# Quantus-Network/qp-zk-circuits

Measured on AMD Instinct MI355X. Metric: Wormhole proofs/sec, higher is better.
Workload: dtype u64

## Files before the change

### include/qpgpu.h

```cpp
#ifndef QPGPU_H
#define QPGPU_H
#include <stddef.h>
#include <stdint.h>

#ifdef __cplusplus
extern "C" {
#endif

typedef struct qpgpu_ctx qpgpu_ctx;
typedef struct qpgpu_circuit qpgpu_circuit;

enum {
    QPGPU_OK = 0,
    QPGPU_EINVAL = -1,
    QPGPU_EDEVICE = -2,
    QPGPU_ENOMEM = -3,
    QPGPU_EUNSAT = -4,
    QPGPU_EBUFSIZE = -5
};

int qpgpu_ctx_create(int device, qpgpu_ctx **out);
void qpgpu_ctx_destroy(qpgpu_ctx *ctx);
const char *qpgpu_last_error(const qpgpu_ctx *ctx);
int qpgpu_ctx_set_stream(qpgpu_ctx *ctx, void *hip_stream);
int qpgpu_sync(qpgpu_ctx *ctx);
const char *qpgpu_version(void);
int qpgpu_ctx_pci_bus_id(const qpgpu_ctx *ctx, char *out, size_t out_len);
int qpgpu_crash_trace_armed(void);

int qpgpu_profile_enable(qpgpu_ctx *ctx, int on);
int qpgpu_profile_read(qpgpu_ctx *ctx, const char *kernel, double *total_ms, uint64_t *launches);

int qpgpu_malloc(qpgpu_ctx *ctx, size_t bytes, void **dptr);
int qpgpu_free(qpgpu_ctx *ctx, void *dptr);
int qpgpu_free_scrubbed(qpgpu_ctx *ctx, void *dptr, size_t bytes);
int qpgpu_memcpy_h2d(qpgpu_ctx *ctx, void *dst_dev, const void *src_host, size_t bytes);
int qpgpu_memcpy_d2h(qpgpu_ctx *ctx, void *dst_host, const void *src_dev, size_t bytes);
int qpgpu_memcpy_d2d(qpgpu_ctx *ctx, void *dst_dev, const void *src_dev, size_t bytes);

typedef struct { uint64_t word; uint32_t region; uint32_t pinned; uint64_t offset_words; uint64_t alloc_bytes; } qpgpu_residue_hit;
#define QPGPU_RESIDUE_MAX_NEEDLES 16
int qpgpu_ctx_residue_scan(qpgpu_ctx *ctx, const uint64_t *needles, size_t n_needles, uint64_t region_mask,
                           uint64_t *hits, qpgpu_residue_hit *first_hits, size_t cap, uint64_t *bytes_scanned);
const char *qpgpu_residue_region_name(uint32_t region);
int qpgpu_ctx_residue_audit_begin(qpgpu_ctx *ctx, const uint64_t *needles, size_t n_needles);
int qpgpu_ctx_residue_audit_end(qpgpu_ctx *ctx, uint64_t *hits, qpgpu_residue_hit *first_hits, size_t cap, uint64_t *buffers_released);

#define QPGPU_HASH_POSEIDON 0
#define QPGPU_HASH_POSEIDON2 1
#define QPGPU_POSEIDON2_PARAM_WORDS 146
int qpgpu_ctx_set_hasher(qpgpu_ctx *ctx, int kind, const uint64_t *params, size_t n_words);
int qpgpu_ctx_get_hasher(const qpgpu_ctx *ctx);
int qpgpu_set_hasher(int kind, const uint64_t *params, size_t n_words);
int qpgpu_get_hasher(void);

enum {
    QPGPU_NTT_FORWARD = 0,
    QPGPU_NTT_INVERSE = 1,
    QPGPU_NTT_OUT_BITREV = 2
};
int qpgpu_ntt_batch(qpgpu_ctx *ctx, uint64_t *data, unsigned log_n, size_t batch, int flags,
                    uint64_t coset_shift);
int qpgpu_ntt_batch_dev(qpgpu_ctx *ctx, const uint64_t *d_in, uint64_t *d_out, unsigned log_n,
                        size_t batch, int flags, uint64_t coset_shift);
int qpgpu_lde_batch_dev(qpgpu_ctx *ctx, const uint64_t *d_coeffs, uint64_t *d_out, unsigned log_n,
                        unsigned rate_bits, size_t batch, int flags, uint64_t coset_shift);

int qpgpu_poseidon_permute_dev(qpgpu_ctx *ctx, uint64_t *d_states, size_t n);
int qpgpu_poseidon2_hash_pad10_dev(qpgpu_ctx *ctx, const uint64_t *params, size_t n_words, const uint64_t *d_in, size_t len,
                                   size_t count, uint64_t *d_out);
size_t qpgpu_merkle_digest_count(unsigned log_leaves, unsigned cap_height);
int qpgpu_merkle_build_dev(qpgpu_ctx *ctx, const uint64_t *d_cols, uint64_t col_stride, uint32_t n_cols,
                           unsigned log_leaves, unsigned cap_height, uint64_t *d_digests, uint64_t *h_cap_out);
int qpgpu_merkle_build_rows_dev(qpgpu_ctx *ctx, const uint64_t *d_rows, uint32_t width, unsigned log_leaves,
                                unsigned cap_height, uint64_t *d_digests, uint64_t *h_cap_out);

int qpgpu_circuit_load(qpgpu_ctx *ctx, const uint64_t *pack_words, size_t n_words, qpgpu_circuit **out);
int qpgpu_circuit_load_batch(qpgpu_ctx *ctx, const uint64_t *pack_words, size_t n_words, unsigned max_batch, qpgpu_circuit **out);
unsigned qpgpu_circuit_max_batch(const qpgpu_circuit *c);
size_t qpgpu_circuit_num_public_inputs(const qpgpu_circuit *c);
void qpgpu_circuit_free(qpgpu_circuit *c);
int qpgpu_circuit_scrub(qpgpu_circuit *c);
int qpgpu_circuit_constants_sigmas_cap(const qpgpu_circuit *c, uint64_t *out, size_t out_words);
int qpgpu_circuit_set_blinding_seed(qpgpu_circuit *c, uint64_t seed);
int qpgpu_circuit_set_witness_check(qpgpu_circuit *c, int on);
int qpgpu_circuit_set_quotient_fused(qpgpu_circuit *c, int on);
int qpgpu_circuit_quotient_info(const qpgpu_circuit *c, int *fused_enabled, int *fused_selected);
int qpgpu_circuit_quotient_pair_info(const qpgpu_circuit *c, int *enabled, int *selected);
size_t qpgpu_proof_size(const qpgpu_circuit *c);
int qpgpu_prove(qpgpu_circuit *c, const uint64_t *wires, const uint64_t *public_inputs, uint8_t *out, size_t out_cap, size_t *out_len);
int qpgpu_prove_dev(qpgpu_circuit *c, const uint64_t *d_wires, const uint64_t *public_inputs, uint8_t *out, size_t out_cap, size_t *out_len);
int qpgpu_prove_batch_dev(qpgpu_circuit *c, const uint64_t *const *d_wires, uint32_t batch, const uint64_t *const *public_inputs,
                          uint8_t *const *outs, size_t out_cap, size_t *out_lens);

int qpgpu_witness_info(qpgpu_circuit *c, uint64_t *num_generators, uint64_t *num_levels, uint64_t *num_free_cells);
int qpgpu_witness_free_mask(qpgpu_circuit *c, uint8_t *mask, size_t mask_len);
int qpgpu_generate_witness_dev(qpgpu_circuit *c, uint64_t *d_wires, const uint64_t *public_inputs);
int qpgpu_generate_witness(qpgpu_circuit *c, uint64_t *wires, const uint64_t *public_inputs);
int qpgpu_circuit_gate_rows(const qpgpu_circuit *c, unsigned gate_type, uint32_t *rows_out, size_t cap, size_t *count);
int qpgpu_generate_witness_batch_dev(qpgpu_circuit *c, uint64_t *d_wires, uint32_t batch, const uint64_t *public_inputs);
int qpgpu_generate_witness_partial_dev(qpgpu_circuit *c, const uint64_t *cells, const uint64_t *values, size_t count,
                                       const uint64_t *public_inputs, uint64_t *d_wires);
int qpgpu_generate_witness_partial_batch_dev(qpgpu_circuit *c, const uint64_t *cells, size_t count, const uint64_t *values,
                                             const uint64_t *public_inputs, uint32_t batch, uint64_t *d_wires, int *status);
int qpgpu_witness_partial_prepare(qpgpu_circuit *c, const uint64_t *cells, size_t count, uint32_t max_batch);
int qpgpu_generate_witness_partial_batch_blinded_dev(qpgpu_circuit *c, const uint64_t *cells, size_t count, size_t n_blinding, const uint64_t *values,
                                                     const uint8_t *seeds, const uint64_t *public_inputs, uint32_t batch, uint64_t *d_wires, int *status);
int qpgpu_witness_public_inputs_dev(qpgpu_circuit *c, const uint64_t *d_wires, uint32_t batch, uint64_t *public_inputs_out);

typedef struct qpgpu_oracle qpgpu_oracle;
#define QPGPU_ORACLE_VALUES 0u
#define QPGPU_ORACLE_COEFFS 1u
#define QPGPU_ORACLE_BLINDING 2u
#define QPGPU_ORACLE_DEVICE_INPUT 4u
int qpgpu_oracle_commit(qpgpu_ctx *ctx, const uint64_t *polys, uint32_t num_polys, unsigned degree_bits, unsigned rate_bits,
                        unsigned cap_height, unsigned flags, uint64_t blinding_seed, uint32_t blinding_stream, qpgpu_oracle **out);
void qpgpu_oracle_free(qpgpu_oracle *o);
int qpgpu_oracle_cap(const qpgpu_oracle *o, uint64_t *out, size_t out_words);
int qpgpu_oracle_eval(qpgpu_oracle *o, const uint64_t point[2], uint32_t first, uint32_t count, uint64_t *out);
#define QPGPU_ORACLE_READ_COEFFS 0u
#define QPGPU_ORACLE_READ_LDE 1u
int qpgpu_oracle_read(qpgpu_oracle *o, unsigned what, uint32_t first, uint32_t count, uint64_t *out);
int qpgpu_oracle_device_ptrs(const qpgpu_oracle *o, const uint64_t **d_coeffs, const uint64_t **d_lde, const uint64_t **d_digests);
int qpgpu_oracle_open(qpgpu_oracle *o, const uint64_t *indices, size_t n, uint64_t *rows_out, uint64_t *paths_out);
size_t qpgpu_oracle_leaf_width(const qpgpu_oracle *o);

int qpgpu_oracle_commit_sharded(qpgpu_ctx *const *ctxs, uint32_t n_ctx, const uint64_t *polys, uint32_t num_polys,
                                unsigned degree_bits, unsigned rate_bits, unsigned cap_height, unsigned flags,
                                uint64_t blinding_seed, uint32_t blinding_stream, qpgpu_oracle **out);
uint32_t qpgpu_oracle_shards(const qpgpu_oracle *o);
int qpgpu_oracle_shard_range(const qpgpu_oracle *o, uint32_t shard, uint64_t *first_leaf, uint64_t *num_leaves);
int qpgpu_oracle_shard_device_ptrs(const qpgpu_oracle *o, uint32_t shard, const uint64_t **d_lde, const uint64_t **d_digests);

int qpgpu_oracle_commit_batch(qpgpu_ctx *ctx, const uint64_t *const *polys, uint32_t batch, uint32_t num_polys, unsigned degree_bits,
                              unsigned rate_bits, unsigned cap_height, unsigned flags, uint64_t blinding_seed, uint32_t blinding_stream,
                              qpgpu_oracle **out);
uint32_t qpgpu_oracle_batch(const qpgpu_oracle *o);
int qpgpu_oracle_strides(const qpgpu_oracle *o, uint64_t *coeffs, uint64_t *lde, uint64_t *digests);
int qpgpu_oracle_eval_batch(qpgpu_oracle *o, const uint64_t *points, uint32_t first, uint32_t count, uint64_t *out);
int qpgpu_oracle_open_batch(qpgpu_oracle *o, const uint64_t *indices, size_t n, uint64_t *rows_out, uint64_t *paths_out);

typedef struct {
    uint64_t sponge_state[12];
    uint64_t input_buffer[8];
    uint64_t output_buffer[8];
    uint32_t input_len, output_len;
} qpgpu_challenger;
void qpgpu_challenger_init(qpgpu_challenger *c);
int qpgpu_ctx_challenger_observe(const qpgpu_ctx *ctx, qpgpu_challenger *c, const uint64_t *elements, size_t n);
int qpgpu_ctx_challenger_get(const qpgpu_ctx *ctx, qpgpu_challenger *c, uint64_t *out);
void qpgpu_challenger_observe(qpgpu_challenger *c, const uint64_t *elements, size_t n);
uint64_t qpgpu_challenger_get(qpgpu_challenger *c);

typedef struct { uint32_t oracle, first, count; } qpgpu_fri_range;
typedef struct { uint64_t point[2]; uint32_t num_ranges; qpgpu_fri_range ranges[8]; } qpgpu_fri_batch;
typedef struct {
    uint32_t rate_bits, cap_height, proof_of_work_bits, num_query_rounds;
    uint32_t num_reduction_rounds; uint32_t reduction_arity_bits[16];
} qpgpu_fri_params;
size_t qpgpu_fri_proof_size(qpgpu_oracle *const *oracles, uint32_t num_oracles, const qpgpu_fri_params *params);
int qpgpu_fri_prove(qpgpu_ctx *ctx, qpgpu_oracle *const *oracles, uint32_t num_oracles, const qpgpu_fri_batch *batches,
                    uint32_t num_batches, const qpgpu_fri_params *params, qpgpu_challenger *challenger,
                    uint8_t *out, size_t out_cap, size_t *out_len);

typedef struct qpgpu_fri_session qpgpu_fri_session;
int qpgpu_fri_begin(qpgpu_ctx *ctx, qpgpu_oracle *const *oracles, uint32_t num_oracles, const qpgpu_fri_batch *batches,
                    uint32_t num_batches, const qpgpu_fri_params *params, const uint64_t alpha[2], qpgpu_fri_session **out);
int qpgpu_fri_round_commit(qpgpu_fri_session *s, uint64_t *cap_out, size_t cap_words);
int qpgpu_fri_round_fold(qpgpu_fri_session *s, const uint64_t beta[2]);
int qpgpu_fri_final_poly(qpgpu_fri_session *s, uint64_t *out, size_t out_words, size_t *num_coeffs);
size_t qpgpu_fri_query_size(const qpgpu_fri_session *s);
int qpgpu_fri_open(qpgpu_fri_session *s, const uint64_t *indices, size_t n, uint8_t *out, size_t out_cap, size_t *out_len);
void qpgpu_fri_session_free(qpgpu_fri_session *s);
int qpgpu_fri_grind(qpgpu_ctx *ctx, const qpgpu_challenger *c, unsigned proof_of_work_bits, uint64_t *nonce_out);

int qpgpu_fri_prove_batch(qpgpu_ctx *ctx, qpgpu_oracle *const *oracles, uint32_t num_oracles, const qpgpu_fri_batch *batches,
                          uint32_t num_batches, const uint64_t *points, uint32_t batch, const qpgpu_fri_params *params,
                          qpgpu_challenger *challengers, uint8_t *const *outs, size_t out_cap, size_t *out_lens);
int qpgpu_fri_begin_batch(qpgpu_ctx *ctx, qpgpu_oracle *const *oracles, uint32_t num_oracles, const qpgpu_fri_batch *batches,
                          uint32_t num_batches, const uint64_t *points, uint32_t batch, const qpgpu_fri_params *params,
                          const uint64_t *alphas, qpgpu_fri_session **out);
uint32_t qpgpu_fri_session_batch(const qpgpu_fri_session *s);
int qpgpu_fri_grind_batch(qpgpu_ctx *ctx, const qpgpu_challenger *cs, uint32_t batch, unsigned proof_of_work_bits, uint64_t *nonces_out);

typedef struct qpgpu_stage_plan qpgpu_stage_plan;
#define QPGPU_STAGE_ERR_CAP 256
int qpgpu_stage_plan_create(qpgpu_ctx *ctx, const uint64_t *words, size_t n_words, const qpgpu_oracle *cs_oracle,
                            qpgpu_stage_plan **out, char *err);
void qpgpu_stage_plan_free(qpgpu_stage_plan *plan);
int qpgpu_stage_plan_info(const qpgpu_stage_plan *plan, unsigned *degree_bits, unsigned *num_challenges,
                          unsigned *num_partial_products, unsigned *quotient_degree_factor, int *fused_selected);
int qpgpu_stage_partial_products(qpgpu_stage_plan *plan, const uint64_t *wires, int wires_on_device, const uint64_t *betas,
                                 const uint64_t *gammas, uint64_t *d_out);
int qpgpu_stage_quotient(qpgpu_stage_plan *plan, const qpgpu_oracle *wires_oracle, const qpgpu_oracle *zs_pp_oracle,
                         const uint64_t *betas, const uint64_t *gammas, const uint64_t *alphas, const uint64_t *public_inputs_hash,
                         uint64_t *d_out);

int qpgpu_stage_plan_create_sharded(qpgpu_ctx *ctx, const uint64_t *words, size_t n_words, const qpgpu_oracle *cs_oracle,
                                    qpgpu_stage_plan **out, char *err);
uint32_t qpgpu_stage_plan_shards(const qpgpu_stage_plan *plan);

int qpgpu_stage_plan_create_batch(qpgpu_ctx *ctx, const uint64_t *words, size_t n_words, const qpgpu_oracle *cs_oracle,
                                  uint32_t max_batch, qpgpu_stage_plan **out, char *err);
uint32_t qpgpu_stage_plan_max_batch(const qpgpu_stage_plan *plan);
int qpgpu_stage_partial_products_batch(qpgpu_stage_plan *plan, const uint64_t *const *wires, uint32_t batch, int wires_on_device,
                                       const uint64_t *betas, const uint64_t *gammas, uint64_t *d_out);
int qpgpu_stage_quotient_batch(qpgpu_stage_plan *plan, const qpgpu_oracle *wires_oracle, const qpgpu_oracle *zs_pp_oracle, uint32_t batch,
                               const uint64_t *betas, const uint64_t *gammas, const uint64_t *alphas,
                               const uint64_t *public_inputs_hashes, uint64_t *d_out);

typedef struct qpgpu_pool qpgpu_pool;
int qpgpu_pool_create(int device, const uint64_t *pack_words, size_t n_words, unsigned workers, qpgpu_pool **out);
int qpgpu_pool_create_batched(int device, const uint64_t *pack_words, size_t n_words, unsigned workers, unsigned max_batch, qpgpu_pool **out);
#define QPGPU_POOL_HOST_WITNESS 1u
int qpgpu_pool_create_multi(const int *devices, unsigned n_devices, const uint64_t *pack_words, size_t n_words, unsigned workers_per_device,
                            unsigned max_batch, unsigned flags, qpgpu_pool **out);
void qpgpu_pool_destroy(qpgpu_pool *p);
int qpgpu_pool_scrub(qpgpu_pool *p);
int qpgpu_pool_residue_scan(qpgpu_pool *p, const uint64_t *needles, size_t n_needles, uint64_t region_mask,
                            uint64_t *hits, qpgpu_residue_hit *first_hits, size_t cap, uint64_t *bytes_scanned);
int qpgpu_pool_set_witness_check(qpgpu_pool *p, int on);
size_t qpgpu_pool_proof_size(const qpgpu_pool *p);
unsigned qpgpu_pool_workers(const qpgpu_pool *p);
unsigned qpgpu_pool_devices(const qpgpu_pool *p);
int qpgpu_pool_serialized(const qpgpu_pool *p);
const char *qpgpu_pool_last_error(const qpgpu_pool *p);
int qpgpu_pool_submit(qpgpu_pool *p, const uint64_t *d_wires, const uint64_t *public_inputs, uint8_t *out, size_t out_cap, uint64_t *ticket);
int qpgpu_pool_submit_on(qpgpu_pool *p, unsigned device_index, const uint64_t *d_wires, const uint64_t *public_inputs, uint8_t *out, size_t out_cap, uint64_t *ticket);
int qpgpu_pool_submit_host(qpgpu_pool *p, const uint64_t *wires, const uint64_t *public_inputs, uint8_t *out, size_t out_cap, uint64_t *ticket);
int qpgpu_pool_set_partial_cells(qpgpu_pool *p, const uint64_t *cells, size_t count);
int qpgpu_pool_set_partial_cells_blinded(qpgpu_pool *p, const uint64_t *cells, size_t count, size_t n_blinding);
int qpgpu_pool_submit_partial(qpgpu_pool *p, const uint64_t *values, const uint64_t *public_inputs, uint8_t *out, size_t out_cap, uint64_t *ticket);
int qpgpu_pool_wait(qpgpu_pool *p, uint64_t ticket, size_t *out_len);

size_t qpgpu_poseidon_constants(uint64_t *round_constants_360, uint64_t *fast_partial, size_t fast_partial_cap);

size_t qpgpu_synth_pack_words(unsigned degree_bits, unsigned num_wires, unsigned num_routed);
size_t qpgpu_synth_p2_sites(unsigned degree_bits, unsigned num_public_inputs, unsigned flags, uint64_t *out, size_t cap_words);
size_t qpgpu_synth_pack_words_ex(unsigned degree_bits, unsigned num_wires, unsigned num_routed, unsigned flags);
int qpgpu_synth_circuit_ex(unsigned degree_bits, unsigned num_wires, unsigned num_routed, unsigned num_public_inputs,
                           uint64_t seed, unsigned flags, uint64_t *pack_out, size_t pack_cap_words, size_t *pack_words,
                           uint64_t *wires_out, uint64_t *pis_out);
int qpgpu_synth_circuit(unsigned degree_bits, unsigned num_wires, unsigned num_routed, unsigned num_public_inputs,
                        uint64_t seed, uint64_t *pack_out, size_t pack_cap_words, size_t *pack_words,
                        uint64_t *wires_out, uint64_t *pis_out);

enum {
    QPGPU_FP_CANON = 0, QPGPU_FP_ADD, QPGPU_FP_SUB, QPGPU_FP_NEG, QPGPU_FP_MUL, QPGPU_FP_SQR, QPGPU_FP_REDUCE128, QPGPU_FP_REDUCE96,
    QPGPU_FP_MUL_EPS, QPGPU_FP_ADD_CANONICAL, QPGPU_FP_MUL7, QPGPU_FP_INV, QPGPU_FP_POW, QPGPU_FP_MUL_POW2, QPGPU_FP_MUL_POW2_DYN,
    QPGPU_FP_MUL_GROUP, QPGPU_FP_ACC, QPGPU_FP_E2_ADD, QPGPU_FP_E2_SUB, QPGPU_FP_E2_MUL, QPGPU_FP_E2_SCALE, QPGPU_FP_E2_INV,
    QPGPU_FP_E2_POW, QPGPU_FP_DIF_REGS, QPGPU_FP_DIF_SPARSE, QPGPU_FP_OP_COUNT
};
int qpgpu_field_probe(qpgpu_ctx *ctx, unsigned op, unsigned param, const uint64_t *a, const uint64_t *b, size_t n,
                      uint64_t *out, size_t out_words, int on_device);

#ifdef __cplusplus
}
#endif
#endif
```

### qp-zk-circuits_amd/__init__.py

```python
from .binding import poseidon_constants, synth_circuit, Circuit, QpGpu, QpGpuError, lib_path, load_library, P, MULT_GEN
from .binding import StagePlan, stage_header_words
from .binding import FriSession, fri_grind
from .binding import FriVerifier
from .binding import fri_prove_batch, fri_grind_batch
from .binding import PolyOracle, Challenger, fri_prove, set_hasher_poseidon, set_hasher_poseidon2, ProvingPool
from .binding import pack_header, pack_public_input_cells, Verifier, poseidon2_qp_params, synth_p2_sites
from .binding import pack_p2_layout, pack_trailers, p2_site_cells, P2_NO_SWAP
from .binding import CircuitConfig, circuit_config, validate_circuit_config
from .binding import FP, FP_OPS, field_probe_host, field_probe_shape
from . import sharding
from . import aggregation
from . import leaf
from . import recursion
```

### qp-zk-circuits_amd/binding.py

```python
import ctypes
import os

import numpy as np

P = 0xFFFFFFFF00000001
MULT_GEN = 14293326489335486720

NTT_FORWARD = 0
NTT_INVERSE = 1
NTT_OUT_BITREV = 2

_HERE = os.path.dirname(os.path.abspath(__file__))


def lib_path():
    return os.path.join(_HERE, "libqpgpu.so")


class QpGpuError(RuntimeError):
    def __init__(self, code, msg):
        super().__init__(f"qpgpu error {code}: {msg}")
        self.code = code


_lib = None


def load_library():
    global _lib
    if _lib is not None:
        return _lib
    path = lib_path()
    if not os.path.exists(path):
        raise FileNotFoundError(f"{path} missing: run `python -c 'import __graft_entry__ as g; g.build()'`")
    lib = ctypes.CDLL(path)
    c = ctypes
    vp, u64p = c.c_void_p, c.c_void_p
    sigs = {
        "qpgpu_version": (c.c_char_p, []),
        "qpgpu_ctx_pci_bus_id": (c.c_int, [c.c_void_p, c.c_char_p, c.c_size_t]),
        "qpgpu_verifier_create": (c.c_int, [vp, c.c_size_t, vp, c.c_size_t, c.c_int, vp, c.c_size_t, c.POINTER(vp), c.c_char_p]),
        "qpgpu_verifier_free": (None, [vp]),
        "qpgpu_verifier_proof_size": (c.c_size_t, [vp]),
        "qpgpu_verifier_constants_sigmas_cap": (c.c_int, [vp, vp, c.c_size_t]),
        "qpgpu_verifier_verify": (c.c_int, [vp, c.c_char_p, c.c_size_t, c.c_char_p]),
        "qpgpu_verifier_verify_many": (c.c_int, [vp, vp, vp, c.c_size_t, c.c_uint, vp, c.c_char_p]),
        "qpgpu_verifier_verify_many_device": (c.c_int, [vp, vp, vp, vp, c.c_size_t, c.c_uint, vp, vp, c.c_char_p]),
        "qpgpu_verifier_verify_many_device_ex": (c.c_int, [vp, vp, vp, vp, c.c_size_t, c.c_uint, c.c_uint, vp, vp, c.c_char_p]),
        "qpgpu_fri_verifier_create": (c.c_int, [vp, c.c_int, vp, c.c_size_t, c.POINTER(vp), c.c_char_p]),
        "qpgpu_fri_verifier_free": (None, [vp]),
        "qpgpu_fri_verifier_proof_size": (c.c_size_t, [vp]),
        "qpgpu_fri_verifier_num_openings": (c.c_size_t, [vp]),
        "qpgpu_fri_verifier_challenges": (c.c_int, [vp, vp, c.c_char_p, c.c_size_t, u64p, u64p, c.POINTER(c.c_uint64), u64p, c.c_char_p]),
        "qpgpu_fri_verify": (c.c_int, [vp, vp, u64p, u64p, u64p, u64p, c.c_uint64, u64p, c.c_char_p, c.c_size_t, c.c_char_p]),
        "qpgpu_fri_verify_many_device": (c.c_int, [vp, vp, c.c_size_t, vp, vp, u64p, u64p, u64p, u64p, u64p, u64p, vp, vp, vp, vp, c.c_char_p]),
        "qpgpu_ctx_create": (c.c_int, [c.c_int, c.POINTER(vp)]),
        "qpgpu_ctx_destroy": (None, [vp]),
        "qpgpu_last_error": (c.c_char_p, [vp]),
        "qpgpu_ctx_set_stream": (c.c_int, [vp, vp]),
        "qpgpu_sync": (c.c_int, [vp]),
        "qpgpu_profile_enable": (c.c_int, [vp, c.c_int]),
        "qpgpu_profile_read": (c.c_int, [vp, c.c_char_p, c.POINTER(c.c_double), c.POINTER(c.c_uint64)]),
        "qpgpu_malloc": (c.c_int, [vp, c.c_size_t, c.POINTER(vp)]),
        "qpgpu_free": (c.c_int, [vp, vp]),
        "qpgpu_free_scrubbed": (c.c_int, [vp, vp, c.c_size_t]),
        "qpgpu_memcpy_h2d": (c.c_int, [vp, vp, vp, c.c_size_t]),
        "qpgpu_memcpy_d2h": (c.c_int, [vp, vp, vp, c.c_size_t]),
        "qpgpu_memcpy_d2d": (c.c_int, [vp, vp, vp, c.c_size_t]),
        "qpgpu_ntt_batch": (c.c_int, [vp, u64p, c.c_uint, c.c_size_t, c.c_int, c.c_uint64]),
        "qpgpu_ntt_batch_dev": (c.c_int, [vp, u64p, u64p, c.c_uint, c.c_size_t, c.c_int, c.c_uint64]),
        "qpgpu_lde_batch_dev": (c.c_int, [vp, u64p, u64p, c.c_uint, c.c_uint, c.c_size_t, c.c_int, c.c_uint64]),
        "qpgpu_poseidon_permute_dev": (c.c_int, [vp, u64p, c.c_size_t]),
        "qpgpu_poseidon2_hash_pad10_dev": (c.c_int, [vp, u64p, c.c_size_t, u64p, c.c_size_t, c.c_size_t, u64p]),
        "qpgpu_poseidon2_qp_params": (c.c_size_t, [u64p, c.c_size_t]),
        "qpgpu_zk_leaf_hash_batch": (c.c_int, [vp, vp, c.c_size_t, vp]),
        "qpgpu_zk_tree_build": (c.c_int, [vp, vp, c.c_size_t, c.c_uint, c.c_uint, c.POINTER(vp), c.c_char_p]),
        "qpgpu_zk_tree_free": (None, [vp]),
        "qpgpu_zk_tree_depth": (c.c_uint, [vp]),
        "qpgpu_zk_tree_leaf_count": (c.c_size_t, [vp]),
        "qpgpu_zk_tree_root": (c.c_int, [vp, vp]),
        "qpgpu_zk_tree_read_level": (c.c_int, [vp, c.c_uint, c.c_size_t, c.c_size_t, vp]),
        "qpgpu_zk_tree_open": (c.c_int, [vp, vp, c.c_size_t, vp, vp]),
        "qpgpu_zk_tree_build_reserved": (c.c_int, [vp, vp, c.c_size_t, c.c_size_t, c.c_uint, c.c_uint, c.POINTER(vp), c.c_char_p]),
        "qpgpu_zk_tree_capacity": (c.c_size_t, [vp]),
        "qpgpu_zk_tree_append": (c.c_int, [vp, vp, c.c_size_t, c.c_uint, vp, c.c_char_p]),
        "qpgpu_zk_tree_snapshot": (c.c_int, [vp, vp]),
        "qpgpu_zk_tree_open_at": (c.c_int, [vp, vp, vp, c.c_size_t, vp, vp]),
        "qpgpu_zk_tree_snapshots_at": (c.c_int, [vp, vp, c.c_size_t, vp]),
        "qpgpu_zk_tree_snapshot_check": (c.c_int, [vp, vp]),
        "qpgpu_zk_tree_open_at_counts": (c.c_int, [vp, vp, vp, c.c_size_t, vp, vp, vp]),
        "qpgpu_zk_tree_truncate": (c.c_int, [vp, c.c_size_t, vp, c.c_char_p]),
        "qpgpu_poseidon2_hash_pad10": (c.c_int, [u64p, c.c_size_t, u64p, c.c_size_t, u64p]),
        "qpgpu_crash_trace_armed": (c.c_int, []),
        "qpgpu_circuit_num_public_inputs": (c.c_size_t, [vp]),
        "qpgpu_merkle_digest_count": (c.c_size_t, [c.c_uint, c.c_uint]),
        "qpgpu_merkle_build_dev": (c.c_int, [vp, u64p, c.c_uint64, c.c_uint32, c.c_uint, c.c_uint, u64p, u64p]),
        "qpgpu_merkle_build_rows_dev": (c.c_int, [vp, u64p, c.c_uint32, c.c_uint, c.c_uint, u64p, u64p]),
        "qpgpu_circuit_load": (c.c_int, [vp, u64p, c.c_size_t, c.POINTER(vp)]),
        "qpgpu_circuit_load_batch": (c.c_int, [vp, u64p, c.c_size_t, c.c_uint, c.POINTER(vp)]),
        "qpgpu_circuit_max_batch": (c.c_uint, [vp]),
        "qpgpu_circuit_scrub": (c.c_int, [vp]),
        "qpgpu_prove_batch_dev": (c.c_int, [vp, vp, c.c_uint32, vp, vp, c.c_size_t, vp]),
        "qpgpu_ctx_set_hasher": (c.c_int, [vp, c.c_int, u64p, c.c_size_t]),
        "qpgpu_ctx_get_hasher": (c.c_int, [vp]),
        "qpgpu_ctx_challenger_observe": (c.c_int, [vp, vp, u64p, c.c_size_t]),
        "qpgpu_ctx_challenger_get": (c.c_int, [vp, vp, c.POINTER(c.c_uint64)]),
        "qpgpu_pool_create_batched": (c.c_int, [c.c_int, u64p, c.c_size_t, c.c_uint, c.c_uint, c.POINTER(vp)]),
        "qpgpu_circuit_free": (None, [vp]),
        "qpgpu_circuit_constants_sigmas_cap": (c.c_int, [vp, u64p, c.c_size_t]),
        "qpgpu_proof_size": (c.c_size_t, [vp]),
        "qpgpu_circuit_set_blinding_seed": (c.c_int, [vp, c.c_uint64]),
        "qpgpu_circuit_set_witness_check": (c.c_int, [vp, c.c_int]),
        "qpgpu_circuit_set_quotient_fused": (c.c_int, [vp, c.c_int]),
        "qpgpu_circuit_quotient_info": (c.c_int, [vp, c.POINTER(c.c_int), c.POINTER(c.c_int)]),
        "qpgpu_circuit_quotient_pair_info": (c.c_int, [vp, c.POINTER(c.c_int), c.POINTER(c.c_int)]),
        "qpgpu_circuit_gate_rows": (c.c_int, [vp, c.c_uint, vp, c.c_size_t, c.POINTER(c.c_size_t)]),
        "qpgpu_prove": (c.c_int, [vp, u64p, u64p, vp, c.c_size_t, c.POINTER(c.c_size_t)]),
        "qpgpu_prove_dev": (c.c_int, [vp, u64p, u64p, vp, c.c_size_t, c.POINTER(c.c_size_t)]),
        "qpgpu_poseidon_constants": (c.c_size_t, [u64p, u64p, c.c_size_t]),
        "qpgpu_pool_create": (c.c_int, [c.c_int, u64p, c.c_size_t, c.c_uint, c.POINTER(vp)]),
        "qpgpu_pool_destroy": (None, [vp]),
        "qpgpu_pool_proof_size": (c.c_size_t, [vp]),
        "qpgpu_pool_workers": (c.c_uint, [vp]),
        "qpgpu_pool_last_error": (c.c_char_p, [vp]),
        "qpgpu_pool_submit": (c.c_int, [vp, u64p, u64p, vp, c.c_size_t, c.POINTER(c.c_uint64)]),
        "qpgpu_pool_wait": (c.c_int, [vp, c.c_uint64, c.POINTER(c.c_size_t)]),
        "qpgpu_pool_set_witness_check": (c.c_int, [vp, c.c_int]),
        "qpgpu_pool_create_multi": (c.c_int, [vp, c.c_uint, u64p, c.c_size_t, c.c_uint, c.c_uint, c.c_uint, c.POINTER(vp)]),
        "qpgpu_pool_devices": (c.c_uint, [vp]),
        "qpgpu_pool_serialized": (c.c_int, [vp]),
        "qpgpu_pool_set_partial_cells": (c.c_int, [vp, u64p, c.c_size_t]),
        "qpgpu_pool_set_partial_cells_blinded": (c.c_int, [vp, u64p, c.c_size_t, c.c_size_t]),
        "qpgpu_pool_submit_on": (c.c_int, [vp, c.c_uint, u64p, u64p, vp, c.c_size_t, c.POINTER(c.c_uint64)]),
        "qpgpu_pool_submit_host": (c.c_int, [vp, u64p, u64p, vp, c.c_size_t, c.POINTER(c.c_uint64)]),
        "qpgpu_pool_submit_partial": (c.c_int, [vp, u64p, u64p, vp, c.c_size_t, c.POINTER(c.c_uint64)]),
        "qpgpu_set_hasher": (c.c_int, [c.c_int, u64p, c.c_size_t]),
        "qpgpu_get_hasher": (c.c_int, []),
        "qpgpu_witness_info": (c.c_int, [vp, c.POINTER(c.c_uint64), c.POINTER(c.c_uint64), c.POINTER(c.c_uint64)]),
        "qpgpu_witness_free_mask": (c.c_int, [vp, vp, c.c_size_t]),
        "qpgpu_generate_witness_dev": (c.c_int, [vp, u64p, u64p]),
        "qpgpu_generate_witness": (c.c_int, [vp, u64p, u64p]),
        "qpgpu_generate_witness_batch_dev": (c.c_int, [vp, u64p, c.c_uint32, u64p]),
        "qpgpu_generate_witness_partial_dev": (c.c_int, [vp, u64p, u64p, c.c_size_t, u64p, u64p]),
        "qpgpu_generate_witness_partial_batch_dev": (c.c_int, [vp, u64p, c.c_size_t, u64p, u64p, c.c_uint32, u64p, vp]),
        "qpgpu_generate_witness_partial_batch_blinded_dev": (c.c_int, [vp, u64p, c.c_size_t, c.c_size_t, u64p, c.c_char_p, u64p, c.c_uint32, u64p, vp]),
        "qpgpu_witness_public_inputs_dev": (c.c_int, [vp, u64p, c.c_uint32, u64p]),
        "qpgpu_witness_partial_prepare": (c.c_int, [vp, u64p, c.c_size_t, c.c_uint32]),
        "qpgpu_oracle_commit": (c.c_int, [vp, u64p, c.c_uint32, c.c_uint, c.c_uint, c.c_uint, c.c_uint, c.c_uint64, c.c_uint32,
                                          c.POINTER(vp)]),
        "qpgpu_oracle_free": (None, [vp]),
        "qpgpu_oracle_cap": (c.c_int, [vp, u64p, c.c_size_t]),
        "qpgpu_oracle_eval": (c.c_int, [vp, u64p, c.c_uint32, c.c_uint32, u64p]),
        "qpgpu_oracle_read": (c.c_int, [vp, c.c_uint, c.c_uint32, c.c_uint32, u64p]),
        "qpgpu_oracle_device_ptrs": (c.c_int, [vp, c.POINTER(vp), c.POINTER(vp), c.POINTER(vp)]),
        "qpgpu_oracle_open": (c.c_int, [vp, u64p, c.c_size_t, u64p, u64p]),
        "qpgpu_oracle_leaf_width": (c.c_size_t, [vp]),
        "qpgpu_oracle_commit_sharded": (c.c_int, [c.POINTER(vp), c.c_uint32, u64p, c.c_uint32, c.c_uint, c.c_uint, c.c_uint, c.c_uint,
                                                  c.c_uint64, c.c_uint32, c.POINTER(vp)]),
        "qpgpu_oracle_shards": (c.c_uint32, [vp]),
        "qpgpu_oracle_shard_range": (c.c_int, [vp, c.c_uint32, c.POINTER(c.c_uint64), c.POINTER(c.c_uint64)]),
        "qpgpu_oracle_shard_device_ptrs": (c.c_int, [vp, c.c_uint32, c.POINTER(vp), c.POINTER(vp)]),
        "qpgpu_stage_plan_create": (c.c_int, [vp, u64p, c.c_size_t, vp, c.POINTER(vp), c.c_char_p]),
        "qpgpu_stage_plan_create_sharded": (c.c_int, [vp, u64p, c.c_size_t, vp, c.POINTER(vp), c.c_char_p]),
        "qpgpu_stage_plan_shards": (c.c_uint32, [vp]),
        "qpgpu_stage_plan_free": (None, [vp]),
        "qpgpu_stage_plan_info": (c.c_int, [vp, c.POINTER(c.c_uint), c.POINTER(c.c_uint), c.POINTER(c.c_uint), c.POINTER(c.c_uint),
                                            c.POINTER(c.c_int)]),
        "qpgpu_stage_partial_products": (c.c_int, [vp, u64p, c.c_int, u64p, u64p, u64p]),
        "qpgpu_stage_quotient": (c.c_int, [vp, vp, vp, u64p, u64p, u64p, u64p, u64p]),
        "qpgpu_challenger_init": (None, [vp]),
        "qpgpu_challenger_observe": (None, [vp, u64p, c.c_size_t]),
        "qpgpu_challenger_get": (c.c_uint64, [vp]),
        "qpgpu_fri_proof_size": (c.c_size_t, [c.POINTER(vp), c.c_uint32, vp]),
        "qpgpu_fri_prove": (c.c_int, [vp, c.POINTER(vp), c.c_uint32, vp, c.c_uint32, vp, vp, vp, c.c_size_t,
                                      c.POINTER(c.c_size_t)]),
        "qpgpu_fri_begin": (c.c_int, [vp, c.POINTER(vp), c.c_uint32, vp, c.c_uint32, vp, u64p, c.POINTER(vp)]),
        "qpgpu_fri_round_commit": (c.c_int, [vp, u64p, c.c_size_t]),
        "qpgpu_fri_round_fold": (c.c_int, [vp, u64p]),
        "qpgpu_fri_final_poly": (c.c_int, [vp, u64p, c.c_size_t, c.POINTER(c.c_size_t)]),
        "qpgpu_fri_query_size": (c.c_size_t, [vp]),
        "qpgpu_fri_open": (c.c_int, [vp, u64p, c.c_size_t, vp, c.c_size_t, c.POINTER(c.c_size_t)]),
        "qpgpu_fri_session_free": (None, [vp]),
        "qpgpu_fri_grind": (c.c_int, [vp, vp, c.c_uint, c.POINTER(c.c_uint64)]),
        "qpgpu_oracle_commit_batch": (c.c_int, [vp, c.POINTER(vp), c.c_uint32, c.c_uint32, c.c_uint, c.c_uint, c.c_uint, c.c_uint,
                                                c.c_uint64, c.c_uint32, c.POINTER(vp)]),
        "qpgpu_oracle_batch": (c.c_uint32, [vp]),
        "qpgpu_oracle_strides": (c.c_int, [vp, c.POINTER(c.c_uint64), c.POINTER(c.c_uint64), c.POINTER(c.c_uint64)]),
        "qpgpu_oracle_eval_batch": (c.c_int, [vp, u64p, c.c_uint32, c.c_uint32, u64p]),
        "qpgpu_oracle_open_batch": (c.c_int, [vp, u64p, c.c_size_t, u64p, u64p]),
        "qpgpu_stage_plan_create_batch": (c.c_int, [vp, u64p, c.c_size_t, vp, c.c_uint32, c.POINTER(vp), c.c_char_p]),
        "qpgpu_stage_plan_max_batch": (c.c_uint32, [vp]),
        "qpgpu_stage_partial_products_batch": (c.c_int, [vp, c.POINTER(vp), c.c_uint32, c.c_int, u64p, u64p, u64p]),
        "qpgpu_stage_quotient_batch": (c.c_int, [vp, vp, vp, c.c_uint32, u64p, u64p, u64p, u64p, u64p]),
        "qpgpu_fri_prove_batch": (c.c_int, [vp, c.POINTER(vp), c.c_uint32, vp, c.c_uint32, u64p, c.c_uint32, vp, vp, c.POINTER(vp),
                                            c.c_size_t, c.POINTER(c.c_size_t)]),
        "qpgpu_fri_begin_batch": (c.c_int, [vp, c.POINTER(vp), c.c_uint32, vp, c.c_uint32, u64p, c.c_uint32, vp, u64p, c.POINTER(vp)]),
        "qpgpu_fri_session_batch": (c.c_uint32, [vp]),
        "qpgpu_fri_grind_batch": (c.c_int, [vp, vp, c.c_uint32, c.c_uint, c.POINTER(c.c_uint64)]),
        "qpgpu_field_probe": (c.c_int, [vp, c.c_uint, c.c_uint, u64p, u64p, c.c_size_t, u64p, c.c_size_t, c.c_int]),
        "qpgpu_synth_pack_words": (c.c_size_t, [c.c_uint, c.c_uint, c.c_uint]),
        "qpgpu_synth_pack_words_ex": (c.c_size_t, [c.c_uint, c.c_uint, c.c_uint, c.c_uint]),
        "qpgpu_synth_p2_sites": (c.c_size_t, [c.c_uint, c.c_uint, c.c_uint, u64p, c.c_size_t]),
        "qpgpu_synth_circuit_ex": (c.c_int, [c.c_uint, c.c_uint, c.c_uint, c.c_uint, c.c_uint64, c.c_uint, u64p, c.c_size_t,
                                             c.POINTER(c.c_size_t), u64p, u64p]),
        "qpgpu_synth_circuit": (c.c_int, [c.c_uint, c.c_uint, c.c_uint, c.c_uint, c.c_uint64, u64p, c.c_size_t,
                                          c.POINTER(c.c_size_t), u64p, u64p]),
        "qpgpu_ctx_residue_scan": (c.c_int, [vp, u64p, c.c_size_t, c.c_uint64, c.POINTER(c.c_uint64), vp, c.c_size_t, c.POINTER(c.c_uint64)]),
        "qpgpu_residue_region_name": (c.c_char_p, [c.c_uint32]),
        "qpgpu_ctx_residue_audit_begin": (c.c_int, [vp, u64p, c.c_size_t]),
        "qpgpu_ctx_residue_audit_end": (c.c_int, [vp, c.POINTER(c.c_uint64), vp, c.c_size_t, c.POINTER(c.c_uint64)]),
        "qpgpu_pool_scrub": (c.c_int, [vp]),
        "qpgpu_pool_residue_scan": (c.c_int, [vp, u64p, c.c_size_t, c.c_uint64, c.POINTER(c.c_uint64), vp, c.c_size_t, c.POINTER(c.c_uint64)]),
    }
    for name, (res, args) in sigs.items():
        fn = getattr(lib, name)
        fn.restype = res
        fn.argtypes = args
    _lib = lib
    return lib


def exported_symbols():
    import glob
    import re
    names = set()
    for hdr in glob.glob(os.path.join(os.path.dirname(_HERE), "include", "*.h")):
        names |= set(re.findall(r"\b(qpgpu_[a-z0-9_]+)\s*\(", open(hdr).read()))
    return sorted(names)


def set_hasher_poseidon():
    load_library().qpgpu_set_hasher(0, None, 0)


def _p2_block(rc_ext, rc_int, diag_m1, m4):
    return np.concatenate([np.asarray(rc_ext, dtype=np.uint64).ravel(), np.asarray(rc_int, dtype=np.uint64).ravel(),
                           np.asarray(diag_m1, dtype=np.uint64).ravel(), np.asarray(m4, dtype=np.uint64).ravel()])


def set_hasher_poseidon2(rc_ext, rc_int, diag_m1, m4):
    flat = _p2_block(rc_ext, rc_int, diag_m1, m4)
    rc = load_library().qpgpu_set_hasher(1, flat.ctypes.data, flat.size)
    if rc != 0:
        raise QpGpuError(rc, "qpgpu_set_hasher: bad Poseidon2 parameter block")


def poseidon2_qp_params():
    flat = np.empty(146, dtype=np.uint64)
    n = load_library().qpgpu_poseidon2_qp_params(flat.ctypes.data, flat.size)
    assert n == 146
    return flat[:96].reshape(8, 12).copy(), flat[96:118].copy(), flat[118:130].copy(), flat[130:146].reshape(4, 4).copy()


def poseidon_constants():
    lib = load_library()
    n = lib.qpgpu_poseidon_constants(None, None, 0)
    rc = np.empty(360, dtype=np.uint64); fp = np.empty(n, dtype=np.uint64)
    lib.qpgpu_poseidon_constants(rc.ctypes.data, fp.ctypes.data, n)
    return rc, fp


FP_OPS = ("canon", "add", "sub", "neg", "mul", "sqr", "reduce128", "reduce96", "mul_eps", "add_canonical", "mul7", "inv", "pow",
          "mul_pow2", "mul_pow2_dyn", "mul_group", "acc", "e2_add", "e2_sub", "e2_mul", "e2_scale", "e2_inv", "e2_pow", "dif_regs",
          "dif_sparse")
FP = {name: i for i, name in enumerate(FP_OPS)}


def field_probe_shape(op, param=0):
    name = FP_OPS[op]
    if name in ("mul_group", "acc"):
        return (param, param, param if name == "mul_group" else 1)
    if name in ("e2_add", "e2_sub", "e2_mul"):
        return (2, 2, 2)
    if name in ("e2_scale", "e2_pow"):
        return (2, 1, 2)
    if name == "e2_inv":
        return (2, 0, 2)
    if name in ("dif_regs", "dif_sparse"):
        return (1 << (param & 0xFF), 0, 1 << (param & 0xFF))
    return (1, 1 if name in ("add", "sub", "mul", "reduce128", "reduce96", "add_canonical", "pow") else 0, 1)

# ... 681 lines not shown
        b, g = self._challenges_batch(betas, batch), self._challenges_batch(gammas, batch)
        if isinstance(wires[0], np.ndarray):
            keep = [np.ascontiguousarray(w, dtype=np.uint64) for w in wires]
            ptrs, on_dev = [w.ctypes.data for w in keep], 0
        else:
            ptrs, on_dev = [_ptr(w) for w in wires], 1
        arr = (ctypes.c_void_p * batch)(*ptrs)
        out = self.gpu.alloc(batch * self.num_zs_pp * self.n * 8)
        rc = self.gpu.lib.qpgpu_stage_partial_products_batch(self.h, arr, batch, on_dev, b.ctypes.data, g.ctypes.data, out.ptr)
        if rc != 0:
            out.free(scrub=True)
            self.gpu._check(rc)
        return out

    def quotient_batch(self, wires_oracle, zs_pp_oracle, batch, betas, gammas, alphas, public_inputs_hashes):
        b, g, a = (self._challenges_batch(x, batch) for x in (betas, gammas, alphas))
        pih = self._challenges_batch(public_inputs_hashes, batch, 4)
        out = self.gpu.alloc(batch * self.num_quotient * self.n * 8)
        rc = self.gpu.lib.qpgpu_stage_quotient_batch(self.h, wires_oracle.h, zs_pp_oracle.h, batch, b.ctypes.data, g.ctypes.data,
                                                     a.ctypes.data, pih.ctypes.data, out.ptr)
        if rc != 0:
            out.free(scrub=True)
            self.gpu._check(rc)
        return out


def _fri_args(oracles, batches, reduction_arity_bits, rate_bits, cap_height, proof_of_work_bits, num_query_rounds):
    hs = (ctypes.c_void_p * len(oracles))(*[o.h for o in oracles])
    bs = (_FriBatch * len(batches))()
    for b, (point, ranges) in zip(bs, batches):
        if np.ndim(point) == 1:
            b.point[0], b.point[1] = int(point[0]), int(point[1])
        b.num_ranges = len(ranges)
        for r, (o, f, cnt) in zip(b.ranges, ranges):
            r.oracle, r.first, r.count = o, f, cnt
    prm = _FriParams(rate_bits, cap_height, proof_of_work_bits, num_query_rounds, len(reduction_arity_bits))
    for i, a in enumerate(reduction_arity_bits):
        prm.reduction_arity_bits[i] = a
    return hs, bs, prm


def fri_prove(gpu, oracles, batches, challenger, reduction_arity_bits, rate_bits=3, cap_height=4, proof_of_work_bits=16,
              num_query_rounds=28):
    hs, bs, prm = _fri_args(oracles, batches, reduction_arity_bits, rate_bits, cap_height, proof_of_work_bits, num_query_rounds)
    size = gpu.lib.qpgpu_fri_proof_size(hs, len(oracles), ctypes.byref(prm))
    if size == 0:
        raise QpGpuError(-1, "fri_prove: bad oracles or FRI parameters")
    out = np.empty(size, dtype=np.uint8)
    ln = ctypes.c_size_t()
    gpu._check(gpu.lib.qpgpu_fri_prove(gpu.ctx, hs, len(oracles), ctypes.byref(bs), len(batches), ctypes.byref(prm),
                                       ctypes.byref(challenger.state), out.ctypes.data, out.size, ctypes.byref(ln)))
    return out[:ln.value].tobytes()


def fri_prove_batch(gpu, oracles, batches, challengers, reduction_arity_bits, rate_bits=3, cap_height=4, proof_of_work_bits=16,
                    num_query_rounds=28):
    nb = len(challengers)
    hs, bs, prm = _fri_args(oracles, batches, reduction_arity_bits, rate_bits, cap_height, proof_of_work_bits, num_query_rounds)
    pts = np.ascontiguousarray(np.array([np.array(pt, dtype=np.uint64).reshape(nb, 2) for pt, _ in batches], dtype=np.uint64))
    size = gpu.lib.qpgpu_fri_proof_size(hs, len(oracles), ctypes.byref(prm))
    if size == 0:
        raise QpGpuError(-1, "fri_prove: bad oracles or FRI parameters")
    states = (ChallengerState * nb)()
    for i, ch in enumerate(challengers):
        ctypes.memmove(ctypes.byref(states[i]), ctypes.byref(ch.state), ctypes.sizeof(ChallengerState))
    outs = [np.empty(size, dtype=np.uint8) for _ in range(nb)]
    optr = (ctypes.c_void_p * nb)(*[o.ctypes.data for o in outs])
    lens = (ctypes.c_size_t * nb)()
    gpu._check(gpu.lib.qpgpu_fri_prove_batch(gpu.ctx, hs, len(oracles), ctypes.byref(bs), len(batches), pts.ctypes.data, nb,
                                             ctypes.byref(prm), ctypes.byref(states), optr, size, lens))
    for i, ch in enumerate(challengers):
        ctypes.memmove(ctypes.byref(ch.state), ctypes.byref(states[i]), ctypes.sizeof(ChallengerState))
    return [outs[i][:lens[i]].tobytes() for i in range(nb)]


def fri_grind_batch(gpu, challengers, proof_of_work_bits):
    nb = len(challengers)
    states = (ChallengerState * nb)()
    for i, ch in enumerate(challengers):
        ctypes.memmove(ctypes.byref(states[i]), ctypes.byref(ch.state), ctypes.sizeof(ChallengerState))
    nonces = (ctypes.c_uint64 * nb)()
    gpu._check(gpu.lib.qpgpu_fri_grind_batch(gpu.ctx, ctypes.byref(states), nb, proof_of_work_bits, nonces))
    return [int(x) for x in nonces]


def fri_grind(gpu, challenger, proof_of_work_bits):
    nonce = ctypes.c_uint64()
    gpu._check(gpu.lib.qpgpu_fri_grind(gpu.ctx, ctypes.byref(challenger.state), proof_of_work_bits, ctypes.byref(nonce)))
    return int(nonce.value)


class FriSession:

    def __init__(self, gpu, oracles, batches, alpha, reduction_arity_bits, rate_bits=3, cap_height=4, batch=None):
        self.gpu, self.oracles, self.batch = gpu, list(oracles), batch
        hs, bs, prm = _fri_args(oracles, batches, reduction_arity_bits, rate_bits, cap_height, 0, 0)
        h = ctypes.c_void_p()
        if batch is None:
            a = np.array([int(alpha[0]), int(alpha[1])], dtype=np.uint64)
            gpu._check(gpu.lib.qpgpu_fri_begin(gpu.ctx, hs, len(oracles), ctypes.byref(bs), len(batches), ctypes.byref(prm), a.ctypes.data,
                                               ctypes.byref(h)))
        else:
            a = np.ascontiguousarray(np.array(alpha, dtype=np.uint64).reshape(batch, 2))
            pts = np.ascontiguousarray(np.array([np.array(pt, dtype=np.uint64).reshape(batch, 2) for pt, _ in batches], dtype=np.uint64))
            gpu._check(gpu.lib.qpgpu_fri_begin_batch(gpu.ctx, hs, len(oracles), ctypes.byref(bs), len(batches), pts.ctypes.data, batch,
                                                     ctypes.byref(prm), a.ctypes.data, ctypes.byref(h)))
            assert int(gpu.lib.qpgpu_fri_session_batch(h)) == batch
        self.h = h
        self.cap_height, self.arity_bits = cap_height, list(reduction_arity_bits)
        self.lde_size = 1 << (oracles[0].degree_bits + rate_bits)
        self.final_len = 1 << (oracles[0].degree_bits - sum(self.arity_bits))
        self.query_size = int(gpu.lib.qpgpu_fri_query_size(h))

    def close(self):
        if self.h:
            self.gpu.lib.qpgpu_fri_session_free(self.h)
            self.h = None

    def __enter__(self):
        return self

    def __exit__(self, *a):
        self.close()

    def round_commit(self):
        shape = (1 << self.cap_height, 4) if self.batch is None else (self.batch, 4 << self.cap_height)
        cap = np.empty(shape, dtype=np.uint64)
        self.gpu._check(self.gpu.lib.qpgpu_fri_round_commit(self.h, cap.ctypes.data, cap.size))
        return cap

    def round_fold(self, beta):
        b = np.ascontiguousarray(np.array(beta, dtype=np.uint64).reshape(self.batch or 1, 2))
        self.gpu._check(self.gpu.lib.qpgpu_fri_round_fold(self.h, b.ctypes.data))

    def final_poly(self):
        out = np.empty((self.final_len, 2) if self.batch is None else (self.batch, self.final_len, 2), dtype=np.uint64)
        n = ctypes.c_size_t()
        self.gpu._check(self.gpu.lib.qpgpu_fri_final_poly(self.h, out.ctypes.data, out.size, ctypes.byref(n)))
        assert n.value == self.final_len
        return out

    def open(self, indices):
        if self.batch is not None:
            idx = np.ascontiguousarray(np.array(indices, dtype=np.uint64).reshape(self.batch, -1))
            n, per = idx.shape[1], idx.shape[1] * self.query_size
            out = np.empty(max(1, self.batch * per), dtype=np.uint8)
            ln = ctypes.c_size_t()
            self.gpu._check(self.gpu.lib.qpgpu_fri_open(self.h, idx.ctypes.data if n else None, n, out.ctypes.data, self.batch * per,
                                                        ctypes.byref(ln)))
            assert ln.value == self.batch * per
            return [out[b * per:(b + 1) * per].tobytes() for b in range(self.batch)]
        idx = np.ascontiguousarray(indices, dtype=np.uint64).ravel()
        out = np.empty(max(1, idx.size * self.query_size), dtype=np.uint8)
        ln = ctypes.c_size_t()
        self.gpu._check(self.gpu.lib.qpgpu_fri_open(self.h, idx.ctypes.data if idx.size else None, idx.size, out.ctypes.data,
                                                    idx.size * self.query_size, ctypes.byref(ln)))
        return out[:ln.value].tobytes()


class _FriOracleShape(ctypes.Structure):
    _fields_ = [("num_polys", ctypes.c_uint32), ("blinded", ctypes.c_uint32)]


class _FriInstance(ctypes.Structure):
    _fields_ = [("degree_bits", ctypes.c_uint32), ("num_oracles", ctypes.c_uint32), ("oracles", ctypes.POINTER(_FriOracleShape)),
                ("num_batches", ctypes.c_uint32), ("batches", ctypes.POINTER(_FriBatch)), ("params", _FriParams)]
# ... 241 lines not shown
        return self._submitted(rc, t, (p, out, None))

    def scrub(self):
        rc = self.lib.qpgpu_pool_scrub(self.h)
        if rc != 0:
            raise QpGpuError(rc, self.lib.qpgpu_pool_last_error(self.h).decode())

    def residue_scan(self, needles, regions=None, cap=16):
        rc, hits, first, nbytes = _residue_call(self.lib.qpgpu_pool_residue_scan, self.h, needles, regions, cap)
        if rc != 0:
            raise QpGpuError(rc, self.lib.qpgpu_pool_last_error(self.h).decode())
        return hits, first, nbytes

    def wait(self, ticket, copy=True):
        ln = ctypes.c_size_t()
        rc = self.lib.qpgpu_pool_wait(self.h, ticket, ctypes.byref(ln))
        p, out, _ = self._keep.pop(ticket, (None, None, None))
        if rc != 0:
            raise QpGpuError(rc, self.lib.qpgpu_pool_last_error(self.h).decode())
        return out[:ln.value].tobytes() if copy else ln.value


class _ResidueAudit:
    def __init__(self, gpu, needles, cap):
        self.gpu, self.cap = gpu, cap
        self.needles = np.ascontiguousarray(needles, dtype=np.uint64)
        self.hits = self.buffers_released = None
        self.first_hits = []

    def __enter__(self):
        self.gpu._check(self.gpu.lib.qpgpu_ctx_residue_audit_begin(self.gpu.ctx, self.needles.ctypes.data, self.needles.size))
        return self

    def __exit__(self, *a):
        hits, released = ctypes.c_uint64(), ctypes.c_uint64()
        first = _blank_hits(self.cap)
        self.gpu._check(self.gpu.lib.qpgpu_ctx_residue_audit_end(self.gpu.ctx, ctypes.byref(hits), first, self.cap, ctypes.byref(released)))
        self.hits, self.buffers_released = hits.value, released.value
        self.first_hits = _written_hits(first, self.cap)


class _Stage3:

    def poseidon_permute(self, states):
        st = np.ascontiguousarray(states, dtype=np.uint64).reshape(-1, 12)
        d = self.to_device(st)
        self._check(self.lib.qpgpu_poseidon_permute_dev(self.ctx, d.ptr, st.shape[0]))
        out = d.download().reshape(-1, 12)
        d.free()
        return out

    def poseidon2_hash_pad10(self, preimages, params=None):
        pre = np.ascontiguousarray(preimages, dtype=np.uint64)
        pre = pre.reshape(1, -1) if pre.ndim == 1 else pre
        count, ln = pre.shape
        d_in = self.to_device(pre) if pre.size else self.alloc(8)
        d_out = self.alloc(max(count, 1) * 32)
        try:
            if params is None:
                self._check(self.lib.qpgpu_poseidon2_hash_pad10_dev(self.ctx, None, 0, d_in.ptr, ln, count, d_out.ptr))
            else:
                blk = np.ascontiguousarray(params, dtype=np.uint64)
                self._check(self.lib.qpgpu_poseidon2_hash_pad10_dev(self.ctx, blk.ctypes.data, blk.size, d_in.ptr, ln, count, d_out.ptr))
            self.sync()
            return d_out.download()[:count * 4].reshape(count, 4).copy()
        finally:
            d_in.free(); d_out.free()

    def merkle_digest_count(self, log_leaves, cap_height):
        return self.lib.qpgpu_merkle_digest_count(log_leaves, cap_height)

    def merkle_build_dev(self, d_cols, col_stride, n_cols, log_leaves, cap_height, d_digests):
        cap = np.empty((1 << cap_height, 4), dtype=np.uint64)
        self._check(self.lib.qpgpu_merkle_build_dev(self.ctx, _ptr(d_cols), col_stride, n_cols, log_leaves,
                                                    cap_height, _ptr(d_digests), cap.ctypes.data))
        return cap

    def merkle_build_rows_dev(self, d_rows, width, log_leaves, cap_height, d_digests):
        cap = np.empty((1 << cap_height, 4), dtype=np.uint64)
        self._check(self.lib.qpgpu_merkle_build_rows_dev(self.ctx, _ptr(d_rows), width, log_leaves, cap_height,
                                                         _ptr(d_digests), cap.ctypes.data))
        return cap


class QpGpu(_Stage3):

    def __init__(self, device=0, stream=None, hasher=None):
        self.lib = load_library()
        ctx = ctypes.c_void_p()
        rc = self.lib.qpgpu_ctx_create(device, ctypes.byref(ctx))
        if rc != 0:
            raise QpGpuError(rc, "qpgpu_ctx_create failed (no gfx950 device visible?)")
        self.ctx = ctx
        if hasher is not None:
            if isinstance(hasher, str):
                self._check(self.lib.qpgpu_ctx_set_hasher(self.ctx, 0, None, 0))
            else:
                flat = _p2_block(*hasher)
                self._check(self.lib.qpgpu_ctx_set_hasher(self.ctx, 1, flat.ctypes.data, flat.size))
        if stream is not None:
            self._check(self.lib.qpgpu_ctx_set_stream(self.ctx, ctypes.c_void_p(stream)))

    def close(self):
        if self.ctx:
            self.lib.qpgpu_ctx_destroy(self.ctx)
            self.ctx = None

    def __enter__(self):
        return self

    def __exit__(self, *a):
        self.close()

    def _check(self, rc):
        if rc != 0:
            raise QpGpuError(rc, self.lib.qpgpu_last_error(self.ctx).decode())

    def last_error(self):
        return self.lib.qpgpu_last_error(self.ctx).decode()

    def sync(self):
        self._check(self.lib.qpgpu_sync(self.ctx))

    def commit_sharded(self, ctxs, polys, **kw):
        assert ctxs and ctxs[0] is self, "the home context comes first"
        return PolyOracle.commit_sharded(ctxs, polys, **kw)

    def pci_bus_id(self):
        buf = ctypes.create_string_buffer(16)
        self._check(self.lib.qpgpu_ctx_pci_bus_id(self.ctx, buf, 16))
        return buf.value.decode()

    def profile(self, on=True):
        self._check(self.lib.qpgpu_profile_enable(self.ctx, 1 if on else 0))

    def profile_read(self, kernel):
        ms, n = ctypes.c_double(), ctypes.c_uint64()
        self._check(self.lib.qpgpu_profile_read(self.ctx, kernel.encode(), ctypes.byref(ms), ctypes.byref(n)))
        return ms.value, n.value

    def residue_scan(self, needles, regions=None, cap=16):
        rc, hits, first, nbytes = _residue_call(self.lib.qpgpu_ctx_residue_scan, self.ctx, needles, regions, cap)
        self._check(rc)
        return hits, first, nbytes

    def residue_audit(self, needles, cap=16):
        return _ResidueAudit(self, needles, cap)

    def alloc(self, nbytes):
        return DeviceBuffer(self, nbytes)

    def to_device(self, arr):
        arr = np.ascontiguousarray(arr)
        return DeviceBuffer(self, arr.nbytes).upload(arr)

    def field_probe(self, op, a, b=None, param=0):
        rc, out = _field_probe(self.ctx, op, a, b, param, True)
        self._check(rc)
        return out

    def ntt_host(self, data, log_n, inverse=False, coset_shift=0, bitrev=False):
        a = np.array(data, dtype=np.uint64, copy=True).reshape(-1, 1 << log_n)
        flags = (NTT_INVERSE if inverse else 0) | (NTT_OUT_BITREV if bitrev else 0)
        self._check(self.lib.qpgpu_ntt_batch(self.ctx, a.ctypes.data, log_n, a.shape[0], flags, coset_shift))
        return a

# ... 16 lines not shown
```

### qp-zk-circuits_amd/csrc/fri_api.cpp

```cpp
#include <hip/hip_runtime.h>
#include <algorithm>
#include <cstring>
#include <string>
#include "fri_prover.hpp"
#include "oracle_handle.hpp"

using gl::e2;
using gl::u64;

namespace {
struct FriCall {
    FriParams fp;
    std::vector<size_t> widths;
    std::vector<FriBatch> bs;
    std::vector<const PolyOracle *> os;
    size_t max_count = 0;
    uint32_t nb = 1;
};

int fri_setup(qpgpu_oracle *const *oracles, uint32_t n, const qpgpu_fri_params *params, FriParams &fp, std::vector<size_t> &widths) {
    if (!oracles || n == 0 || !params || params->num_reduction_rounds > 16) return QPGPU_EINVAL;
    for (uint32_t i = 0; i < n; i++) if (!oracles[i] || oracles[i]->ctx != oracles[0]->ctx) return QPGPU_EINVAL;
    fp.degree_bits = oracles[0]->o.log_n; fp.rate_bits = params->rate_bits; fp.cap_h = params->cap_height;
    fp.pow_bits = params->proof_of_work_bits; fp.num_queries = params->num_query_rounds;
// ... 198 lines not shown
        return ctx->fail(QPGPU_EINVAL, "fri_round_commit: cap_words is " + std::to_string(cap_words) + ", the cap has " + std::to_string(want) + " words" +
                                           (s->st.nb > 1 ? " for the session's " + std::to_string(s->st.nb) + " proofs" : ""));
    QP_FRI_ORDER(s, FriSteps::COMMIT);
    QP_TRY(fri_round_commit(s->st));
    std::memcpy(cap_out, s->st.caps.back().data(), cap_words * 8);
    return QPGPU_OK;
}

int qpgpu_fri_round_fold(qpgpu_fri_session *s, const uint64_t *beta) {
    if (!s) return QPGPU_EINVAL;
    qpgpu_ctx *ctx = s->ctx;
    QP_DEV(ctx);
    if (!beta) return ctx->fail(QPGPU_EINVAL, "fri_round_fold: beta is NULL");
    QP_FRI_ORDER(s, FriSteps::FOLD);
    std::vector<e2> b(s->st.nb);
    for (uint32_t i = 0; i < s->st.nb; i++) b[i] = gl::e2_make(gl::canon(beta[2 * i]), gl::canon(beta[2 * i + 1]));
    return fri_round_fold(s->st, b.data());
}

int qpgpu_fri_final_poly(qpgpu_fri_session *s, uint64_t *out, size_t out_words, size_t *num_coeffs) {
    if (!s) return QPGPU_EINVAL;
    qpgpu_ctx *ctx = s->ctx;
    QP_DEV(ctx);
    if (!out) return ctx->fail(QPGPU_EINVAL, "fri_final_poly: out is NULL");
    const size_t len = s->st.w->proof.final_len, nb = s->st.nb;
    if (out_words != nb * 2 * len)
        return ctx->fail(QPGPU_EINVAL, "fri_final_poly: out_words is " + std::to_string(out_words) + ", the final polynomial has " + std::to_string(nb * 2 * len) + " words" +
                                           (nb > 1 ? " for the session's " + std::to_string(nb) + " proofs" : ""));
    QP_FRI_ORDER(s, FriSteps::FINAL_POLY);
    std::vector<u64> fc;
    QP_TRY(fri_final_poly(s->st, fc));
    for (size_t b = 0; b < nb; b++)
        for (size_t i = 0; i < len; i++) { out[2 * (b * len + i)] = fc[2 * b * len + i]; out[2 * (b * len + i) + 1] = fc[2 * b * len + len + i]; }
    if (num_coeffs) *num_coeffs = len;
    return QPGPU_OK;
}

size_t qpgpu_fri_query_size(const qpgpu_fri_session *s) { return s ? s->st.w->proof.round_bytes : 0; }

int qpgpu_fri_open(qpgpu_fri_session *s, const uint64_t *indices, size_t n, uint8_t *out, size_t out_cap, size_t *out_len) {
    if (!s) return QPGPU_EINVAL;
    qpgpu_ctx *ctx = s->ctx;
    QP_DEV(ctx);
    QP_FRI_ORDER(s, FriSteps::OPEN);
    if (n == 0) { if (out_len) *out_len = 0; return QPGPU_OK; }
    if (!indices) return ctx->fail(QPGPU_EINVAL, "fri_open: indices is NULL");
    if (!out) return ctx->fail(QPGPU_EINVAL, "fri_open: out is NULL");
    const size_t qs = qpgpu_fri_query_size(s), nb = s->st.nb;
    if (out_cap / qs / nb < n)
        return ctx->fail(QPGPU_EINVAL, "fri_open: out_cap is " + std::to_string(out_cap) + ", " + std::to_string(n) + " query rounds take " +
                                           (nb > 1 ? std::to_string(nb) + " x " : "") + std::to_string(n) + " x " + std::to_string(qs) + " bytes");
    const unsigned L = s->st.p.degree_bits + s->st.p.rate_bits;
    for (size_t b = 0; b < nb; b++)
        for (size_t i = 0; i < n; i++)
            if (indices[b * n + i] >> L)
                return ctx->fail(QPGPU_EINVAL, "fri_open: indices[" + (nb > 1 ? std::to_string(b) + "][" : "") + std::to_string(i) + "] = " + std::to_string(indices[b * n + i]) +
                                                   " is not below 2^" + std::to_string(L));
    Stager &stage = s->space.stage;
    if (!s->opened) { s->opened = true; s->open_pos = stage.pos; }
    std::vector<ByteWriter> ws;
    for (size_t b = 0; b < nb; b++) ws.push_back(ByteWriter{out + b * n * qs, n * qs});
    std::vector<u64> idx;
    for (size_t at = 0; at < n; at += kOpenChunk) {
        stage.pos = s->open_pos;
        const uint32_t m = (uint32_t)std::min<size_t>(kOpenChunk, n - at);
        idx.resize(nb * m);
        for (size_t b = 0; b < nb; b++) std::memcpy(idx.data() + b * m, indices + b * n + at, (size_t)m * 8);
        QP_TRY(fri_gather(s->st, idx.data(), m, ws.data()));
    }
    if (out_len) *out_len = nb * n * qs;
    return QPGPU_OK;
}

static int grind_impl(qpgpu_ctx *ctx, const qpgpu_challenger *cs, uint32_t nb, unsigned proof_of_work_bits, uint64_t *nonces_out) {
    if (proof_of_work_bits > 40) return ctx->fail(QPGPU_EINVAL, "fri_grind: proof_of_work_bits above 40");
    std::vector<Challenger> chs(nb, Challenger(ctx->hasher));
    for (uint32_t b = 0; b < nb; b++) {
        if (!challenger_to_host(&cs[b], chs[b])) return ctx->fail(QPGPU_EINVAL, "fri_grind: invalid challenger state (input_len must be < 8, output_len <= 8)");
        if (chs[b].n_in != chs[0].n_in) return ctx->fail(QPGPU_EINVAL, "fri_grind: challengers[" + std::to_string(b) + "] holds another number of pending inputs than challengers[0]: the transcripts of a batch advance together");
    }
    if (proof_of_work_bits == 0) { for (uint32_t b = 0; b < nb; b++) nonces_out[b] = 0; return QPGPU_OK; }
    ctx->hasher_in_use = true;
    QP_TRY(merkle_ensure_constants(ctx));
    QP_TRY(ctx->ensure_scratch((size_t)nb * 16 * 8));
    Stager bounce;
    std::vector<u64> nonces(nb, 0);
    u64 *t = ctx->scratch;
    QP_TRY(fri_grind(ctx, chs.data(), nb, proof_of_work_bits, PowTables{t, t + 12 * (size_t)nb, t + 13 * (size_t)nb}, bounce, nonces.data()));
    for (uint32_t b = 0; b < nb; b++) nonces_out[b] = nonces[b];
    return QPGPU_OK;
}

int qpgpu_fri_grind(qpgpu_ctx *ctx, const qpgpu_challenger *c, unsigned proof_of_work_bits, uint64_t *nonce_out) {
    if (!ctx || !c || !nonce_out) return QPGPU_EINVAL;
    QP_DEV(ctx);
    return grind_impl(ctx, c, 1, proof_of_work_bits, nonce_out);
}

int qpgpu_fri_grind_batch(qpgpu_ctx *ctx, const qpgpu_challenger *cs, uint32_t batch, unsigned proof_of_work_bits, uint64_t *nonces_out) {
    if (!ctx || !cs || !nonces_out) return QPGPU_EINVAL;
    QP_DEV(ctx);
    if (batch == 0 || batch > 1024) return ctx->fail(QPGPU_EINVAL, "fri_grind_batch: batch must be 1..1024");
    return grind_impl(ctx, cs, batch, proof_of_work_bits, nonces_out);
}

}
```

### qp-zk-circuits_amd/csrc/fri_prover.cpp

```cpp
#include <hip/hip_runtime.h>
#include <sys/random.h>
#include <algorithm>
#include <string>
#include "fri_prover.hpp"
#include "merkle.hpp"
#include "prover_kernels.hpp"

using gl::e2;
using gl::u64;

int Stager::put(qpgpu_ctx *ctx, void *dst, const void *src, size_t bytes) {
    const size_t w = (bytes + 7) / 8;
    if (!h || pos + w > words) {
        QP_TRY(ctx->reserve_read_back(bytes));
        QP_HIP(ctx, hipStreamSynchronize(ctx->stream));
        std::memcpy(ctx->h_pin, src, bytes);
        QP_HIP(ctx, pk_copy(dst, ctx->h_pin, bytes, ctx->stream));
        QP_HIP(ctx, hipStreamSynchronize(ctx->stream));
        return QPGPU_OK;
    }
    u64 *slot = h + pos;
    pos += w;
    std::memcpy(slot, src, bytes);
    QP_HIP(ctx, pk_copy(dst, slot, bytes, ctx->stream));
// ... 6 lines not shown
        for (size_t r = 0; r < rows; r++) QP_TRY(put(ctx, dst + r * dst_pitch, src + r * src_pitch, row_words * 8));
        return QPGPU_OK;
    }
    u64 *slot = h + pos;
    pos += w;
    for (size_t r = 0; r < rows; r++) std::memcpy(slot + r * row_words, src + r * src_pitch, row_words * 8);
    QP_HIP(ctx, pk_unpack_rows(slot, dst_pitch, row_words, rows, dst, ctx->stream));
    return QPGPU_OK;
}

int salt_key_random(uint32_t key[8]) {
    size_t got = 0;
    while (got < 32) {
        const ssize_t r = getrandom((uint8_t *)key + got, 32 - got, 0);
        if (r <= 0) return QPGPU_EDEVICE;
        got += (size_t)r;
    }
    return QPGPU_OK;
}
void salt_key_from_seed(uint64_t seed, uint32_t key[8]) {
    key[0] = (uint32_t)seed; key[1] = (uint32_t)(seed >> 32);
    key[2] = 0x51504750u; key[3] = 0x53414c54u;
    key[4] = key[5] = key[6] = key[7] = 0;
}

int oracle_commit_coeffs(qpgpu_ctx *ctx, PolyOracle &o, const uint32_t *d_keys) {
    const unsigned L = o.log_lde();
    const uint32_t nb = o.nb;
    if (nb > 1 && (o.ps_coeffs != ((u64)o.ncols << o.log_n) || o.ps_lde != ((u64)o.ncols << L)))
        return ctx->fail(QPGPU_EINVAL, "oracle_commit: batched oracles are dense arrays");
    QP_TRY(ntt_run(ctx, o.coeffs, o.lde, o.log_n, L, (size_t)nb * o.ncols, false, true, gl::MULT_GEN));
    MerkleLeafArgs a{};
    a.src0 = o.lde; a.stride0 = 1ull << L; a.ncols0 = o.ncols; a.n_leaves = 1ull << L; a.digests = o.digests;
    a.batch = nb; a.ps_src0 = o.ps_lde; a.ps_digests = o.ps_digests;
    if (o.salt) {
        if (!d_keys) return ctx->fail(QPGPU_EINVAL, "oracle_commit: a blinded oracle needs salt keys");
        QP_HIP(ctx, pk_salt(d_keys, o.oracle_index, 1ull << L, o.salt, nb, ctx->stream));
        a.src1 = o.salt; a.stride1 = 1ull << L; a.ncols1 = 4; a.ps_src1 = o.ps_salt;
    }
    QP_TRY(merkle_build(ctx, a, L, o.cap_h, o.digests));
    const size_t total = digest_words(L, o.cap_h), cw = o.cap_words();
    o.cap.resize(cw * nb);
    QP_TRY(ctx->read_back_2d(o.cap.data(), o.digests + total - cw, o.ps_digests * 8, cw * 8, nb));
    return QPGPU_OK;
}

int oracle_commit_values(qpgpu_ctx *ctx, const u64 *d_values, PolyOracle &o, const uint32_t *d_keys) {
    QP_TRY(ntt_run(ctx, d_values, o.coeffs, o.log_n, o.log_n, (size_t)o.nb * o.ncols, true, false, 0));
    return oracle_commit_coeffs(ctx, o, d_keys);
}

namespace {
proof_layout::Fri proof_part(const FriParams &p, const std::vector<size_t> &leaf_widths) {
    return proof_layout::fri_part(p.degree_bits, p.rate_bits, p.cap_h, std::vector<uint64_t>(p.arity_bits.begin(), p.arity_bits.end()), p.num_queries, leaf_widths);
}
struct Layout {
    size_t comp, fin, vals, coeffs0, coeffs1, gather, alpha, ws;
    std::vector<size_t> digests, leafrows;
    proof_layout::Fri proof;
    size_t gather_words;
    size_t t_points, t_shifts, t_betas, pow_states, pow_bases, pow_results, qidx, total;
};
Layout layout(const FriParams &p, const std::vector<size_t> &leaf_widths, size_t max_batch_polys, uint32_t nb) {
    Layout l;
    const size_t n = 1ull << p.degree_bits, lde_n = n << p.rate_bits;
    const unsigned L = p.degree_bits + p.rate_bits;
    size_t off = 0;
    auto take = [&](size_t words) { size_t o = off; off += (words + 1) & ~(size_t)1; return o; };
    l.comp = take(2 * n); l.fin = take(2 * n); l.vals = take(2 * lde_n); l.coeffs0 = take(2 * n); l.coeffs1 = take(2 * n);
    unsigned lvl = L;
    for (unsigned a : p.arity_bits) {
        lvl -= a;
        l.digests.push_back(take(digest_words(lvl, p.cap_h)));
        l.leafrows.push_back(take((size_t)2 << (lvl + a)));
    }
    l.proof = proof_part(p, leaf_widths);
    size_t gw = 0;
    for (const proof_layout::Opening &o : l.proof.op) gw += o.row_words + o.path_len * 4;
    l.gather_words = gw * p.num_queries;
    l.gather = take(l.gather_words); l.alpha = take(2 * max_batch_polys);
    l.ws = off;
    off = l.ws * nb;
    l.t_points = take(2 * (size_t)nb); l.t_shifts = take(2 * (size_t)nb); l.t_betas = take(2 * (size_t)nb);
    l.pow_states = take(12 * (size_t)nb); l.pow_bases = take(nb); l.pow_results = take(nb); l.qidx = take((size_t)nb * p.num_queries);
    l.total = off;
    return l;
}
}

size_t FriWork::words(const FriParams &p, const std::vector<size_t> &leaf_widths, size_t max_batch_polys, uint32_t nb) {
    return layout(p, leaf_widths, max_batch_polys, nb).total;
}
void FriWork::bind(u64 *base, const FriParams &p, const std::vector<size_t> &leaf_widths, size_t mbp, uint32_t nb) {
    const Layout l = layout(p, leaf_widths, mbp, nb);
    ws = l.ws; nb_cap = nb;
    comp = base + l.comp; fin = base + l.fin; vals = base + l.vals; coeffs[0] = base + l.coeffs0; coeffs[1] = base + l.coeffs1;
    digests.clear(); leafrows.clear();
    for (size_t o : l.digests) digests.push_back(base + o);
    for (size_t o : l.leafrows) leafrows.push_back(base + o);
    gather = base + l.gather; alpha_ext = (e2 *)(base + l.alpha);
    gather_words = l.gather_words; max_batch_polys = mbp; proof = l.proof;
    t_points = (e2 *)(base + l.t_points); t_shifts = (e2 *)(base + l.t_shifts); t_betas = (e2 *)(base + l.t_betas);
    pow_states = base + l.pow_states; pow_bases = base + l.pow_bases; pow_results = base + l.pow_results; qidx = base + l.qidx;
}

size_t fri_proof_bytes(const FriParams &p, const std::vector<size_t> &leaf_widths) { return proof_part(p, leaf_widths).total; }

int fri_begin(qpgpu_ctx *ctx, const FriParams &p, const PolyOracle *const *oracles, size_t n_oracles, const std::vector<FriBatch> &batches,
              uint32_t nb, const e2 *alphas, FriWork &w, Stager &stage, bool one_call, FriState &s) {
    hipStream_t st = ctx->stream;
    const unsigned d = p.degree_bits, L = d + p.rate_bits, cap_h = p.cap_h;
    const u64 n = 1ull << d;
    if (nb == 0 || nb > w.nb_cap) return ctx->fail(QPGPU_EINVAL, "fri_prove: batch larger than the workspace");
    if (w.proof.op.size() != n_oracles + p.arity_bits.size()) return ctx->fail(QPGPU_EINVAL, "fri_prove: workspace bound for other oracles or FRI rounds");
    for (size_t i = 0; i < n_oracles; i++) {
        if (oracles[i]->log_n != d || oracles[i]->rate_bits != p.rate_bits || oracles[i]->cap_h != cap_h)
            return ctx->fail(QPGPU_EINVAL, "fri_prove: oracle " + std::to_string(i) + " does not match the FRI parameters");
        if (oracles[i]->nb != 1 && oracles[i]->nb < nb) return ctx->fail(QPGPU_EINVAL, "fri_prove: oracle committed for fewer proofs than the batch");
    }
    { unsigned tot = 0; for (unsigned a : p.arity_bits) { tot += a; if (a == 0 || a > 8) return ctx->fail(QPGPU_EINVAL, "fri_prove: bad reduction arity"); }
      if (tot > d || L - tot < cap_h) return ctx->fail(QPGPU_EINVAL, "fri_prove: reduction schedule does not fit the degree / cap height"); }

    size_t max_count = 0;
    for (const FriBatch &fb : batches) {
        if (fb.ranges.empty() || fb.ranges.size() > 8) return ctx->fail(QPGPU_EINVAL, "fri_prove: a batch needs 1..8 polynomial ranges");
        if (fb.points.size() != nb) return ctx->fail(QPGPU_EINVAL, "fri_prove: one opening point per proof expected");
        size_t cnt = 0;
        for (const FriRange &rg : fb.ranges) {
            if (rg.oracle >= n_oracles || (size_t)rg.first + rg.count > oracles[rg.oracle]->ncols || rg.count == 0)
                return ctx->fail(QPGPU_EINVAL, "fri_prove: polynomial range outside its oracle");
            cnt += rg.count;
        }
        max_count = std::max(max_count, cnt);
    }
    if (max_count == 0 || max_count > w.max_batch_polys) return ctx->fail(QPGPU_EINVAL, "fri_prove: empty batch or workspace too small");
    ctx->prof_begin("prove_fri_batch");
    {
        std::vector<e2> apw((size_t)nb * max_count);
        for (uint32_t b = 0; b < nb; b++) {
            e2 a = gl::e2_from(1);
            for (size_t i = 0; i < max_count; i++) { apw[(size_t)b * max_count + i] = gl::e2_canon(a); a = gl::e2_mul(a, alphas[b]); }
        }
        QP_TRY(stage.put_rows(ctx, (u64 *)w.alpha_ext, w.ws, (const u64 *)apw.data(), 2 * max_count, 2 * max_count, nb));
    }
    for (size_t bi = 0; bi < batches.size(); bi++) {
        const FriBatch &fb = batches[bi];
        ReduceArgs ra{};
        size_t count = 0;
        for (size_t r = 0; r < fb.ranges.size(); r++) {
            const FriRange &rg = fb.ranges[r];
            const PolyOracle *o = oracles[rg.oracle];
            ra.src[r] = o->coeffs + (size_t)rg.first * n; ra.ps_src[r] = o->ps_coeffs; ra.ncols[r] = rg.count;
            count += rg.count;
        }
        ra.nsrc = (uint32_t)fb.ranges.size();
        ra.alpha_pows = w.alpha_ext; ra.comp_a = w.comp; ra.comp_b = w.comp + n; ra.n = n;
        ra.batch = nb; ra.ps_alpha = w.ws / 2; ra.ps_comp = w.ws;
        QP_HIP(ctx, pk_reduce_polys(ra, st));
        std::vector<e2> pts(nb), shifts(nb);
        for (uint32_t b = 0; b < nb; b++) {
            pts[b] = gl::e2_canon(fb.points[b]);
            shifts[b] = bi == 0 ? gl::e2_from(1) : gl::e2_canon(gl::e2_pow(alphas[b], count));
        }
        QP_TRY(stage.put(ctx, w.t_points, pts.data(), nb * sizeof(e2)));
        QP_TRY(stage.put(ctx, w.t_shifts, shifts.data(), nb * sizeof(e2)));
        QP_HIP(ctx, pk_divide_linear(w.comp, w.comp + n, n, w.t_points, w.t_shifts, bi == 0 ? 0 : 1, w.fin, w.fin + n, nb, w.ws, w.ws, st));
    }
    ctx->prof_end();

    s = FriState();
    s.ctx = ctx; s.p = p; s.oracles.assign(oracles, oracles + n_oracles); s.nb = nb; s.w = &w; s.stage = &stage; s.one_call = one_call;
    s.steps = FriSteps((unsigned)p.arity_bits.size());
    s.shift = gl::MULT_GEN;
    s.coef = w.fin; s.valid = n; s.log_len = L; s.slot = 0;
    ctx->prof_begin("prove_fri_commit");
    NttProofs np; np.nproofs = nb; np.in_ps = w.ws; np.out_ps = w.ws;
    QP_TRY(ntt_run(ctx, s.coef, w.vals, d, L, 2, false, true, s.shift, np));
    if (!one_call) ctx->prof_end();
    return QPGPU_OK;
}

int fri_round_commit(FriState &s) {
    qpgpu_ctx *ctx = s.ctx; hipStream_t st = ctx->stream; FriWork &w = *s.w;
    const HasherDev hd = ctx->hasher_dev();
    const size_t r = s.steps.round;
    const uint32_t nb = s.nb;
    const unsigned ab = s.p.arity_bits[r], cap_h = s.p.cap_h;
    const u64 len = 1ull << s.log_len, arity = 1ull << ab;
    const unsigned log_leaves = s.log_len - ab;
    const size_t cap_words = s.cap_words();
    if (!s.one_call) ctx->prof_begin("prove_fri_commit");
    u64 *rows = w.leafrows[r];
    QP_HIP(ctx, pk_interleave_ext(w.vals, w.vals + len, len, rows, nb, w.ws, w.ws, st));
    QP_HIP(ctx, merkle_leaf_hash_rows(rows, 1ull << log_leaves, (uint32_t)(2 * arity), w.digests[r], nb, w.ws, w.ws, hd, st));
    {
        u64 cnt = 1ull << log_leaves; u64 *lvl = w.digests[r];
        QP_HIP(ctx, merkle_reduce_to_cap(lvl, cnt, 1ull << cap_h, nb, w.ws, hd, st));
        while (cnt > (1ull << cap_h)) { lvl += cnt * 4; cnt >>= 1; }
        std::vector<u64> capv(cap_words * nb);
        QP_TRY(ctx->read_back_2d(capv.data(), lvl, w.ws * 8, cap_words * 8, nb));
        s.caps.push_back(capv);
    }
    if (!s.one_call) ctx->prof_end();
    s.tree_log_leaves.push_back(log_leaves);
    s.steps.done(FriSteps::COMMIT);
    return QPGPU_OK;
}

int fri_round_fold(FriState &s, const e2 *betas) {
    qpgpu_ctx *ctx = s.ctx; hipStream_t st = ctx->stream; FriWork &w = *s.w;
    const size_t r = s.steps.round;
    const uint32_t nb = s.nb;
    const unsigned ab = s.p.arity_bits[r];
    const u64 arity = 1ull << ab;
    if (!s.one_call) ctx->prof_begin("prove_fri_commit");
    QP_TRY(s.stage->put(ctx, w.t_betas, betas, nb * sizeof(e2)));
    const u64 new_valid = s.valid >> ab;
    u64 *ncoef = w.coeffs[s.slot]; s.slot ^= 1;
    QP_HIP(ctx, pk_fri_fold(s.coef, s.coef + s.valid, new_valid, (uint32_t)arity, w.t_betas, ncoef, ncoef + new_valid, nb, w.ws, w.ws, st));
    s.coef = ncoef; s.valid = new_valid; s.log_len -= ab;
    s.shift = gl::pow(s.shift, arity);
    s.steps.done(FriSteps::FOLD);
    if (r + 1 < s.p.arity_bits.size()) {
        unsigned lv = 0; while ((1ull << lv) < s.valid) lv++;
        NttProofs np; np.nproofs = nb; np.in_ps = w.ws; np.out_ps = w.ws;
        QP_TRY(ntt_run(ctx, s.coef, w.vals, lv, s.log_len, 2, false, true, s.shift, np));
    }
    if (!s.one_call) ctx->prof_end();
    return QPGPU_OK;
}

int fri_final_poly(FriState &s, std::vector<u64> &out) {
    qpgpu_ctx *ctx = s.ctx;
    if (!s.one_call) ctx->prof_begin("prove_fri_commit");
    out.resize(2 * s.valid * s.nb);
    QP_TRY(ctx->read_back_2d(out.data(), s.coef, s.w->ws * 8, 2 * s.valid * 8, s.nb));
    ctx->prof_end();
    return QPGPU_OK;
}

int fri_grind(qpgpu_ctx *ctx, const Challenger *chs, uint32_t nb, unsigned pow_bits, const PowTables &t, Stager &stage, u64 *witness) {
    hipStream_t st = ctx->stream;
    ctx->prof_begin("prove_pow");
    for (uint32_t b = 0; b < nb; b++) witness[b] = 0;
    if (pow_bits > 0) {
        const HasherDev hd = ctx->hasher_dev();
        std::vector<u64> states(12 * (size_t)nb);
        for (uint32_t b = 0; b < nb; b++) {
            std::memcpy(states.data() + 12 * (size_t)b, chs[b].state, 12 * 8);
            for (int i = 0; i < chs[b].n_in; i++) states[12 * (size_t)b + i] = chs[b].in[i];
            if (chs[b].n_in != chs[0].n_in) return ctx->fail(QPGPU_EDEVICE, "prove: transcripts of a batch diverged in length");
        }
        QP_TRY(stage.put(ctx, t.states, states.data(), states.size() * 8));
        PowArgs pw{};
        pw.states = t.states; pw.bases = t.bases; pw.results = t.results;
        pw.pos = (uint32_t)chs[0].n_in; pw.pow_bits = pow_bits; pw.batch = nb;
        const u64 span = std::max<u64>(1ull << 16, 4ull << pw.pow_bits);
        pw.count = span;
        std::vector<u64> bases(nb, 0), res(nb);
        std::vector<char> found(nb, 0);
        uint32_t n_found = 0;
        QP_HIP(ctx, hipMemsetAsync(t.results, 0xFF, 8 * (size_t)nb, st));
        const size_t stage_pos = stage.pos;
        for (u64 round = 0; n_found < nb; round++) {
            stage.pos = stage_pos;
            for (uint32_t b = 0; b < nb; b++) bases[b] = found[b] ? ~0ull : round * span;
            QP_TRY(stage.put(ctx, t.bases, bases.data(), 8 * (size_t)nb));
            QP_HIP(ctx, pk_pow(pw, hd, st));
            QP_TRY(ctx->read_back(res.data(), t.results, 8 * (size_t)nb));
            for (uint32_t b = 0; b < nb; b++)
                if (!found[b] && res[b] != ~0ull) { witness[b] = res[b]; found[b] = 1; n_found++; }
            if (round * span > (1ull << 41)) return ctx->fail(QPGPU_EDEVICE, "prove: proof of work not found");
        }
    }
    ctx->prof_end();
    return QPGPU_OK;
}

int fri_gather(FriState &s, const u64 *qidx, uint32_t nq, ByteWriter *outs) {
    qpgpu_ctx *ctx = s.ctx; hipStream_t st = ctx->stream; FriWork &w = *s.w;
    const uint32_t nb = s.nb;
    const size_t n_oracles = s.oracles.size();
    const u64 lde_n = s.lde_n();
    if (nq > s.p.num_queries) return ctx->fail(QPGPU_EINVAL, "fri_gather: more query indices than the workspace holds");
    ctx->prof_begin("prove_queries");
    QP_TRY(s.stage->put(ctx, w.qidx, qidx, (size_t)nq * nb * 8));
    struct Sec { size_t off, words; bool is_path; };
    std::vector<Sec> secs;
    struct Routed { size_t oracle, off; };
    std::vector<Routed> sharded;
    size_t goff = 0;
    for (size_t i = 0; i < n_oracles; i++) {
        const PolyOracle *o = s.oracles[i];
        const uint32_t plen0 = (uint32_t)w.proof.op[i].path_len;
        if (o->sh) {
            if (nb != 1) return ctx->fail(QPGPU_EINVAL, "fri_gather: sharded oracles are not taken in a lockstep batch yet");
            sharded.push_back({i, goff});
            secs.push_back({goff, o->ncols, false}); goff += (size_t)o->ncols * nq;
            if (o->blinded) { secs.push_back({goff, 4, false}); goff += (size_t)4 * nq; }
            secs.push_back({goff, (size_t)plen0 * 4, true}); goff += (size_t)plen0 * 4 * nq;
            continue;
        }
        QP_HIP(ctx, pk_gather_rows(o->lde, lde_n, o->ncols, w.qidx, nq, w.gather + goff, nb, o->ps_lde, w.ws, st));
        secs.push_back({goff, o->ncols, false}); goff += (size_t)o->ncols * nq;
        if (o->salt) {
            QP_HIP(ctx, pk_gather_rows(o->salt, lde_n, 4, w.qidx, nq, w.gather + goff, nb, o->ps_salt, w.ws, st));
            secs.push_back({goff, 4, false}); goff += (size_t)4 * nq;
        }
        QP_HIP(ctx, pk_gather_paths(o->digests, lde_n, plen0, w.qidx, 0, nq, w.gather + goff, nb, o->ps_digests, w.ws, st));
        secs.push_back({goff, (size_t)plen0 * 4, true}); goff += (size_t)plen0 * 4 * nq;
    }
    for (size_t r = 0; r < s.p.arity_bits.size(); r++) {
        const proof_layout::Opening &op = w.proof.op[n_oracles + r];
        const uint32_t width = (uint32_t)op.row_words, pl = (uint32_t)op.path_len, sh = (uint32_t)op.shift;
        QP_HIP(ctx, pk_gather_leaf_rows(w.leafrows[r], width, w.qidx, sh, nq, w.gather + goff, nb, w.ws, w.ws, st));
        secs.push_back({goff, width, false}); goff += (size_t)width * nq;
        QP_HIP(ctx, pk_gather_paths(w.digests[r], 1ull << s.tree_log_leaves[r], pl, w.qidx, sh, nq, w.gather + goff, nb, w.ws, w.ws, st));
        secs.push_back({goff, (size_t)pl * 4, true}); goff += (size_t)pl * 4 * nq;
    }
    if (goff * s.p.num_queries != w.gather_words * nq) return ctx->fail(QPGPU_EDEVICE, "prove: internal gather size mismatch");
    std::vector<u64> gathered(goff * nb);
    QP_TRY(ctx->read_back_2d(gathered.data(), w.gather, w.ws * 8, goff * 8, nb));
    for (const Routed &rt : sharded) {
        const PolyOracle *o = s.oracles[rt.oracle];
        const size_t width = (size_t)o->ncols + (o->blinded ? 4 : 0), plen0 = w.proof.op[rt.oracle].path_len;
        std::vector<u64> rows(width * nq), paths(plen0 * 4 * nq);
        QP_TRY(oracle_sharded_open(*o, qidx, nq, rows.data(), plen0 ? paths.data() : nullptr));
        u64 *g_rows = gathered.data() + rt.off, *g_salt = g_rows + (size_t)o->ncols * nq, *g_paths = g_rows + width * nq;
        for (uint32_t q = 0; q < nq; q++) {
            std::memcpy(g_rows + (size_t)q * o->ncols, rows.data() + q * width, (size_t)o->ncols * 8);
            if (o->blinded) std::memcpy(g_salt + (size_t)q * 4, rows.data() + q * width + o->ncols, 32);
        }
        if (plen0) std::memcpy(g_paths, paths.data(), paths.size() * 8);
    }
    ctx->prof_end();
    for (uint32_t b = 0; b < nb; b++) {
        const u64 *g = gathered.data() + (size_t)b * goff;
        for (uint32_t q = 0; q < nq; q++) {
            for (const Sec &sc : secs) {
                if (sc.is_path) outs[b].u8((uint8_t)(sc.words / 4));
                outs[b].vec(g + sc.off + (size_t)q * sc.words, sc.words);
            }
        }
    }
    return QPGPU_OK;
}

int fri_prove(qpgpu_ctx *ctx, const FriParams &p, const PolyOracle *const *oracles, size_t n_oracles,
              const std::vector<FriBatch> &batches, uint32_t nb, Challenger *chs, FriWork &w, Stager &stage, ByteWriter *outs) {
    if (p.pow_bits > 40) return ctx->fail(QPGPU_EINVAL, "fri_prove: proof_of_work_bits above 40");
    if (nb == 0 || nb > w.nb_cap) return ctx->fail(QPGPU_EINVAL, "fri_prove: batch larger than the workspace");
    const u64 lde_n = 1ull << (p.degree_bits + p.rate_bits);
// ... 46 lines not shown
```

### qp-zk-circuits_amd/csrc/fri_prover.hpp

```cpp
#pragma once
#include "fri_steps.hpp"
#include "prover_host.hpp"

struct FriState {
    qpgpu_ctx *ctx = nullptr;
    FriParams p;
    std::vector<const PolyOracle *> oracles;
    uint32_t nb = 0;
    FriWork *w = nullptr;
    Stager *stage = nullptr;
    bool one_call = false;
    FriSteps steps;
    gl::u64 *coef = nullptr;
    gl::u64 valid = 0, shift = 0;
    unsigned log_len = 0;
    size_t slot = 0;
    std::vector<unsigned> tree_log_leaves;
    std::vector<std::vector<gl::u64>> caps;
    size_t cap_words() const { return (size_t)4 << p.cap_h; }
    gl::u64 lde_n() const { return 1ull << (p.degree_bits + p.rate_bits); }
};

int fri_begin(qpgpu_ctx *ctx, const FriParams &p, const PolyOracle *const *oracles, size_t n_oracles, const std::vector<FriBatch> &batches,
              uint32_t nb, const gl::e2 *alphas, FriWork &w, Stager &stage, bool one_call, FriState &s);
int fri_round_commit(FriState &s);
int fri_round_fold(FriState &s, const gl::e2 *betas);
int fri_final_poly(FriState &s, std::vector<gl::u64> &out);
struct PowTables { gl::u64 *states, *bases, *results; };
int fri_grind(qpgpu_ctx *ctx, const Challenger *chs, uint32_t nb, unsigned pow_bits, const PowTables &t, Stager &stage, gl::u64 *witness);
int fri_gather(FriState &s, const gl::u64 *qidx, uint32_t nq, ByteWriter *outs);
```

### qp-zk-circuits_amd/csrc/merkle_api.cpp

```cpp
#include <hip/hip_runtime.h>
#include <cstring>
#include <mutex>
#include "ctx.hpp"
#include "merkle.hpp"
#include "poseidon.hpp"

bool qpgpu_ctx::hasher_is_qp() const {
    const poseidon2::Params &q = poseidon2::qp_params();
    return memcmp(hasher.p2.rc_ext, q.rc_ext, sizeof q.rc_ext) == 0 && memcmp(hasher.p2.rc_int, q.rc_int, sizeof q.rc_int) == 0 &&
           memcmp(hasher.p2.diag_m1, q.diag_m1, sizeof q.diag_m1) == 0 && memcmp(hasher.p2.m4, q.m4, sizeof q.m4) == 0;
}

int merkle_ensure_constants(qpgpu_ctx *ctx) {
    static std::mutex mu;
    static bool uploaded[64] = {false}, uploaded_p2[64] = {false};
    {
        std::lock_guard<std::mutex> lk(mu);
        const int dev = ctx->device;
        if (dev < 0 || dev >= 64) return ctx->fail(QPGPU_EINVAL, "device index out of range");
        if (!uploaded[dev]) {
            QP_HIP(ctx, merkle_upload_constants(poseidon::host_hash_round_constants()));
            uploaded[dev] = true;
        }
        if (ctx->hasher.kind == hasher::POSEIDON2 && ctx->hasher_is_qp() && !uploaded_p2[dev] && merkle_mx_in_use()) {
// ... 46 lines not shown
    if (!ctx) return QPGPU_EINVAL;
    QP_DEV(ctx);
    if (ctx->hasher_in_use) return ctx->fail(QPGPU_EINVAL, "ctx_set_hasher: circuits or oracles already exist on this context; choose the hasher first");
    if (kind == hasher::POSEIDON) { ctx->hasher.kind = hasher::POSEIDON; return QPGPU_OK; }
    if (kind != hasher::POSEIDON2) return ctx->fail(QPGPU_EINVAL, "ctx_set_hasher: unknown hasher kind");
    poseidon2::Params p;
    if (parse_p2(params, n_words, p) != QPGPU_OK) return ctx->fail(QPGPU_EINVAL, "ctx_set_hasher: bad Poseidon2 parameter block");
    ctx->hasher.kind = hasher::POSEIDON2; ctx->hasher.p2 = p;
    if (ctx->d_p2) {
        QP_HIP(ctx, hipMemcpyAsync(ctx->d_p2, &ctx->hasher.p2, sizeof(poseidon2::Params), hipMemcpyHostToDevice, ctx->stream));
        QP_HIP(ctx, hipStreamSynchronize(ctx->stream));
    }
    return QPGPU_OK;
}
extern "C" int qpgpu_ctx_get_hasher(const qpgpu_ctx *ctx) { return ctx ? ctx->hasher.kind : QPGPU_EINVAL; }

int merkle_build(qpgpu_ctx *ctx, const MerkleLeafArgs &leaf, unsigned log_leaves, unsigned cap_height, uint64_t *d_digests) {
    int rc = merkle_ensure_constants(ctx);
    if (rc) return rc;
    if (cap_height > log_leaves) return ctx->fail(QPGPU_EINVAL, "merkle: cap_height exceeds tree height");
    const HasherDev hd = ctx->hasher_dev();
    const uint32_t nb = leaf.batch ? leaf.batch : 1;
    ctx->prof_begin("merkle_leaf_hash");
    hipError_t e = merkle_leaf_hash(leaf, hd, ctx->stream);
    ctx->prof_end();
    QP_HIP(ctx, e);
    ctx->prof_begin("merkle_nodes");
    e = merkle_reduce_to_cap(d_digests, 1ull << log_leaves, 1ull << cap_height, nb, leaf.ps_digests, hd, ctx->stream);
    ctx->prof_end();
    QP_HIP(ctx, e);
    return QPGPU_OK;
}

extern "C" {

size_t qpgpu_merkle_digest_count(unsigned log_leaves, unsigned cap_height) {
    if (cap_height > log_leaves) return 0;
    return (size_t)((2ull << log_leaves) - (1ull << cap_height));
}

int qpgpu_merkle_build_dev(qpgpu_ctx *ctx, const uint64_t *d_cols, uint64_t col_stride, uint32_t n_cols,
                           unsigned log_leaves, unsigned cap_height, uint64_t *d_digests, uint64_t *h_cap_out) {
    if (!ctx) return QPGPU_EINVAL;
    QP_DEV(ctx);
    if (!d_cols || !d_digests || n_cols == 0) return ctx->fail(QPGPU_EINVAL, "merkle: null buffer or no columns");
    if (log_leaves > 40) return ctx->fail(QPGPU_EINVAL, "merkle: log_leaves out of range");
    MerkleLeafArgs a{};
    a.src0 = d_cols; a.stride0 = col_stride; a.ncols0 = n_cols; a.src1 = nullptr; a.ncols1 = 0; a.stride1 = 0;
    a.n_leaves = 1ull << log_leaves; a.digests = d_digests; a.batch = 1;
    ctx->hasher_in_use = true;
    int rc = merkle_build(ctx, a, log_leaves, cap_height, d_digests);
    if (rc) return rc;
    if (h_cap_out) {
        size_t total = qpgpu_merkle_digest_count(log_leaves, cap_height), cap_n = (size_t)1 << cap_height;
        QP_HIP(ctx, hipMemcpyAsync(h_cap_out, d_digests + (total - cap_n) * 4, cap_n * 4 * sizeof(uint64_t), hipMemcpyDeviceToHost, ctx->stream));
        QP_HIP(ctx, hipStreamSynchronize(ctx->stream));
    }
    return QPGPU_OK;
}

int qpgpu_merkle_build_rows_dev(qpgpu_ctx *ctx, const uint64_t *d_rows, uint32_t width, unsigned log_leaves,
                                unsigned cap_height, uint64_t *d_digests, uint64_t *h_cap_out) {
    if (!ctx) return QPGPU_EINVAL;
    QP_DEV(ctx);
    if (!d_rows || !d_digests || width == 0) return ctx->fail(QPGPU_EINVAL, "merkle: null buffer or zero width");
    if (cap_height > log_leaves) return ctx->fail(QPGPU_EINVAL, "merkle: cap_height exceeds tree height");
    int rc = merkle_ensure_constants(ctx);
    if (rc) return rc;
    uint64_t cnt = 1ull << log_leaves;
    ctx->hasher_in_use = true;
    const HasherDev hd = ctx->hasher_dev();
    QP_HIP(ctx, merkle_leaf_hash_rows(d_rows, cnt, width, d_digests, 1, 0, 0, hd, ctx->stream));
    QP_HIP(ctx, merkle_reduce_to_cap(d_digests, cnt, 1ull << cap_height, 1, 0, hd, ctx->stream));
    uint64_t *lvl = d_digests;
    while (cnt > (1ull << cap_height)) { lvl += cnt * 4; cnt >>= 1; }
    if (h_cap_out) {
        size_t cap_n = (size_t)1 << cap_height;
        QP_HIP(ctx, hipMemcpyAsync(h_cap_out, lvl, cap_n * 4 * sizeof(uint64_t), hipMemcpyDeviceToHost, ctx->stream));
        QP_HIP(ctx, hipStreamSynchronize(ctx->stream));
    }
    return QPGPU_OK;
}

int qpgpu_poseidon2_hash_pad10_dev(qpgpu_ctx *ctx, const uint64_t *params, size_t n_words, const uint64_t *d_in, size_t len, size_t count, uint64_t *d_out) {
    if (!ctx) return QPGPU_EINVAL;
    QP_DEV(ctx);
    if ((!d_in && len && count) || (!d_out && count)) return ctx->fail(QPGPU_EINVAL, "poseidon2_hash_pad10: null buffer");
    if (len > (1u << 20)) return ctx->fail(QPGPU_EINVAL, "poseidon2_hash_pad10: preimage longer than 2^20 elements");
    if (!params && n_words == 0) {
        int rc = ctx->ensure_p2_app();
        if (rc) return rc;
        QP_HIP(ctx, poseidon2_hash_pad10_batch(d_in, len, count, d_out, ctx->d_p2_app, true, ctx->stream));
        return QPGPU_OK;
    }
    poseidon2::Params p;
    if (parse_p2(params, n_words, p) != QPGPU_OK) return ctx->fail(QPGPU_EINVAL, "poseidon2_hash_pad10: bad Poseidon2 parameter block");
    void *v = nullptr;
    QP_HIP(ctx, hipMalloc(&v, sizeof p));
    hipError_t e = hipMemcpyAsync(v, &p, sizeof p, hipMemcpyHostToDevice, ctx->stream);
    if (e == hipSuccess) e = poseidon2_hash_pad10_batch(d_in, len, count, d_out, (const poseidon2::Params *)v, false, ctx->stream);
    const hipError_t e2 = hipStreamSynchronize(ctx->stream);
    (void)hipFree(v);
    if (e != hipSuccess) return ctx->hip_fail(e, "poseidon2_hash_pad10");
    if (e2 != hipSuccess) return ctx->hip_fail(e2, "poseidon2_hash_pad10");
    return QPGPU_OK;
}

int qpgpu_poseidon_permute_dev(qpgpu_ctx *ctx, uint64_t *d_states, size_t n) {
    if (!ctx) return QPGPU_EINVAL;
    QP_DEV(ctx);
    if (!d_states && n) return ctx->fail(QPGPU_EINVAL, "poseidon: null buffer");
    int rc = merkle_ensure_constants(ctx);
    if (rc) return rc;
    ctx->hasher_in_use = true;
    QP_HIP(ctx, poseidon_permute_batch(d_states, n, ctx->hasher_dev(), ctx->stream));
    return QPGPU_OK;
}

}
```

### qp-zk-circuits_amd/csrc/merkle_kernels.hip

```cpp
#include <hip/hip_runtime.h>
#include <cstdlib>
#include "merkle.hpp"
#include "poseidon.hpp"
#include "prover_kernels.hpp"

using gl::u32;
using gl::u64;

__constant__ u64 c_poseidon_rc[poseidon::ROUNDS * poseidon::WIDTH];

hipError_t merkle_tp_upload_constants(const u64 *rc360);
hipError_t merkle_tp_leaves(const MerkleLeafArgs &a, u64 total, const HasherDev &h, hipStream_t st);
hipError_t merkle_tp_rows(const u64 *rows, u64 n_leaves, u32 width, u64 *digests, u32 batch, u64 ps_rows, u64 ps_digests, const HasherDev &h, hipStream_t st);
hipError_t merkle_tp_nodes(const u64 *in, u64 *out, u64 n_out, u32 batch, u64 ps, const HasherDev &h, hipStream_t st);
hipError_t merkle_tp_pow(const PowArgs &a, dim3 g, const HasherDev &h, hipStream_t st);
hipError_t verify_upload_constants(const u64 *rc360);
hipError_t verify_head_upload_constants(const u64 *rc360);
hipError_t fri_verify_upload_constants(const u64 *rc360);
hipError_t merkle_mx_upload_constants(const u64 *rc360);
hipError_t merkle_mx_leaves(const MerkleLeafArgs &a, u64 total, const HasherDev &h, hipStream_t st);
hipError_t merkle_mx_nodes(const u64 *in, u64 *out, u64 n_out, u32 batch, u64 ps, const HasherDev &h, hipStream_t st);
hipError_t merkle_mx_pow(const PowArgs &a, const HasherDev &h, hipStream_t st);
static bool mx_serves(const HasherDev &h) { return h.kind != hasher::POSEIDON2 || h.qp; }

uint64_t qpgpu_tp_min_threads() {
    static const uint64_t v = [] { const char *e = getenv("QPGPU_TP_MIN_THREADS"); return e && *e ? strtoull(e, nullptr, 10) : (uint64_t)1 << 18; }();
    return v;
}

static bool mx_enabled() {
    static const bool v = [] { const char *e = getenv("QPGPU_MX"); return !(e && *e == '0'); }();
    return v;
}
static u64 coop_max_init() {
    const char *e = getenv("QPGPU_COOP_MAX");
    if (e && *e) { const long long v = atoll(e); if (v >= 0) return (u64)v; }
    return 16384;
}
static const u64 COOP_MAX = coop_max_init();
static u32 tput_batch() {
    static const u32 v = [] { const char *e = getenv("QPGPU_TPUT_BATCH"); return e && *e ? (u32)strtoul(e, nullptr, 10) : 8u; }();
    return v;
}
static inline bool tput(u32 batch) { return batch >= tput_batch(); }
static inline u64 coop_max_for(u32 batch) { return tput(batch) ? 0 : COOP_MAX; }
static inline u64 tp_min_for(u32 batch) { return tput(batch) ? 0 : qpgpu_tp_min_threads(); }

bool merkle_mx_in_use() { return mx_enabled(); }
hipError_t merkle_upload_constants(const u64 *rc360) {
    hipError_t e = hipMemcpyToSymbol(HIP_SYMBOL(c_poseidon_rc), rc360, sizeof(u64) * poseidon::ROUNDS * poseidon::WIDTH);
    if (e == hipSuccess) e = merkle_tp_upload_constants(rc360);
    if (e == hipSuccess) e = verify_upload_constants(rc360);
    if (e == hipSuccess) e = verify_head_upload_constants(rc360);
    if (e == hipSuccess) e = fri_verify_upload_constants(rc360);
    if (e != hipSuccess || !mx_enabled()) return e;
    return merkle_mx_upload_constants(rc360);
}

#include "merkle_hash_impl.hpp"

namespace {

__device__ __forceinline__ u64 coop_permute(u64 s, const int g, const int lane_base) {
    constexpr u32 C[12] = {17, 15, 41, 16, 2, 28, 13, 13, 39, 18, 34, 20};
    int src[12];
#pragma unroll
    for (int i = 0; i < 12; i++) { int e = g + i; e -= e >= 12 ? 12 : 0; src[i] = lane_base + (g < 12 ? e : i); }
#pragma unroll 1
    for (int r = 0; r < poseidon::ROUNDS; r++) {
        const u64 rc = g < 12 ? c_poseidon_rc[r * 12 + g] : 0;
        s = gl::add(s, rc);
        const bool full = r < poseidon::HALF_FULL || r >= poseidon::HALF_FULL + poseidon::PARTIAL;
        const u64 sb = poseidon::sbox7(s);
        s = (full || g == 0) ? sb : s;
        const u32 lo = (u32)s, hi = (u32)(s >> 32);
        u64 al = 0, ah = 0;
#pragma unroll
        for (int i = 0; i < 12; i++) {
            const u32 l = (u32)__shfl((int)lo, src[i], 64), h = (u32)__shfl((int)hi, src[i], 64);
            al += (u64)l * C[i];
            ah += (u64)h * C[i];
        }
        if (g == 0) { al += (u64)lo * 8u; ah += (u64)hi * 8u; }
        const u64 low = al + (ah << 32);
        const u32 top = (u32)(ah >> 32) + (low < al ? 1u : 0u);
        s = gl::reduce96(low, top);
    }
    return gl::canon(s);
}

__global__ void __launch_bounds__(256) node_coop_kernel(const u64 *in, u64 *out, u64 n_out, u32 batch, u64 ps) {
    const u64 ggrp = (blockIdx.x * (u64)blockDim.x + threadIdx.x) >> 4;
    const int lane = threadIdx.x & 63, g = lane & 15, base = lane & 48;
    const bool live = ggrp < n_out * batch;
    const u64 pr = live ? ggrp >> ilog2_64(n_out) : 0, grp = ggrp & (n_out - 1);
    in += pr * ps; out += pr * ps;
    u64 s = (live && g < 8) ? in[grp * 8 + g] : 0;
    s = coop_permute(s, g, base);
    if (live && g < 4) out[grp * 4 + g] = s;
}

template <int MAXM>
__global__ void __launch_bounds__(MAXM >= 512 ? 512 : 256) tree_top_kernel(u64 *levels, u64 cnt, u32 m, u64 ps) {
// ... 60 lines not shown
        return c < a.ncols0 ? a.src0[(u64)c * a.stride0 + j] : a.src1[(u64)(c - a.ncols0) * a.stride1 + j];
    };
    if (W <= 4) {
        if (live && g < 4) a.digests[j * 4 + g] = g < (int)W ? gl::canon(elem(g)) : 0;
        return;
    }
    u64 s = 0;
    for (u32 c = 0; c < W; c += 8) {
        if (g < 8 && c + g < W) s = elem(c + g);
        s = coop_permute(s, g, base);
    }
    if (live && g < 4) a.digests[j * 4 + g] = s;
}

template <bool QP>
__global__ void __launch_bounds__(256) p2_pad10_sponge_kernel(const u64 *in, u64 len, u64 count, u64 *out, const poseidon2::Params *p2) {
    const u64 i = blockIdx.x * (u64)blockDim.x + threadIdx.x;
    if (i >= count) return;
    const u64 *src = in + i * len;
    u64 s[12];
#pragma unroll
    for (int k = 0; k < 12; k++) s[k] = 0;
    for (u64 c = 0; c <= len; c += 8) {
#pragma unroll
        for (int k = 0; k < 8; k++) {
            const u64 idx = c + k;
            const u64 v = idx < len ? gl::canon(src[idx]) : (idx == len ? 1 : 0);
            s[k] = gl::add_canonical(s[k], v);
        }
        if constexpr (QP) poseidon2::permute_qp(s, *p2); else poseidon2::permute(s, *p2);
    }
#pragma unroll
    for (int k = 0; k < 4; k++) out[i * 4 + k] = s[k];
}

template <class Perm>
__global__ void permute_kernel(u64 *states, u64 n, const poseidon2::Params *p2) {
    const u64 i = blockIdx.x * (u64)blockDim.x + threadIdx.x;
    if (i >= n) return;
    u64 s[12];
#pragma unroll
    for (int k = 0; k < 12; k++) s[k] = gl::canon(states[i * 12 + k]);
    Perm::permute(s, p2);
#pragma unroll
    for (int k = 0; k < 12; k++) states[i * 12 + k] = s[k];
}

}

hipError_t pk_pow(const PowArgs &a, const HasherDev &h, hipStream_t st) {
    if (a.count == 0 || a.batch == 0) return hipSuccess;
    const u64 chunks = (a.count + 255) / 256;
    if (chunks * a.batch > 0x7FFFFFFFull) return hipErrorInvalidValue;
    dim3 g((unsigned)(chunks * a.batch));
    if (chunks * a.batch * 256 < tp_min_for(a.batch)) return hash_launch_pow(a, g, h, st);
    return (mx_serves(h) && mx_enabled()) ? merkle_mx_pow(a, h, st) : merkle_tp_pow(a, g, h, st);
}

hipError_t merkle_leaf_hash(const MerkleLeafArgs &a0, const HasherDev &h, hipStream_t st) {
    MerkleLeafArgs a = a0;
    if (a.batch == 0) a.batch = 1;
    if (a.n_leaves == 0) return hipSuccess;
    if (a.n_leaves & (a.n_leaves - 1)) return hipErrorInvalidValue;
    const u64 total = a.n_leaves * a.batch;
    const bool p2 = h.kind == hasher::POSEIDON2;
    if (!p2 && total <= coop_max_for(a.batch) / 2) {
        dim3 block(256), grid((unsigned)((total * 16 + 255) / 256));
        hipLaunchKernelGGL(leaf_cols_coop_kernel, grid, block, 0, st, a);
        return hipGetLastError();
    }
    if (total < tp_min_for(a.batch)) return hash_launch_leaves(a, total, h, st);
    return (mx_serves(h) && a.ncols0 + a.ncols1 > 4 && mx_enabled()) ? merkle_mx_leaves(a, total, h, st) : merkle_tp_leaves(a, total, h, st);
}
hipError_t merkle_leaf_hash_rows(const u64 *rows, u64 n_leaves, u32 width, u64 *digests, u32 batch, u64 ps_rows, u64 ps_digests, const HasherDev &h, hipStream_t st) {
    if (n_leaves == 0 || batch == 0) return hipSuccess;
    if (n_leaves & (n_leaves - 1)) return hipErrorInvalidValue;
    const u64 total = n_leaves * batch;
    const bool p2 = h.kind == hasher::POSEIDON2;
    if (!p2 && total <= coop_max_for(batch)) {
        dim3 block(256), grid((unsigned)((total * 16 + 255) / 256));
        hipLaunchKernelGGL(leaf_rows_coop_kernel, grid, block, 0, st, rows, n_leaves, width, digests, batch, ps_rows, ps_digests);
        return hipGetLastError();
    }
    return total >= tp_min_for(batch) ? merkle_tp_rows(rows, n_leaves, width, digests, batch, ps_rows, ps_digests, h, st)
                                           : hash_launch_rows(rows, n_leaves, width, digests, batch, ps_rows, ps_digests, h, st);
}
static hipError_t merkle_reduce_level(const u64 *in, u64 *out, u64 n_out, u32 batch, u64 ps, const HasherDev &h, hipStream_t st) {
    if (n_out == 0) return hipSuccess;
    const u64 total = n_out * batch;
    const bool p2 = h.kind == hasher::POSEIDON2;
    if (!p2 && total <= coop_max_for(batch)) {
        dim3 block(256), grid((unsigned)((total * 16 + 255) / 256));
        hipLaunchKernelGGL(node_coop_kernel, grid, block, 0, st, in, out, n_out, batch, ps);
        return hipGetLastError();
    }
    if (total < tp_min_for(batch)) return hash_launch_nodes(in, out, n_out, batch, ps, h, st);
    return (mx_serves(h) && mx_enabled()) ? merkle_mx_nodes(in, out, n_out, batch, ps, h, st) : merkle_tp_nodes(in, out, n_out, batch, ps, h, st);
}
hipError_t merkle_reduce_to_cap(u64 *levels, u64 cnt, u64 cap_n, u32 batch, u64 ps, const HasherDev &h, hipStream_t st) {
    if (batch == 0) return hipSuccess;
    if ((cnt & (cnt - 1)) || (cap_n & (cap_n - 1))) return hipErrorInvalidValue;
    u64 *lvl = levels;
    while (cnt > cap_n) {
        const u64 m = cnt / cap_n;
        static const u32 top_m = [] { const char *e = getenv("QPGPU_TREE_TOP"); const int v = e ? atoi(e) : 32; return (u32)(v < 0 ? 0 : v > 512 ? 512 : v); }();
        if (top_m >= 2 && !tput(batch) && h.kind != hasher::POSEIDON2 && m <= top_m && cap_n <= 65535 && batch <= 65535) {
            if (m <= 32) hipLaunchKernelGGL((tree_top_kernel<32>), dim3((unsigned)cap_n, batch), dim3(256), 0, st, lvl, cnt, (u32)m, ps);
            else if (m <= 256) hipLaunchKernelGGL((tree_top_kernel<256>), dim3((unsigned)cap_n, batch), dim3(256), 0, st, lvl, cnt, (u32)m, ps);
            else hipLaunchKernelGGL((tree_top_kernel<512>), dim3((unsigned)cap_n, batch), dim3(512), 0, st, lvl, cnt, (u32)m, ps);
            return hipGetLastError();
        }
        hipError_t e = merkle_reduce_level(lvl, lvl + cnt * 4, cnt / 2, batch, ps, h, st);
        if (e != hipSuccess) return e;
        lvl += cnt * 4; cnt >>= 1;
    }
    return hipSuccess;
}
hipError_t poseidon2_hash_pad10_batch(const u64 *in, u64 len, u64 count, u64 *out, const poseidon2::Params *p2, bool qp_set, hipStream_t st) {
    if (count == 0) return hipSuccess;
    const dim3 grid((unsigned)((count + 255) / 256)), block(256);
    if (qp_set) hipLaunchKernelGGL((p2_pad10_sponge_kernel<true>), grid, block, 0, st, in, len, count, out, p2);
    else hipLaunchKernelGGL((p2_pad10_sponge_kernel<false>), grid, block, 0, st, in, len, count, out, p2);
    return hipGetLastError();
}
hipError_t poseidon_permute_batch(u64 *states, u64 n, const HasherDev &h, hipStream_t st) {
    if (n == 0) return hipSuccess;
    dim3 block(256), grid((unsigned)((n + 255) / 256));
    if (h.kind == hasher::POSEIDON2) hipLaunchKernelGGL((permute_kernel<Poseidon2P>), grid, block, 0, st, states, n, h.p2);
    else hipLaunchKernelGGL((permute_kernel<PoseidonV1>), grid, block, 0, st, states, n, h.p2);
    return hipGetLastError();
}
```

### qp-zk-circuits_amd/csrc/merkle_kernels_mx.hip

```cpp
#define POSEIDON_GROUPED_SBOX 1
#include <hip/hip_runtime.h>
#include <vector>
#include "merkle.hpp"
#include "poseidon_mfma.hpp"
#include "prover_kernels.hpp"

using gl::u32;
using gl::u64;

namespace mx {
constexpr int WG = 512;
__constant__ u64 c_poseidon_rc[poseidon::ROUNDS * poseidon::WIDTH];
__device__ uint4 g_table[pmf::TABLE_BYTES / 16];
__device__ uint4 g_table_p2[pmf::TABLE_BYTES / 16];

#define MX_KERNEL __global__ void __launch_bounds__(WG) __attribute__((amdgpu_waves_per_eu(4, 4)))

struct PoseidonV1 {
    static __device__ __forceinline__ const uint4 *table() { return g_table; }
    static __device__ __forceinline__ void body(u64 (&s)[12], const poseidon2::Params *, const unsigned char *lds) {
        pmf::permute_head(s, c_poseidon_rc, lds);
        pmf::permute_tail_rounds(s, c_poseidon_rc);
    }
    template <int FIRST, int COUNT, bool CANON>
    static __device__ __forceinline__ void last_rows(u64 (&s)[12]) { pmf::last_layer_rows<FIRST, COUNT, CANON>(s); }
    static __device__ __forceinline__ void own_copy(u64 (&s)[12]) {
#pragma unroll
        for (int i = 0; i < 12; i++) asm volatile("" : "+v"(s[i]));
    }
};
struct Poseidon2QP {
    static __device__ __forceinline__ const uint4 *table() { return g_table_p2; }
    static __device__ __forceinline__ void body(u64 (&s)[12], const poseidon2::Params *p2, const unsigned char *lds) { pmf::permute_p2qp(s, *p2, lds); }
    template <int FIRST, int COUNT, bool CANON>
    static __device__ __forceinline__ void last_rows(u64 (&)[12]) {}
    static __device__ __forceinline__ void own_copy(u64 (&)[12]) {}
};
template <class Perm, int FIRST, int COUNT, bool CANON>
__device__ __forceinline__ void permute_rows(u64 (&s)[12], const poseidon2::Params *p2, const unsigned char *lds) {
    Perm::body(s, p2, lds);
    Perm::template last_rows<FIRST, COUNT, CANON>(s);
}
template <class Perm>
__device__ __forceinline__ const unsigned char *table_to_lds() {
    extern __shared__ uint4 mx_lds[];
    const uint4 *t = Perm::table();
    for (int i = threadIdx.x; i < pmf::TABLE_BYTES / 16; i += WG) mx_lds[i] = t[i];
    __syncthreads();
    return (const unsigned char *)mx_lds;
}
__device__ __forceinline__ u32 ilog2_64(u64 x) { return 63u - (u32)__clzll((long long)x); }

template <class Perm>
MX_KERNEL leaf_hash_kernel(MerkleLeafArgs a, const poseidon2::Params *p2) {
    const unsigned char *lds = table_to_lds<Perm>();
    const u64 total = a.n_leaves * a.batch;
    u64 gj = blockIdx.x * (u64)WG + threadIdx.x;
    const bool live = gj < total;
    gj = live ? gj : total - 1;
    const u64 pr = gj >> ilog2_64(a.n_leaves), j = gj & (a.n_leaves - 1);
    a.src0 += pr * a.ps_src0; a.src1 += pr * a.ps_src1; a.digests += pr * a.ps_digests;
    const u32 W = a.ncols0 + a.ncols1;
    auto elem = [&](u32 c) -> u64 {
        return c < a.ncols0 ? a.src0[(u64)c * a.stride0 + j] : a.src1[(u64)(c - a.ncols0) * a.stride1 + j];
    };
    u64 s[12];
#pragma unroll
    for (int i = 0; i < 12; i++) s[i] = 0;
    for (u32 c = 0; c < W; c += 8) {
#pragma unroll
        for (int i = 0; i < 8; i++)
            if (c + i < W) s[i] = elem(c + i);
        Perm::body(s, p2, lds);
        const u32 rest = W - c;
        if (rest <= 8) { Perm::own_copy(s); Perm::template last_rows<0, 4, true>(s); }
        else if (rest >= 16) { Perm::own_copy(s); Perm::template last_rows<8, 4, false>(s); }
        else { Perm::own_copy(s); Perm::template last_rows<0, 12, false>(s); }
    }
    if (live) {
        u64 *out = a.digests + j * 4;
#pragma unroll
        for (int i = 0; i < 4; i++) out[i] = s[i];
    }
}

template <class Perm>
MX_KERNEL node_kernel(const u64 *in, u64 *out, u64 n_out, u32 batch, u64 ps, u32 per_thread, const poseidon2::Params *p2) {
    const unsigned char *lds = table_to_lds<Perm>();
    const u64 total = n_out * batch;
    const u32 sh = ilog2_64(n_out);
    for (u32 k = 0; k < per_thread; k++) {
        u64 gi = ((u64)blockIdx.x * per_thread + k) * WG + threadIdx.x;
        const bool live = gi < total;
        gi = live ? gi : total - 1;
        const u64 pr = gi >> sh, i = gi & (n_out - 1);
        const ulonglong2 *p = reinterpret_cast<const ulonglong2 *>(in + pr * ps + i * 8);
        const ulonglong2 a = p[0], b = p[1], c = p[2], d = p[3];
        u64 s[12];
        s[0] = a.x; s[1] = a.y; s[2] = b.x; s[3] = b.y; s[4] = c.x; s[5] = c.y; s[6] = d.x; s[7] = d.y;
        s[8] = s[9] = s[10] = s[11] = 0;
        permute_rows<Perm, 0, 4, true>(s, p2, lds);
        if (live) {
            ulonglong2 *o = reinterpret_cast<ulonglong2 *>(out + pr * ps + i * 4);
            o[0] = make_ulonglong2(s[0], s[1]);
            o[1] = make_ulonglong2(s[2], s[3]);
        }
    }
}

template <class Perm>
MX_KERNEL pow_kernel(PowArgs a, const poseidon2::Params *p2) {
    const u32 chunk = blockIdx.x / a.batch, pr = (blockIdx.x % a.batch + chunk) % a.batch;
    const u64 first = (u64)chunk * WG;
    if (first >= a.count) return;
    const u64 base = a.bases[pr];
    if (base == ~0ull) return;
    __shared__ u32 s_leave;
    if (threadIdx.x == 0) s_leave = __hip_atomic_load(&a.results[pr], __ATOMIC_RELAXED, __HIP_MEMORY_SCOPE_AGENT) < base + first ? 1u : 0u;
    __syncthreads();
    if (s_leave) return;
    const unsigned char *lds = table_to_lds<Perm>();
    const u64 idx = first + threadIdx.x, nonce = base + idx;
    const u64 *st = a.states + 12 * (u64)pr;
    u64 s[12];
#pragma unroll
    for (int i = 0; i < 12; i++) s[i] = (i == (int)a.pos) ? nonce : st[i];
    permute_rows<Perm, 7, 1, true>(s, p2, lds);
    if (idx < a.count && (s[7] >> (64 - a.pow_bits)) == 0) atomicMin((unsigned long long *)&a.results[pr], (unsigned long long)nonce);
}

template <class Perm>
MX_KERNEL selftest_kernel(u64 *states, const poseidon2::Params *p2) {
    const unsigned char *lds = table_to_lds<Perm>();
    const u64 t = blockIdx.x * (u64)WG + threadIdx.x;
    u64 s[12];
#pragma unroll
    for (int i = 0; i < 12; i++) s[i] = states[t * 12 + i];
    permute_rows<Perm, 0, 12, true>(s, p2, lds);
#pragma unroll
    for (int i = 0; i < 12; i++) states[t * 12 + i] = s[i];
}
}

template <class Perm>
static hipError_t allow_table_in_lds() {
    hipError_t e = hipFuncSetAttribute((const void *)mx::leaf_hash_kernel<Perm>, hipFuncAttributeMaxDynamicSharedMemorySize, pmf::TABLE_BYTES);
    if (e == hipSuccess) e = hipFuncSetAttribute((const void *)mx::node_kernel<Perm>, hipFuncAttributeMaxDynamicSharedMemorySize, pmf::TABLE_BYTES);
    if (e == hipSuccess) e = hipFuncSetAttribute((const void *)mx::pow_kernel<Perm>, hipFuncAttributeMaxDynamicSharedMemorySize, pmf::TABLE_BYTES);
    return e;
}
template <class Perm, class HostPerm>
static hipError_t device_selftest(HostPerm host_perm, const poseidon2::Params *host_p2) {
    constexpr int N = 4 * mx::WG;
    std::vector<u64> in((size_t)N * 12), out((size_t)N * 12);
    u64 seed = 0x9E3779B97F4A7C15ull;
    for (int t = 0; t < N; t++)
        for (int i = 0; i < 12; i++) {
            seed = seed * 6364136223846793005ull + 1442695040888963407ull;
            u64 v = (seed ^ (seed >> 31)) % gl::P;
            if (t % 9 == 0) v = (i & 1) ? gl::P - 1 - (v & 3) : (v & 7);
            in[(size_t)t * 12 + i] = v;
        }
    u64 *d = nullptr; poseidon2::Params *dp = nullptr; hipStream_t st = nullptr;
    hipError_t e = hipMalloc((void **)&d, in.size() * 8);
    if (e == hipSuccess && host_p2) { e = hipMalloc((void **)&dp, sizeof *host_p2); if (e == hipSuccess) e = hipMemcpy(dp, host_p2, sizeof *host_p2, hipMemcpyHostToDevice); }
    if (e == hipSuccess) e = hipMemcpy(d, in.data(), in.size() * 8, hipMemcpyHostToDevice);
    if (e == hipSuccess) e = hipStreamCreateWithFlags(&st, hipStreamNonBlocking);
    if (e == hipSuccess) e = hipFuncSetAttribute((const void *)mx::selftest_kernel<Perm>, hipFuncAttributeMaxDynamicSharedMemorySize, pmf::TABLE_BYTES);
    if (e == hipSuccess) {
        hipLaunchKernelGGL(mx::selftest_kernel<Perm>, dim3(N / mx::WG), dim3(mx::WG), pmf::TABLE_BYTES, st, d, dp);
        e = hipGetLastError();
        if (e == hipSuccess) e = hipStreamSynchronize(st);
    }
    if (e == hipSuccess) e = hipMemcpy(out.data(), d, out.size() * 8, hipMemcpyDeviceToHost);
    if (e == hipSuccess)
        for (int t = 0; t < N && e == hipSuccess; t++) {
            u64 s[12];
            for (int i = 0; i < 12; i++) s[i] = in[(size_t)t * 12 + i];
            host_perm(s);
            for (int i = 0; i < 12; i++) if (s[i] != out[(size_t)t * 12 + i]) e = hipErrorAssert;
        }
    constexpr u64 NL = 1ull << 19, NN = NL / 2, POW_COUNT = 1ull << 18;
    constexpr u32 WCOLS = 17, POW_BITS = 11, POW_BATCH = 2;
    u64 *d_cols = nullptr, *d_dig = nullptr, *d_pow = nullptr;
    std::vector<u64> cols((size_t)WCOLS * NL), dig(4 * (NL + NN)), powbuf(12 * POW_BATCH + 2 * POW_BATCH);
    if (e == hipSuccess) {
        for (size_t i = 0; i < cols.size(); i++) { seed = seed * 6364136223846793005ull + 1442695040888963407ull; cols[i] = (seed ^ (seed >> 29)) % gl::P; }
        for (u32 b = 0; b < POW_BATCH; b++) {
            for (int i = 0; i < 12; i++) { seed = seed * 6364136223846793005ull + 1442695040888963407ull; powbuf[12 * b + i] = (seed ^ (seed >> 29)) % gl::P; }
            powbuf[12 * POW_BATCH + b] = 1000 * (b + 1);
            powbuf[12 * POW_BATCH + POW_BATCH + b] = ~0ull;
        }
        e = hipMalloc((void **)&d_cols, cols.size() * 8);
        if (e == hipSuccess) e = hipMalloc((void **)&d_dig, dig.size() * 8);
        if (e == hipSuccess) e = hipMalloc((void **)&d_pow, powbuf.size() * 8);
        if (e == hipSuccess) e = hipMemcpy(d_cols, cols.data(), cols.size() * 8, hipMemcpyHostToDevice);
        if (e == hipSuccess) e = hipMemcpy(d_pow, powbuf.data(), powbuf.size() * 8, hipMemcpyHostToDevice);
    }
    if (e == hipSuccess) {
        MerkleLeafArgs la{};
        la.src0 = d_cols; la.stride0 = NL; la.ncols0 = WCOLS; la.n_leaves = NL; la.digests = d_dig; la.batch = 1;
        hipLaunchKernelGGL(mx::leaf_hash_kernel<Perm>, dim3((unsigned)(NL / mx::WG)), dim3(mx::WG), pmf::TABLE_BYTES, st, la, dp);
        hipLaunchKernelGGL(mx::node_kernel<Perm>, dim3((unsigned)(NN / mx::WG)), dim3(mx::WG), pmf::TABLE_BYTES, st, d_dig, d_dig + 4 * NL, NN, 1u, (u64)0, 1u, dp);
        PowArgs pa{};
        pa.states = d_pow; pa.bases = d_pow + 12 * POW_BATCH; pa.results = d_pow + 12 * POW_BATCH + POW_BATCH;
        pa.pos = 3; pa.pow_bits = POW_BITS; pa.batch = POW_BATCH; pa.count = POW_COUNT;
        hipLaunchKernelGGL(mx::pow_kernel<Perm>, dim3((unsigned)(POW_COUNT / mx::WG * POW_BATCH)), dim3(mx::WG), pmf::TABLE_BYTES, st, pa, dp);
        e = hipGetLastError();
        if (e == hipSuccess) e = hipStreamSynchronize(st);
        if (e == hipSuccess) e = hipMemcpy(dig.data(), d_dig, dig.size() * 8, hipMemcpyDeviceToHost);
        if (e == hipSuccess) e = hipMemcpy(powbuf.data(), d_pow, powbuf.size() * 8, hipMemcpyDeviceToHost);
    }
    if (e == hipSuccess) {
        for (u64 w = 0; w < NL / 64 && e == hipSuccess; w++) {
            const u64 j = w * 64 + (w * 7) % 64;
            u64 s[12] = {0};
            for (u32 c = 0; c < WCOLS; c += 8) {
                for (u32 i = 0; i < 8 && c + i < WCOLS; i++) s[i] = cols[(size_t)(c + i) * NL + j];
                host_perm(s);
            }
            for (int i = 0; i < 4; i++) if (s[i] != dig[4 * j + i]) e = hipErrorAssert;
        }
        for (u64 w = 0; w < NN / 64 && e == hipSuccess; w++) {
            const u64 i0 = w * 64 + (w * 11) % 64;
            u64 s[12] = {0};
            for (int i = 0; i < 8; i++) s[i] = dig[8 * i0 + i];
            host_perm(s);
            for (int i = 0; i < 4; i++) if (s[i] != dig[4 * NL + 4 * i0 + i]) e = hipErrorAssert;
        }
        for (u32 b = 0; b < POW_BATCH && e == hipSuccess; b++) {
            const u64 base = 1000 * (b + 1), got = powbuf[12 * POW_BATCH + POW_BATCH + b];
            u64 want = ~0ull;
            for (u64 k = 0; k < POW_COUNT && want == ~0ull; k++) {
                u64 s[12];
                for (int i = 0; i < 12; i++) s[i] = i == 3 ? base + k : powbuf[12 * b + i];
                host_perm(s);
                if ((s[7] >> (64 - POW_BITS)) == 0) want = base + k;
            }
            if (got != want) e = hipErrorAssert;
        }
    }
    if (d_cols) (void)hipFree(d_cols);
    if (d_dig) (void)hipFree(d_dig);
    if (d_pow) (void)hipFree(d_pow);
    if (st) (void)hipStreamDestroy(st);
    if (d) (void)hipFree(d);
    if (dp) (void)hipFree(dp);
    return e;
}
hipError_t merkle_mx_upload_constants(const u64 *rc360) {
    std::vector<unsigned char> tab(pmf::TABLE_BYTES);
    if (!pmf::build_tables(rc360, tab.data()) || !pmf::host_selfcheck(rc360, tab.data(), 64)) return hipErrorInvalidValue;
    hipError_t e = hipMemcpyToSymbol(HIP_SYMBOL(mx::c_poseidon_rc), rc360, sizeof(u64) * poseidon::ROUNDS * poseidon::WIDTH);
    if (e != hipSuccess) return e;
    e = hipMemcpyToSymbol(HIP_SYMBOL(mx::g_table), tab.data(), pmf::TABLE_BYTES);
    if (e == hipSuccess) e = allow_table_in_lds<mx::PoseidonV1>();
    return e != hipSuccess ? e : device_selftest<mx::PoseidonV1>([&](u64 (&s)[12]) { poseidon::permute(s, rc360); }, nullptr);
}
hipError_t merkle_upload_p2_tables(const poseidon2::Params &qp) {
    std::vector<unsigned char> tab(pmf::TABLE_BYTES);
    if (!pmf::build_tables_p2(qp, tab.data()) || !pmf::host_selfcheck_p2(qp, tab.data(), 64)) return hipErrorInvalidValue;
    hipError_t e = hipMemcpyToSymbol(HIP_SYMBOL(mx::g_table_p2), tab.data(), pmf::TABLE_BYTES);
    if (e == hipSuccess) e = allow_table_in_lds<mx::Poseidon2QP>();
    return e != hipSuccess ? e : device_selftest<mx::Poseidon2QP>([&](u64 (&s)[12]) { poseidon2::permute(s, qp); }, &qp);
}
hipError_t merkle_mx_leaves(const MerkleLeafArgs &a, u64 total, const HasherDev &h, hipStream_t st) {
    const u64 blocks = (total + mx::WG - 1) / mx::WG;
    if (blocks > 0x7FFFFFFFull) return hipErrorInvalidValue;
    if (h.kind == hasher::POSEIDON2) hipLaunchKernelGGL(mx::leaf_hash_kernel<mx::Poseidon2QP>, dim3((unsigned)blocks), dim3(mx::WG), pmf::TABLE_BYTES, st, a, h.p2);
    else hipLaunchKernelGGL(mx::leaf_hash_kernel<mx::PoseidonV1>, dim3((unsigned)blocks), dim3(mx::WG), pmf::TABLE_BYTES, st, a, h.p2);
    return hipGetLastError();
}
hipError_t merkle_mx_nodes(const u64 *in, u64 *out, u64 n_out, u32 batch, u64 ps, const HasherDev &h, hipStream_t st) {
    const u64 total = n_out * batch;
    u64 per_thread = total >> 18;
    per_thread = per_thread < 1 ? 1 : per_thread > 8 ? 8 : per_thread;
    const u64 blocks = (total + mx::WG * per_thread - 1) / (mx::WG * per_thread);
    if (blocks > 0x7FFFFFFFull) return hipErrorInvalidValue;
    if (h.kind == hasher::POSEIDON2) hipLaunchKernelGGL(mx::node_kernel<mx::Poseidon2QP>, dim3((unsigned)blocks), dim3(mx::WG), pmf::TABLE_BYTES, st, in, out, n_out, batch, ps, (u32)per_thread, h.p2);
    else hipLaunchKernelGGL(mx::node_kernel<mx::PoseidonV1>, dim3((unsigned)blocks), dim3(mx::WG), pmf::TABLE_BYTES, st, in, out, n_out, batch, ps, (u32)per_thread, h.p2);
    return hipGetLastError();
}
hipError_t merkle_mx_pow(const PowArgs &a, const HasherDev &h, hipStream_t st) {
    const u64 chunks = (a.count + mx::WG - 1) / mx::WG;
    if (chunks * a.batch > 0x7FFFFFFFull) return hipErrorInvalidValue;
    if (h.kind == hasher::POSEIDON2) hipLaunchKernelGGL(mx::pow_kernel<mx::Poseidon2QP>, dim3((unsigned)(chunks * a.batch)), dim3(mx::WG), pmf::TABLE_BYTES, st, a, h.p2);
    else hipLaunchKernelGGL(mx::pow_kernel<mx::PoseidonV1>, dim3((unsigned)(chunks * a.batch)), dim3(mx::WG), pmf::TABLE_BYTES, st, a, h.p2);
    return hipGetLastError();
}
```

### qp-zk-circuits_amd/csrc/poseidon.hpp

```cpp
#pragma once
#include <stddef.h>
#include "gl64.hpp"

namespace poseidon {
using gl::u32;
using gl::u64;

constexpr int WIDTH = 12, RATE = 8, HALF_FULL = 4, PARTIAL = 22, ROUNDS = 30;

GL_HD u64 sbox7(u64 x) {
    u64 x2 = gl::sqr(x), x4 = gl::sqr(x2), x3 = gl::mul(x, x2);
    return gl::mul(x3, x4);
}
#if defined(__HIP_DEVICE_COMPILE__) && defined(POSEIDON_GROUPED_SBOX)
template <int N>
__device__ __forceinline__ void sbox7_layer(u64 (&x)[N]) {
    u64 x2[N], x3[N], x4[N];
    gl::mul_group(x2, x, x);
    gl::mul_group(x4, x2, x2);
    gl::mul_group(x3, x, x2);
    gl::mul_group(x, x3, x4);
}
__device__ __forceinline__ u64 sbox7_lane(u64 x) {
    u64 a[1] = {x}, x2[1];
// ... 153 lines not shown
    }
}
GL_HD void spectrum_times_circulant(Spectrum &s) {
    const i64 T = s.U1[0] + s.U1[1] + s.U1[2];
    const i64 A0 = T + s.U1[2], A1 = T + s.U1[0], A2 = T + s.U1[1];
    const i64 B0 = shl(s.Um[2], 3) - s.Um[0] - shl(s.Um[1], 1);
    const i64 B1 = -(shl(s.Um[0], 3) + s.Um[1] + shl(s.Um[2], 1));
    const i64 B2 = shl(s.Um[0], 1) - shl(s.Um[1], 3) - s.Um[2];
    const i64 f0 = s.F[0], f1 = s.F[1], f2 = s.F[2], h0 = s.H[0], h1 = s.H[1], h2 = s.H[2];
    const i64 R0 = shl(f0, 1) - h0 + f1 - shl(h1, 4) + f2 + shl(h2, 2);
    const i64 R1 = -shl(f0, 2) + h0 + shl(f1, 1) - h1 + f2 - shl(h2, 4);
    const i64 R2 = shl(f0, 4) + h0 - shl(f1, 2) + h1 + shl(f2, 1) - h2;
    const i64 I0 = f0 + shl(h0, 1) + shl(f1, 4) + h1 - shl(f2, 2) + h2;
    const i64 I1 = -f0 - shl(h0, 2) + f1 + shl(h1, 1) + shl(f2, 4) + h2;
    const i64 I2 = -f0 + shl(h0, 4) - f1 - shl(h1, 2) + f2 + shl(h2, 1);
    s.U1[0] = shl(A0, 6); s.U1[1] = shl(A1, 6); s.U1[2] = shl(A2, 6);
    s.Um[0] = shl(B0, 2); s.Um[1] = shl(B1, 2); s.Um[2] = shl(B2, 2);
    s.F[0] = shl(R0, 1); s.F[1] = shl(R1, 1); s.F[2] = shl(R2, 1);
    s.H[0] = shl(I0, 1); s.H[1] = shl(I1, 1); s.H[2] = shl(I2, 1);
}
GL_HD i64 spectrum_lane0(const Spectrum &s) { return (s.U1[0] + s.Um[0] + shl(s.F[0], 1)) >> 2; }
GL_HD void vector_of(const Spectrum &s, i64 (&x)[WIDTH]) {
#pragma unroll
    for (int b = 0; b < 3; b++) {
        const i64 p = s.U1[b] + s.Um[b], q = s.U1[b] - s.Um[b], f2 = shl(s.F[b], 1), h2 = shl(s.H[b], 1);
        x[b] = (p + f2) >> 2; x[b + 6] = (p - f2) >> 2; x[b + 3] = (q + h2) >> 2; x[b + 9] = (q - h2) >> 2;
    }
}
GL_HD u64 join_halves(i64 lo, i64 hi) {
    const u64 al = (u64)lo, ah = (u64)hi;
    const u64 low = al + (ah << 32);
    const u32 top = (u32)(ah >> 32) + (low < al ? 1u : 0u);
    return gl::reduce96(low, top);
}
GL_HD void renormalize_pair(i64 &lo, i64 &hi) {
    const i64 k = (lo >> 32) & ~(i64)3;
    lo -= shl(k, 32); hi += k;
    const i64 m = (hi >> 32) & ~(i64)3;
    hi -= shl(m, 32); hi += m; lo -= m;
}
GL_HD void renormalize(Spectrum &sl, Spectrum &sh) {
#pragma unroll
    for (int b = 0; b < 3; b++) {
        renormalize_pair(sl.U1[b], sh.U1[b]); renormalize_pair(sl.Um[b], sh.Um[b]);
        renormalize_pair(sl.F[b], sh.F[b]); renormalize_pair(sl.H[b], sh.H[b]);
    }
}
GL_HD u64 join_signed_halves(i64 lo, i64 hi) { return join_halves(lo + (((i64)1 << 60) + ((i64)1 << 28)), hi + (((i64)1 << 60) - ((i64)1 << 29))); }

GL_HD void partial_rounds_spectral(u64 (&s)[WIDTH], const u64 *rc0) {
    i64 lo[WIDTH], hi[WIDTH];
#pragma unroll
    for (int i = 0; i < WIDTH; i++) { lo[i] = (i64)(u32)s[i]; hi[i] = (i64)(s[i] >> 32); }
    Spectrum sl, sh;
    spectrum_of(lo, sl); spectrum_of(hi, sh);
    i64 x_lo = lo[0], x_hi = hi[0];
    i64 d_lo = 0, d_hi = 0;
    u64 x0 = s[0];
#pragma unroll 1
    for (int k0 = 0; k0 < PARTIAL; k0 += 3) {
#pragma unroll
        for (int kk = 0; kk < 3; kk++) {
            const int k = k0 + kk;
            if (k < PARTIAL) {
                if (k) x0 = join_signed_halves(x_lo + d_lo, x_hi + d_hi);
                const u64 y = sbox7_lane(gl::add_canonical(x0, rc0[k * WIDTH]));
                const i64 y_lo = (i64)(u32)y, y_hi = (i64)(y >> 32);
                const i64 in_lo = y_lo - x_lo, in_hi = y_hi - x_hi;
                sl.U1[0] += in_lo; sl.Um[0] += in_lo; sl.F[0] += in_lo;
                sh.U1[0] += in_hi; sh.Um[0] += in_hi; sh.F[0] += in_hi;
                spectrum_times_circulant(sl); spectrum_times_circulant(sh);
                d_lo = shl(y_lo, 3); d_hi = shl(y_hi, 3);
                if (kk == 2 && k + 1 < PARTIAL) renormalize(sl, sh);
                x_lo = spectrum_lane0(sl); x_hi = spectrum_lane0(sh);
            }
        }
    }
    vector_of(sl, lo); vector_of(sh, hi);
    lo[0] += d_lo; hi[0] += d_hi;
#pragma unroll
    for (int i = 0; i < WIDTH; i++) s[i] = join_signed_halves(lo[i], hi[i]);
}

GL_HD void permute(u64 (&s)[WIDTH], const u64 *rc) {
    int r = 0;
    for (int k = 0; k < HALF_FULL; k++, r++) {
#pragma unroll
        for (int i = 0; i < WIDTH; i++) s[i] = gl::add_canonical(s[i], rc[r * WIDTH + i]);
        sbox7_layer(s);
        mds_layer(s);
    }
#pragma unroll
    for (int i = 1; i < WIDTH; i++) s[i] = gl::add_canonical(s[i], rc[r * WIDTH + i]);
    partial_rounds_spectral(s, rc + r * WIDTH);
    r += PARTIAL;
    for (int k = 0; k < HALF_FULL; k++, r++) {
#pragma unroll
        for (int i = 0; i < WIDTH; i++) s[i] = gl::add_canonical(s[i], rc[r * WIDTH + i]);
        sbox7_layer(s);
        mds_layer(s);
    }
#pragma unroll
    for (int i = 0; i < WIDTH; i++) s[i] = gl::canon(s[i]);
}
GL_HD void permute_layerwise(u64 (&s)[WIDTH], const u64 *rc) {
    int r = 0;
    for (int k = 0; k < HALF_FULL; k++, r++) {
#pragma unroll
        for (int i = 0; i < WIDTH; i++) s[i] = sbox7(gl::add_canonical(s[i], rc[r * WIDTH + i]));
        mds_layer(s);
    }
#pragma unroll
    for (int i = 1; i < WIDTH; i++) s[i] = gl::add_canonical(s[i], rc[r * WIDTH + i]);
    for (int k = 0; k < PARTIAL; k++, r++) {
        s[0] = sbox7(gl::add_canonical(s[0], rc[r * WIDTH]));
        mds_layer(s);
    }
    for (int k = 0; k < HALF_FULL; k++, r++) {
#pragma unroll
        for (int i = 0; i < WIDTH; i++) s[i] = sbox7(gl::add_canonical(s[i], rc[r * WIDTH + i]));
        mds_layer(s);
    }
#pragma unroll
    for (int i = 0; i < WIDTH; i++) s[i] = gl::canon(s[i]);
}
GL_HD void permute_textbook(u64 (&s)[WIDTH], const u64 *rc) {
    int r = 0;
    for (int k = 0; k < ROUNDS; k++, r++) {
        const bool full = k < HALF_FULL || k >= HALF_FULL + PARTIAL;
        for (int i = 0; i < WIDTH; i++) s[i] = gl::add_canonical(s[i], rc[r * WIDTH + i]);
        for (int i = 0; i < (full ? WIDTH : 1); i++) s[i] = sbox7(s[i]);
        mds_layer_naive(s);
    }
    for (int i = 0; i < WIDTH; i++) s[i] = gl::canon(s[i]);
}

constexpr int FP_FIRST = 0, FP_RC = 12, FP_VS = 34, FP_WHATS = FP_VS + 22 * 11, FP_INIT = FP_WHATS + 22 * 11, FP_WORDS = FP_INIT + 121;
constexpr u64 MDS_00 = 25;

GL_HD void fast_partial_enter(u64 (&s)[WIDTH], const u64 *fp) {
#pragma unroll
    for (int i = 0; i < WIDTH; i++) s[i] = gl::add(s[i], fp[FP_FIRST + i]);
    u64 t[11];
    for (int c = 0; c < 11; c++) {
        u64 acc = 0;
        for (int r = 0; r < 11; r++) acc = gl::add(acc, gl::mul(fp[FP_INIT + c * 11 + r], s[1 + r]));
        t[c] = acc;
    }
    for (int c = 0; c < 11; c++) s[1 + c] = t[c];
}
GL_HD void fast_partial_linear(u64 (&s)[WIDTH], const u64 *fp, int r) {
    const u64 s0 = gl::add(s[0], fp[FP_RC + r]);
    u64 d = gl::mul(s0, MDS_00);
    for (int i = 0; i < 11; i++) d = gl::add(d, gl::mul(fp[FP_WHATS + r * 11 + i], s[1 + i]));
    for (int i = 0; i < 11; i++) s[1 + i] = gl::add(s[1 + i], gl::mul(s0, fp[FP_VS + r * 11 + i]));
    s[0] = d;
}
const u64 *host_fast_partial();

void derive_round_constants(u64 *out360);
const u64 *host_round_constants();
const u64 *host_hash_round_constants();

}

namespace poseidon2 {
using gl::u64;
struct Params {
    u64 rc_ext[8 * 12];
    u64 rc_int[22];
    u64 diag_m1[12];
    u64 m4[16];
};
constexpr int PARAM_WORDS = 96 + 22 + 12 + 16;
const Params &qp_params();

GL_HD void ext_layer(u64 (&s)[12], const Params &p) {
    u64 t[12];
#pragma unroll
    for (int b = 0; b < 3; b++)
#pragma unroll
        for (int i = 0; i < 4; i++) {
            u64 acc = 0;
#pragma unroll
            for (int j = 0; j < 4; j++) acc = gl::add(acc, gl::mul(p.m4[4 * i + j], s[4 * b + j]));
            t[4 * b + i] = acc;
// ... 98 lines not shown
```

### qp-zk-circuits_amd/csrc/poseidon_mfma.hpp

```cpp
#pragma once
#include <string.h>
#include <utility>
#include "poseidon.hpp"

namespace pmf {
using gl::u32;
using gl::u64;
#if defined(__HIPCC__)
typedef int v4i __attribute__((ext_vector_type(4)));
typedef int v16i __attribute__((ext_vector_type(16)));
#endif

constexpr int LIMBS = 8, N_GROUP = 6, N_FIN = 3, FIN_STEPS = 9, N_ELEM = 36;
constexpr int group_steps(int g) { return 3 + g; }
constexpr int group_base(int g) { int b = 0; for (int i = 0; i < g; i++) b += group_steps(i); return b; }
constexpr int N_GROUP_TILES = group_base(N_GROUP);
constexpr int N_TILES = N_GROUP_TILES + N_FIN * FIN_STEPS;
constexpr int CINIT_OFF = N_TILES * 1024;
constexpr int G_OFF = CINIT_OFF + (N_GROUP + N_FIN) * 128;
constexpr int TABLE_BYTES = G_OFF + 32;
static_assert(N_GROUP_TILES == 33 && TABLE_BYTES % 16 == 0, "table layout");
constexpr u64 DIGIT_BIAS = 0x8080808080808080ull;

constexpr u64 mds_entry(int r, int j) {
// ... 380 lines not shown
    for (int i = 0; i < 4; i++) {
        const v4i c = cp[i];
        a0[4 * i] = c[0]; a0[4 * i + 1] = c[1]; a0[4 * i + 2] = c[2]; a0[4 * i + 3] = c[3];
    }
    a1 = a0;
    const v4i *ap = (const v4i *)(st.lds + (size_t)tile0 * 1024) + lane;
#pragma unroll
    for (int q = 0; q < STEPS; q++) {
        const v4i a = ap[q * 64];
        a0 = __builtin_amdgcn_mfma_i32_32x32x32_i8(a, st.B0[q], a0, 0, 0, 0);
        a1 = __builtin_amdgcn_mfma_i32_32x32x32_i8(a, st.B1[q], a1, 0, 0, 0);
    }
#ifndef PMF_NO_KEEPALIVE
    asm volatile("" : "+v"(a0), "+v"(a1));
#endif
#pragma unroll
    for (int i = 0; i < 16; i++) {
        u32 x = (u32)a0[i], yv = (u32)a1[i];
        swap32(x, yv);
        Z[i >> 3][i & 7] = x; Z[2 + (i >> 3)][i & 7] = yv;
    }
}
struct SboxOfInput { __device__ __forceinline__ u64 operator()(int, u64 x) const { return poseidon::sbox7_lane(x); } };
template <int G, bool SMALL_G, class F>
__device__ __forceinline__ void group_step(Run &st, F &f) {
    u32 Z[4][LIMBS];
    gemm<group_steps(G)>(st, group_base(G), G, Z);
    constexpr int n = 4 * G + 4 <= 22 ? 4 : 22 - 4 * G;
#pragma unroll
    for (int o = 0; o < n; o++) {
        const int k = 4 * G + o;
        u64 x;
        if constexpr (SMALL_G) {
            constexpr u32 Gc[3] = {G0, G1, G2};
            u64 lo, yy[MAX_GROUP_TERMS] = {};
            u32 top, gg[MAX_GROUP_TERMS] = {};
            recombine_wide(Z[o], lo, top);
#pragma unroll
            for (int i = 0; i < o; i++) { yy[i] = st.y[4 * G + i]; gg[i] = Gc[o - 1 - i]; }
            x = reduce96_terms(lo, top, yy, gg, o);
        } else {
            x = recombine(Z[o]);
#pragma unroll
            for (int j = 4 * G; j < k; j++) x = gl::add(x, gl::mul(st.y[j], st.Gd[k - 1 - j]));
        }
        st.y[k] = f(k, x);
    }
#pragma unroll
    for (int o = 0; o < n; o++) {
        const u64 t = to_digits(st.y[4 * G + o]);
        st.Dlo[12 + 4 * G + o] = (u32)t; st.Dhi[12 + 4 * G + o] = (u32)(t >> 32);
    }
    form_step(st, 3 + G);
}
template <bool SMALL_G, class F, int... G>
__device__ __forceinline__ void all_groups(Run &st, F &f, std::integer_sequence<int, G...>) { (group_step<G, SMALL_G>(st, f), ...); }

template <bool SMALL_G, class F>
__device__ __forceinline__ void partial_rounds(u64 (&s)[12], const unsigned char *lds, F &f) {
    Run st;
    st.lds = lds;
    if (!SMALL_G) {
#pragma unroll
        for (int d = 0; d < 3; d++) {
            const u64 g = *(const u64 *)(lds + G_OFF + 8 * d);
            st.Gd[d] = ((u64)(u32)__builtin_amdgcn_readfirstlane((int)(g >> 32)) << 32) | (u32)__builtin_amdgcn_readfirstlane((int)(u32)g);
        }
    }
#pragma unroll
    for (int e = 0; e < N_ELEM; e++) {
        const u64 t = e < 12 ? to_digits(s[e]) : 0;
        st.Dlo[e] = (u32)t; st.Dhi[e] = (u32)(t >> 32);
    }
    form_step(st, 0); form_step(st, 1); form_step(st, 2);
    all_groups<SMALL_G>(st, f, std::make_integer_sequence<int, N_GROUP>{});
#pragma unroll
    for (int f = 0; f < N_FIN; f++) {
        u32 Z[4][LIMBS];
        gemm<FIN_STEPS>(st, N_GROUP_TILES + f * FIN_STEPS, N_GROUP + f, Z);
#pragma unroll
        for (int o = 0; o < 4; o++) s[4 * f + o] = recombine(Z[o]);
    }
}
__device__ __forceinline__ void permute_head(u64 (&s)[12], const u64 *rc, const unsigned char *lds) {
    using namespace poseidon;
#pragma unroll
    for (int i = 0; i < WIDTH; i++) s[i] = gl::add_canonical(s[i], rc[i]);
    for (int k = 0; k < HALF_FULL; k++) {
        sbox7_layer(s);
        if (k + 1 < HALF_FULL) mds_layer_words_rc(s, rc + (k + 1) * WIDTH);
    }
    SboxOfInput f;
    partial_rounds<true>(s, lds, f);
}
__device__ __forceinline__ void permute_tail_rounds(u64 (&s)[12], const u64 *rc) {
    using namespace poseidon;
    int r = HALF_FULL + 1 + PARTIAL;
    for (int k = 1; k < HALF_FULL; k++, r++) {
        sbox7_layer(s);
        mds_layer_words_rc(s, rc + r * WIDTH);
    }
    sbox7_layer(s);
}
template <int FIRST, int COUNT, bool CANON>
__device__ __forceinline__ void last_layer_rows(u64 (&s)[12]) {
    poseidon::mds_layer_rows_words<FIRST, COUNT>(s);
    if (CANON) {
#pragma unroll
        for (int i = FIRST; i < FIRST + COUNT; i++) s[i] = gl::canon(s[i]);
    }
}
template <int FIRST, int COUNT, bool CANON>
__device__ __forceinline__ void permute_tail_rows(u64 (&s)[12], const u64 *rc) {
    permute_tail_rounds(s, rc);
    last_layer_rows<FIRST, COUNT, CANON>(s);
}
__device__ __forceinline__ void permute_tail(u64 (&s)[12], const u64 *rc) { permute_tail_rows<0, 12, true>(s, rc); }
__device__ __forceinline__ void permute(u64 (&s)[12], const u64 *rc, const unsigned char *lds) {
    permute_head(s, rc, lds);
    permute_tail(s, rc);
}
__device__ __forceinline__ void permute_p2qp(u64 (&s)[12], const poseidon2::Params &p, const unsigned char *lds) {
    poseidon2::ext_layer_qp(s);
    for (int r = 0; r < 4; r++) {
#pragma unroll
        for (int i = 0; i < 12; i++) s[i] = gl::add_canonical(s[i], p.rc_ext[r * 12 + i]);
        poseidon::sbox7_layer(s);
        if (r < 3) poseidon2::ext_layer_qp(s);
    }
    SboxOfInput f;
    partial_rounds<false>(s, lds, f);
    poseidon::sbox7_layer(s);
    poseidon2::ext_layer_qp(s);
    for (int r = 5; r < 8; r++) {
#pragma unroll
        for (int i = 0; i < 12; i++) s[i] = gl::add_canonical(s[i], p.rc_ext[r * 12 + i]);
        poseidon::sbox7_layer(s);
        poseidon2::ext_layer_qp(s);
    }
#pragma unroll
    for (int i = 0; i < 12; i++) s[i] = gl::canon(s[i]);
}
#elif defined(__HIPCC__)
__device__ void permute(u64 (&s)[12], const u64 *rc, const unsigned char *lds);
__device__ void permute_head(u64 (&s)[12], const u64 *rc, const unsigned char *lds);
__device__ void permute_tail(u64 (&s)[12], const u64 *rc);
__device__ void permute_tail_rounds(u64 (&s)[12], const u64 *rc);
template <int FIRST, int COUNT, bool CANON> __device__ void last_layer_rows(u64 (&)[12]) {}
template <int FIRST, int COUNT, bool CANON> __device__ void permute_tail_rows(u64 (&)[12], const u64 *) {}
__device__ void permute_p2qp(u64 (&s)[12], const poseidon2::Params &p, const unsigned char *lds);
template <bool SMALL_G, class F> __device__ void partial_rounds(u64 (&)[12], const unsigned char *, F &) {}
#endif

}
```

### qp-zk-circuits_amd/csrc/prover_host.hpp

```cpp
#pragma once
#include <hip/hip_runtime_api.h>
#include <cstring>
#include <vector>
#include "challenger.hpp"
#include "ctx.hpp"
#include "gl64.hpp"
#include "poseidon.hpp"
#include "proof_layout.hpp"

struct ByteWriter {
    uint8_t *p; size_t cap, len = 0; bool overflow = false;
    void u64le(gl::u64 v) { if (len + 8 > cap) { overflow = true; len += 8; return; } std::memcpy(p + len, &v, 8); len += 8; }
    void u8(uint8_t v) { if (len + 1 > cap) { overflow = true; len += 1; return; } p[len++] = v; }
    void vec(const gl::u64 *v, size_t n) { for (size_t i = 0; i < n; i++) u64le(v[i]); }
    void ext(gl::e2 v) { u64le(v.a); u64le(v.b); }
};

struct OracleShards;
struct PolyOracle {
    uint32_t ncols = 0;
    unsigned log_n = 0, rate_bits = 0, cap_h = 0;
    gl::u64 *coeffs = nullptr, *lde = nullptr, *digests = nullptr;
    gl::u64 *salt = nullptr;
    uint32_t nb = 1;
    gl::u64 ps_coeffs = 0, ps_lde = 0, ps_digests = 0, ps_salt = 0;
    uint32_t oracle_index = 0;
    std::vector<gl::u64> cap;
    const OracleShards *sh = nullptr;
    bool blinded = false;
    bool salted() const { return salt || blinded; }
    gl::u64 lde_n() const { return 1ull << (log_n + rate_bits); }
    unsigned log_lde() const { return log_n + rate_bits; }
    size_t cap_words() const { return (size_t)4 << cap_h; }
    const gl::u64 *cap_of(uint32_t b) const { return cap.data() + (size_t)(nb == 1 ? 0 : b) * cap_words(); }
    void set_batch(uint32_t n_proofs, bool shared = false);
};

inline size_t digest_words(unsigned log_leaves, unsigned cap_h) { return ((2ull << log_leaves) - (1ull << cap_h)) * 4; }

inline void PolyOracle::set_batch(uint32_t n_proofs, bool shared) {
    nb = shared ? 1 : n_proofs;
    if (shared) { ps_coeffs = ps_lde = ps_digests = ps_salt = 0; return; }
    ps_coeffs = (gl::u64)ncols << log_n; ps_lde = (gl::u64)ncols << log_lde();
    ps_digests = digest_words(log_lde(), cap_h); ps_salt = (gl::u64)4 << log_lde();
}

struct Stager {
    gl::u64 *h = nullptr;
    size_t words = 0, pos = 0;
    int put(qpgpu_ctx *ctx, void *dst, const void *src, size_t bytes);
    int put_rows(qpgpu_ctx *ctx, gl::u64 *dst, size_t dst_pitch, const gl::u64 *src, size_t src_pitch, size_t row_words, size_t rows);
};

struct FriParams {
    unsigned degree_bits = 0, rate_bits = 0, cap_h = 0, pow_bits = 0;
    uint32_t num_queries = 0;
    std::vector<unsigned> arity_bits;
};
struct FriRange { uint32_t oracle, first, count; };
struct FriBatch { std::vector<gl::e2> points; std::vector<FriRange> ranges; };

struct FriWork {
    gl::u64 ws = 0;
    uint32_t nb_cap = 0;
    gl::u64 *comp = nullptr, *fin = nullptr, *vals = nullptr, *coeffs[2] = {nullptr, nullptr};
    std::vector<gl::u64 *> digests, leafrows;
    gl::u64 *gather = nullptr;
    gl::e2 *alpha_ext = nullptr;
    size_t gather_words = 0, max_batch_polys = 0;
    proof_layout::Fri proof;
    gl::e2 *t_points = nullptr, *t_shifts = nullptr, *t_betas = nullptr;
    gl::u64 *pow_states = nullptr, *pow_bases = nullptr, *pow_results = nullptr, *qidx = nullptr;
    static size_t words(const FriParams &p, const std::vector<size_t> &leaf_widths, size_t max_batch_polys, uint32_t nb);
    void bind(gl::u64 *base, const FriParams &p, const std::vector<size_t> &leaf_widths, size_t max_batch_polys, uint32_t nb);
    static size_t stage_words(const FriParams &p, size_t max_batch_polys, uint32_t nb) {
        return (size_t)nb * (2 * max_batch_polys + p.num_queries + 2 * 2 * 4 + 2 * (p.arity_bits.size() + 1) + 14 + 8) + 64;
    }
};

int oracle_commit_coeffs(qpgpu_ctx *ctx, PolyOracle &o, const uint32_t *d_keys);
int oracle_commit_values(qpgpu_ctx *ctx, const gl::u64 *d_values, PolyOracle &o, const uint32_t *d_keys);
int oracle_sharded_open(const PolyOracle &o, const gl::u64 *indices, size_t n, gl::u64 *rows_out, gl::u64 *paths_out);

int fri_prove(qpgpu_ctx *ctx, const FriParams &p, const PolyOracle *const *oracles, size_t n_oracles,
              const std::vector<FriBatch> &batches, uint32_t nb, Challenger *chs, FriWork &w, Stager &stage, ByteWriter *outs);
size_t fri_proof_bytes(const FriParams &p, const std::vector<size_t> &leaf_widths);

int salt_key_random(uint32_t key[8]);
void salt_key_from_seed(uint64_t seed, uint32_t key[8]);

#define QP_TRY(expr) do { int _rc = (expr); if (_rc) return _rc; } while (0)
```

### qp-zk-circuits_amd/csrc/prover_kernels.hpp

```cpp
#pragma once
#include <hip/hip_runtime_api.h>
#include <stdint.h>
#include "circuit.hpp"
#include "gl64.hpp"
#include "quotient_kernels.hpp"

struct PpArgs {
    const uint64_t *wires;
    const uint64_t *sigmas;
    const uint64_t *omega_pows;
    const uint64_t *beta_k_is;
    const uint64_t *betas, *gammas;
    uint64_t *qcp;
    uint64_t *rowprod;
    uint64_t n;
    uint32_t num_routed, chunk, nchunks, nch;
    uint32_t batch;
    uint64_t ps_wires, ps_small, ps_qcp, ps_rowprod;
};

struct ReduceArgs {
    const uint64_t *src[8];
    uint64_t ps_src[8];
    uint32_t ncols[8];
    uint32_t nsrc;
    const gl::e2 *alpha_pows;
    uint64_t *comp_a, *comp_b;
    uint64_t n;
    uint32_t batch;
    uint64_t ps_alpha, ps_comp;
};

struct PowArgs {
    const uint64_t *states;
    const uint64_t *bases;
    uint64_t *results;
    uint32_t pos, pow_bits, batch;
    uint64_t count;
};

hipError_t pk_pp_rows(const PpArgs &a, hipStream_t st);
hipError_t pk_pp_scan(const uint64_t *rowprod, uint64_t *z, uint64_t n, uint32_t nch_total, hipStream_t st);
hipError_t pk_pp_finish(const PpArgs &a, const uint64_t *z, uint64_t *zs_pp, uint64_t ps_z, uint64_t ps_zs, hipStream_t st);
hipError_t pk_scale_powers(uint64_t *data, uint64_t n, uint64_t ncols, const uint64_t *pw_lo, const uint64_t *pw_hi, uint32_t lo_bits, hipStream_t st);
hipError_t pk_poly_eval(const uint64_t *coeffs, uint64_t n, uint32_t npolys, const gl::e2 *points, uint32_t npoints, gl::e2 *out,
                        uint32_t batch, uint64_t ps_coeffs, uint64_t ps_points, uint64_t ps_out, hipStream_t st);
hipError_t pk_reduce_polys(const ReduceArgs &a, hipStream_t st);
hipError_t pk_divide_linear(const uint64_t *comp_a, const uint64_t *comp_b, uint64_t n, const gl::e2 *zs, const gl::e2 *shifts, int mode,
                            uint64_t *fin_a, uint64_t *fin_b, uint32_t batch, uint64_t ps_comp, uint64_t ps_fin, hipStream_t st);
hipError_t pk_copy(void *dst, const void *src, size_t bytes, hipStream_t st);
hipError_t pk_unpack_rows(const uint64_t *src, uint64_t pitch_words, uint64_t width_words, uint64_t rows, uint64_t *dst, hipStream_t st);
hipError_t pk_pack_rows(const uint64_t *src, uint64_t pitch_words, uint64_t width_words, uint64_t rows, uint64_t *dst, hipStream_t st);
hipError_t pk_interleave_ext(const uint64_t *va, const uint64_t *vb, uint64_t n, uint64_t *rows, uint32_t batch, uint64_t ps_vals, uint64_t ps_rows, hipStream_t st);
hipError_t pk_fri_fold(const uint64_t *ca, const uint64_t *cb, uint64_t new_n, uint32_t arity, const gl::e2 *betas, uint64_t *oa, uint64_t *ob,
                       uint32_t batch, uint64_t ps_in, uint64_t ps_out, hipStream_t st);
struct HasherDev;
hipError_t pk_pow(const PowArgs &a, const HasherDev &h, hipStream_t st);
hipError_t pk_gather_rows(const uint64_t *cols, uint64_t stride, uint32_t ncols, const uint64_t *idx, uint32_t nq, uint64_t *out,
                          uint32_t batch, uint64_t ps_cols, uint64_t ps_out, hipStream_t st);
hipError_t pk_gather_paths(const uint64_t *digests, uint64_t n_leaves, uint32_t path_len, const uint64_t *idx, uint32_t shift, uint32_t nq, uint64_t *out,
                           uint32_t batch, uint64_t ps_digests, uint64_t ps_out, hipStream_t st);
hipError_t pk_gather_leaf_rows(const uint64_t *rows, uint32_t width, const uint64_t *idx, uint32_t shift, uint32_t nq, uint64_t *out,
                               uint32_t batch, uint64_t ps_rows, uint64_t ps_out, hipStream_t st);
hipError_t pk_salt(const uint32_t *keys, uint32_t oracle_index, uint64_t lde_n, uint64_t *out, uint32_t batch, hipStream_t st);
hipError_t pk_salt_slice(const uint32_t *key, uint32_t oracle_index, uint64_t first_leaf, uint64_t count, uint64_t *out, hipStream_t st);
hipError_t pk_random_felts(const uint32_t *keys, uint64_t count, uint64_t *out, uint64_t pitch, uint32_t batch, hipStream_t st);
hipError_t pk_coset_tables(uint64_t lde_n, uint32_t log_lde, uint64_t shift, const uint64_t *pw_lo, const uint64_t *pw_hi, uint32_t lo_bits, const uint64_t *zh,
                           uint32_t rate, uint64_t n_field, uint64_t *x_coset, uint64_t *l0_coset, hipStream_t st);
```

Measured before the change: 1718.

## Precompute Poseidon PoW first round on host and add MFMA row-leaf hashing

For proof-of-work grinding with Poseidon v1, the first full round's contribution from all fixed state words is precomputed on the host into a head table. The kernel then only applies the sbox to the nonce lane and a linear combination, and starts the permutation from round 1. Separately, wide-row Merkle leaf hashing above the tensor-path threshold now goes through a new MFMA row kernel. New API entry points and self-tests are added. This cuts per-nonce work in grinding and speeds leaf hashing, at the cost of extra scratch space and more code paths.

```diff
diff --git a/include/qpgpu.h b/include/qpgpu.h
--- a/include/qpgpu.h
+++ b/include/qpgpu.h
@@ -74,6 +74,8 @@
                            unsigned log_leaves, unsigned cap_height, uint64_t *d_digests, uint64_t *h_cap_out);
 int qpgpu_merkle_build_rows_dev(qpgpu_ctx *ctx, const uint64_t *d_rows, uint32_t width, unsigned log_leaves,
                                 unsigned cap_height, uint64_t *d_digests, uint64_t *h_cap_out);
+int qpgpu_merkle_leaf_hash_rows_dev(qpgpu_ctx *ctx, const uint64_t *d_rows, uint32_t width, unsigned log_leaves, uint32_t batch,
+                                    uint64_t ps_rows, uint64_t ps_digests, uint64_t *d_digests);
 
 int qpgpu_circuit_load(qpgpu_ctx *ctx, const uint64_t *pack_words, size_t n_words, qpgpu_circuit **out);
 int qpgpu_circuit_load_batch(qpgpu_ctx *ctx, const uint64_t *pack_words, size_t n_words, unsigned max_batch, qpgpu_circuit **out);
@@ -182,6 +184,8 @@
                           const uint64_t *alphas, qpgpu_fri_session **out);
 uint32_t qpgpu_fri_session_batch(const qpgpu_fri_session *s);
 int qpgpu_fri_grind_batch(qpgpu_ctx *ctx, const qpgpu_challenger *cs, uint32_t batch, unsigned proof_of_work_bits, uint64_t *nonces_out);
+int qpgpu_pow_search(qpgpu_ctx *ctx, const uint64_t *states, uint32_t batch, uint32_t pos, unsigned proof_of_work_bits,
+                     const uint64_t *bases, uint64_t count, uint64_t *results_out);
 
 typedef struct qpgpu_stage_plan qpgpu_stage_plan;
 #define QPGPU_STAGE_ERR_CAP 256
diff --git a/qp-zk-circuits_amd/__init__.py b/qp-zk-circuits_amd/__init__.py
--- a/qp-zk-circuits_amd/__init__.py
+++ b/qp-zk-circuits_amd/__init__.py
@@ -2,7 +2,7 @@
 from .binding import StagePlan, stage_header_words
 from .binding import FriSession, fri_grind
 from .binding import FriVerifier
-from .binding import fri_prove_batch, fri_grind_batch
+from .binding import fri_prove_batch, fri_grind_batch, pow_search
 from .binding import PolyOracle, Challenger, fri_prove, set_hasher_poseidon, set_hasher_poseidon2, ProvingPool
 from .binding import pack_header, pack_public_input_cells, Verifier, poseidon2_qp_params, synth_p2_sites
 from .binding import pack_p2_layout, pack_trailers, p2_site_cells, P2_NO_SWAP
diff --git a/qp-zk-circuits_amd/binding.py b/qp-zk-circuits_amd/binding.py
--- a/qp-zk-circuits_amd/binding.py
+++ b/qp-zk-circuits_amd/binding.py
@@ -96,6 +96,7 @@
         "qpgpu_merkle_digest_count": (c.c_size_t, [c.c_uint, c.c_uint]),
         "qpgpu_merkle_build_dev": (c.c_int, [vp, u64p, c.c_uint64, c.c_uint32, c.c_uint, c.c_uint, u64p, u64p]),
         "qpgpu_merkle_build_rows_dev": (c.c_int, [vp, u64p, c.c_uint32, c.c_uint, c.c_uint, u64p, u64p]),
+        "qpgpu_merkle_leaf_hash_rows_dev": (c.c_int, [vp, u64p, c.c_uint32, c.c_uint, c.c_uint32, c.c_uint64, c.c_uint64, u64p]),
         "qpgpu_circuit_load": (c.c_int, [vp, u64p, c.c_size_t, c.POINTER(vp)]),
         "qpgpu_circuit_load_batch": (c.c_int, [vp, u64p, c.c_size_t, c.c_uint, c.POINTER(vp)]),
         "qpgpu_circuit_max_batch": (c.c_uint, [vp]),
@@ -197,6 +198,7 @@
         "qpgpu_fri_begin_batch": (c.c_int, [vp, c.POINTER(vp), c.c_uint32, vp, c.c_uint32, u64p, c.c_uint32, vp, u64p, c.POINTER(vp)]),
         "qpgpu_fri_session_batch": (c.c_uint32, [vp]),
         "qpgpu_fri_grind_batch": (c.c_int, [vp, vp, c.c_uint32, c.c_uint, c.POINTER(c.c_uint64)]),
+        "qpgpu_pow_search": (c.c_int, [vp, u64p, c.c_uint32, c.c_uint32, c.c_uint, u64p, c.c_uint64, u64p]),
         "qpgpu_field_probe": (c.c_int, [vp, c.c_uint, c.c_uint, u64p, u64p, c.c_size_t, u64p, c.c_size_t, c.c_int]),
         "qpgpu_synth_pack_words": (c.c_size_t, [c.c_uint, c.c_uint, c.c_uint]),
         "qpgpu_synth_pack_words_ex": (c.c_size_t, [c.c_uint, c.c_uint, c.c_uint, c.c_uint]),
@@ -1044,6 +1046,15 @@
     nonces = (ctypes.c_uint64 * nb)()
     gpu._check(gpu.lib.qpgpu_fri_grind_batch(gpu.ctx, ctypes.byref(states), nb, proof_of_work_bits, nonces))
     return [int(x) for x in nonces]
+
+
+def pow_search(gpu, states, pos, proof_of_work_bits, bases, count):
+    st = np.ascontiguousarray(states, dtype=np.uint64).reshape(-1, 12)
+    bs = np.ascontiguousarray(bases, dtype=np.uint64)
+    out = np.empty(st.shape[0], dtype=np.uint64)
+    gpu._check(gpu.lib.qpgpu_pow_search(gpu.ctx, st.ctypes.data, st.shape[0], pos, proof_of_work_bits, bs.ctypes.data, count,
+                                        out.ctypes.data))
+    return out
 
 
 def fri_grind(gpu, challenger, proof_of_work_bits):
@@ -1451,6 +1462,10 @@
                                                          _ptr(d_digests), cap.ctypes.data))
         return cap
 
+    def merkle_leaf_hash_rows_dev(self, d_rows, width, log_leaves, batch, ps_rows, ps_digests, d_digests):
+        self._check(self.lib.qpgpu_merkle_leaf_hash_rows_dev(self.ctx, _ptr(d_rows), width, log_leaves, batch, ps_rows, ps_digests,
+                                                             _ptr(d_digests)))
+
 
 class QpGpu(_Stage3):
 
diff --git a/qp-zk-circuits_amd/csrc/fri_api.cpp b/qp-zk-circuits_amd/csrc/fri_api.cpp
--- a/qp-zk-circuits_amd/csrc/fri_api.cpp
+++ b/qp-zk-circuits_amd/csrc/fri_api.cpp
@@ -304,13 +304,31 @@
     if (proof_of_work_bits == 0) { for (uint32_t b = 0; b < nb; b++) nonces_out[b] = 0; return QPGPU_OK; }
     ctx->hasher_in_use = true;
     QP_TRY(merkle_ensure_constants(ctx));
-    QP_TRY(ctx->ensure_scratch((size_t)nb * 16 * 8));
+    QP_TRY(ctx->ensure_scratch((size_t)nb * (16 + poseidon::POW_HEAD_WORDS) * 8));
     Stager bounce;
     std::vector<u64> nonces(nb, 0);
     u64 *t = ctx->scratch;
-    QP_TRY(fri_grind(ctx, chs.data(), nb, proof_of_work_bits, PowTables{t, t + 12 * (size_t)nb, t + 13 * (size_t)nb}, bounce, nonces.data()));
+    QP_TRY(fri_grind(ctx, chs.data(), nb, proof_of_work_bits, PowTables{t, t + (12 + poseidon::POW_HEAD_WORDS) * (size_t)nb, t + (13 + poseidon::POW_HEAD_WORDS) * (size_t)nb}, bounce, nonces.data()));
     for (uint32_t b = 0; b < nb; b++) nonces_out[b] = nonces[b];
     return QPGPU_OK;
+}
+
+int qpgpu_pow_search(qpgpu_ctx *ctx, const uint64_t *states, uint32_t batch, uint32_t pos, unsigned proof_of_work_bits,
+                     const uint64_t *bases, uint64_t count, uint64_t *results_out) {
+    if (!ctx) return QPGPU_EINVAL;
+    QP_DEV(ctx);
+    if (!states || !bases || !results_out || batch == 0) return ctx->fail(QPGPU_EINVAL, "pow_search: null pointer or empty batch");
+    if (pos >= 12 || proof_of_work_bits == 0 || proof_of_work_bits > 40) return ctx->fail(QPGPU_EINVAL, "pow_search: pos must be below 12, proof_of_work_bits in 1..40");
+    if (batch > 65536 || count == 0 || count > (1ull << 41)) return ctx->fail(QPGPU_EINVAL, "pow_search: batch above 65 536 or count outside 1..2^41");
+    ctx->hasher_in_use = true;
+    QP_TRY(merkle_ensure_constants(ctx));
+    QP_TRY(ctx->ensure_scratch((size_t)batch * (16 + poseidon::POW_HEAD_WORDS) * 8));
+    Stager bounce;
+    u64 *t = ctx->scratch;
+    const PowTables tabs{t, t + (12 + poseidon::POW_HEAD_WORDS) * (size_t)batch, t + (13 + poseidon::POW_HEAD_WORDS) * (size_t)batch};
+    QP_TRY(pow_put_states(ctx, states, batch, pos, tabs, bounce));
+    QP_HIP(ctx, hipMemsetAsync(tabs.results, 0xFF, 8 * (size_t)batch, ctx->stream));
+    return pow_search(ctx, batch, pos, proof_of_work_bits, bases, count, tabs, bounce, results_out);
 }
 
 int qpgpu_fri_grind(qpgpu_ctx *ctx, const qpgpu_challenger *c, unsigned proof_of_work_bits, uint64_t *nonce_out) {
diff --git a/qp-zk-circuits_amd/csrc/fri_prover.cpp b/qp-zk-circuits_amd/csrc/fri_prover.cpp
--- a/qp-zk-circuits_amd/csrc/fri_prover.cpp
+++ b/qp-zk-circuits_amd/csrc/fri_prover.cpp
@@ -112,7 +112,7 @@
     l.ws = off;
     off = l.ws * nb;
     l.t_points = take(2 * (size_t)nb); l.t_shifts = take(2 * (size_t)nb); l.t_betas = take(2 * (size_t)nb);
-    l.pow_states = take(12 * (size_t)nb); l.pow_bases = take(nb); l.pow_results = take(nb); l.qidx = take((size_t)nb * p.num_queries);
+    l.pow_states = take((12 + poseidon::POW_HEAD_WORDS) * (size_t)nb); l.pow_bases = take(nb); l.pow_results = take(nb); l.qidx = take((size_t)nb * p.num_queries);
     l.total = off;
     return l;
 }
@@ -269,24 +269,37 @@
     return QPGPU_OK;
 }
 
+int pow_put_states(qpgpu_ctx *ctx, const u64 *states, uint32_t nb, uint32_t pos, const PowTables &t, Stager &stage) {
+    const HasherDev hd = ctx->hasher_dev();
+    std::vector<u64> up((12 + poseidon::POW_HEAD_WORDS) * (size_t)nb);
+    std::memcpy(up.data(), states, 12 * 8 * (size_t)nb);
+    if (hd.kind != hasher::POSEIDON2)
+        for (uint32_t b = 0; b < nb; b++)
+            poseidon::pow_head(states + 12 * (size_t)b, (int)pos, poseidon::host_hash_round_constants(), up.data() + 12 * (size_t)nb + poseidon::POW_HEAD_WORDS * (size_t)b);
+    return stage.put(ctx, t.states, up.data(), up.size() * 8);
+}
+int pow_search(qpgpu_ctx *ctx, uint32_t nb, uint32_t pos, unsigned pow_bits, const u64 *bases, u64 count, const PowTables &t, Stager &stage, u64 *res) {
+    PowArgs pw{};
+    pw.states = t.states; pw.heads = t.states + 12 * (size_t)nb; pw.bases = t.bases; pw.results = t.results;
+    pw.pos = pos; pw.pow_bits = pow_bits; pw.batch = nb; pw.count = count;
+    QP_TRY(stage.put(ctx, t.bases, bases, 8 * (size_t)nb));
+    QP_HIP(ctx, pk_pow(pw, ctx->hasher_dev(), ctx->stream));
+    return ctx->read_back(res, t.results, 8 * (size_t)nb);
+}
+
 int fri_grind(qpgpu_ctx *ctx, const Challenger *chs, uint32_t nb, unsigned pow_bits, const PowTables &t, Stager &stage, u64 *witness) {
     hipStream_t st = ctx->stream;
     ctx->prof_begin("prove_pow");
     for (uint32_t b = 0; b < nb; b++) witness[b] = 0;
     if (pow_bits > 0) {
-        const HasherDev hd = ctx->hasher_dev();
         std::vector<u64> states(12 * (size_t)nb);
         for (uint32_t b = 0; b < nb; b++) {
             std::memcpy(states.data() + 12 * (size_t)b, chs[b].state, 12 * 8);
             for (int i = 0; i < chs[b].n_in; i++) states[12 * (size_t)b + i] = chs[b].in[i];
             if (chs[b].n_in != chs[0].n_in) return ctx->fail(QPGPU_EDEVICE, "prove: transcripts of a batch diverged in length");
         }
-        QP_TRY(stage.put(ctx, t.states, states.data(), states.size() * 8));
-        PowArgs pw{};
-        pw.states = t.states; pw.bases = t.bases; pw.results = t.results;
-        pw.pos = (uint32_t)chs[0].n_in; pw.pow_bits = pow_bits; pw.batch = nb;
-        const u64 span = std::max<u64>(1ull << 16, 4ull << pw.pow_bits);
-        pw.count = span;
+        QP_TRY(pow_put_states(ctx, states.data(), nb, (uint32_t)chs[0].n_in, t, stage));
+        const u64 span = std::max<u64>(1ull << 16, 4ull << pow_bits);
         std::vector<u64> bases(nb, 0), res(nb);
         std::vector<char> found(nb, 0);
         uint32_t n_found = 0;
@@ -295,9 +308,7 @@
         for (u64 round = 0; n_found < nb; round++) {
             stage.pos = stage_pos;
             for (uint32_t b = 0; b < nb; b++) bases[b] = found[b] ? ~0ull : round * span;
-            QP_TRY(stage.put(ctx, t.bases, bases.data(), 8 * (size_t)nb));
-            QP_HIP(ctx, pk_pow(pw, hd, st));
-            QP_TRY(ctx->read_back(res.data(), t.results, 8 * (size_t)nb));
+            QP_TRY(pow_search(ctx, nb, (uint32_t)chs[0].n_in, pow_bits, bases.data(), span, t, stage, res.data()));
             for (uint32_t b = 0; b < nb; b++)
                 if (!found[b] && res[b] != ~0ull) { witness[b] = res[b]; found[b] = 1; n_found++; }
             if (round * span > (1ull << 41)) return ctx->fail(QPGPU_EDEVICE, "prove: proof of work not found");
diff --git a/qp-zk-circuits_amd/csrc/fri_prover.hpp b/qp-zk-circuits_amd/csrc/fri_prover.hpp
--- a/qp-zk-circuits_amd/csrc/fri_prover.hpp
+++ b/qp-zk-circuits_amd/csrc/fri_prover.hpp
@@ -27,5 +27,7 @@
 int fri_round_fold(FriState &s, const gl::e2 *betas);
 int fri_final_poly(FriState &s, std::vector<gl::u64> &out);
 struct PowTables { gl::u64 *states, *bases, *results; };
+int pow_put_states(qpgpu_ctx *ctx, const gl::u64 *states, uint32_t nb, uint32_t pos, const PowTables &t, Stager &stage);
+int pow_search(qpgpu_ctx *ctx, uint32_t nb, uint32_t pos, unsigned pow_bits, const gl::u64 *bases, gl::u64 count, const PowTables &t, Stager &stage, gl::u64 *res);
 int fri_grind(qpgpu_ctx *ctx, const Challenger *chs, uint32_t nb, unsigned pow_bits, const PowTables &t, Stager &stage, gl::u64 *witness);
 int fri_gather(FriState &s, const gl::u64 *qidx, uint32_t nq, ByteWriter *outs);
diff --git a/qp-zk-circuits_amd/csrc/merkle_api.cpp b/qp-zk-circuits_amd/csrc/merkle_api.cpp
--- a/qp-zk-circuits_amd/csrc/merkle_api.cpp
+++ b/qp-zk-circuits_amd/csrc/merkle_api.cpp
@@ -152,6 +152,21 @@
     return QPGPU_OK;
 }
 
+int qpgpu_merkle_leaf_hash_rows_dev(qpgpu_ctx *ctx, const uint64_t *d_rows, uint32_t width, unsigned log_leaves, uint32_t batch,
+                                    uint64_t ps_rows, uint64_t ps_digests, uint64_t *d_digests) {
+    if (!ctx) return QPGPU_EINVAL;
+    QP_DEV(ctx);
+    if (!d_rows || !d_digests || width == 0 || batch == 0) return ctx->fail(QPGPU_EINVAL, "merkle: null buffer, zero width or empty batch");
+    if (log_leaves > 40) return ctx->fail(QPGPU_EINVAL, "merkle: log_leaves out of range");
+    const uint64_t cnt = 1ull << log_leaves;
+    if (ps_rows / width < cnt || ps_digests < cnt * 4) return ctx->fail(QPGPU_EINVAL, "merkle: a tree's stride is shorter than the tree");
+    int rc = merkle_ensure_constants(ctx);
+    if (rc) return rc;
+    ctx->hasher_in_use = true;
+    QP_HIP(ctx, merkle_leaf_hash_rows(d_rows, cnt, width, d_digests, batch, ps_rows, ps_digests, ctx->hasher_dev(), ctx->stream));
+    return QPGPU_OK;
+}
+
 int qpgpu_poseidon2_hash_pad10_dev(qpgpu_ctx *ctx, const uint64_t *params, size_t n_words, const uint64_t *d_in, size_t len, size_t count, uint64_t *d_out) {
     if (!ctx) return QPGPU_EINVAL;
     QP_DEV(ctx);
diff --git a/qp-zk-circuits_amd/csrc/merkle_kernels.hip b/qp-zk-circuits_amd/csrc/merkle_kernels.hip
--- a/qp-zk-circuits_amd/csrc/merkle_kernels.hip
+++ b/qp-zk-circuits_amd/csrc/merkle_kernels.hip
@@ -19,6 +19,7 @@
 hipError_t fri_verify_upload_constants(const u64 *rc360);
 hipError_t merkle_mx_upload_constants(const u64 *rc360);
 hipError_t merkle_mx_leaves(const MerkleLeafArgs &a, u64 total, const HasherDev &h, hipStream_t st);
+hipError_t merkle_mx_rows(const u64 *rows, u64 n_leaves, u32 width, u64 *digests, u32 batch, u64 ps_rows, u64 ps_digests, const HasherDev &h, hipStream_t st);
 hipError_t merkle_mx_nodes(const u64 *in, u64 *out, u64 n_out, u32 batch, u64 ps, const HasherDev &h, hipStream_t st);
 hipError_t merkle_mx_pow(const PowArgs &a, const HasherDev &h, hipStream_t st);
 static bool mx_serves(const HasherDev &h) { return h.kind != hasher::POSEIDON2 || h.qp; }
@@ -245,8 +246,9 @@
         hipLaunchKernelGGL(leaf_rows_coop_kernel, grid, block, 0, st, rows, n_leaves, width, digests, batch, ps_rows, ps_digests);
         return hipGetLastError();
     }
-    return total >= tp_min_for(batch) ? merkle_tp_rows(rows, n_leaves, width, digests, batch, ps_rows, ps_digests, h, st)
-                                           : hash_launch_rows(rows, n_leaves, width, digests, batch, ps_rows, ps_digests, h, st);
+    if (total < tp_min_for(batch)) return hash_launch_rows(rows, n_leaves, width, digests, batch, ps_rows, ps_digests, h, st);
+    return (mx_serves(h) && width > 4 && mx_enabled()) ? merkle_mx_rows(rows, n_leaves, width, digests, batch, ps_rows, ps_digests, h, st)
+                                                       : merkle_tp_rows(rows, n_leaves, width, digests, batch, ps_rows, ps_digests, h, st);
 }
 static hipError_t merkle_reduce_level(const u64 *in, u64 *out, u64 n_out, u32 batch, u64 ps, const HasherDev &h, hipStream_t st) {
     if (n_out == 0) return hipSuccess;
diff --git a/qp-zk-circuits_amd/csrc/merkle_kernels_mx.hip b/qp-zk-circuits_amd/csrc/merkle_kernels_mx.hip
--- a/qp-zk-circuits_amd/csrc/merkle_kernels_mx.hip
+++ b/qp-zk-circuits_amd/csrc/merkle_kernels_mx.hip
@@ -22,6 +22,17 @@
         pmf::permute_head(s, c_poseidon_rc, lds);
         pmf::permute_tail_rounds(s, c_poseidon_rc);
     }
+    static constexpr bool POW_FROM_ROUND1 = true;
+    static __device__ __forceinline__ void pow_body(u64 (&s)[12], const u64 *head, u32 pos, u64 nonce, const poseidon2::Params *, const unsigned char *lds) {
+        const u64 y[1] = {poseidon::sbox7_lane(gl::add_canonical(nonce, c_poseidon_rc[pos]))};
+#pragma unroll
+        for (int r = 0; r < 12; r++) {
+            const u32 g[1] = {(u32)head[12 + r]};
+            s[r] = pmf::reduce96_terms(head[r], 0, y, g, 1);
+        }
+        pmf::permute_head<true>(s, c_poseidon_rc, lds);
+        pmf::permute_tail_rounds(s, c_poseidon_rc);
+    }
     template <int FIRST, int COUNT, bool CANON>
     static __device__ __forceinline__ void last_rows(u64 (&s)[12]) { pmf::last_layer_rows<FIRST, COUNT, CANON>(s); }
     static __device__ __forceinline__ void own_copy(u64 (&s)[12]) {
@@ -32,6 +43,8 @@
 struct Poseidon2QP {
     static __device__ __forceinline__ const uint4 *table() { return g_table_p2; }
     static __device__ __forceinline__ void body(u64 (&s)[12], const poseidon2::Params *p2, const unsigned char *lds) { pmf::permute_p2qp(s, *p2, lds); }
+    static constexpr bool POW_FROM_ROUND1 = false;
+    static __device__ __forceinline__ void pow_body(u64 (&)[12], const u64 *, u32, u64, const poseidon2::Params *, const unsigned char *) {}
     template <int FIRST, int COUNT, bool CANON>
     static __device__ __forceinline__ void last_rows(u64 (&)[12]) {}
     static __device__ __forceinline__ void own_copy(u64 (&)[12]) {}
@@ -79,6 +92,42 @@
     }
     if (live) {
         u64 *out = a.digests + j * 4;
+#pragma unroll
+        for (int i = 0; i < 4; i++) out[i] = s[i];
+    }
+}
+
+template <class Perm>
+MX_KERNEL leaf_hash_rows_kernel(const u64 *rows, u64 n_leaves, u32 width, u64 *digests, u32 batch, u64 ps_rows, u64 ps_digests, const poseidon2::Params *p2) {
+    const unsigned char *lds = table_to_lds<Perm>();
+    const u64 total = n_leaves * batch;
+    u64 gj = blockIdx.x * (u64)WG + threadIdx.x;
+    const bool live = gj < total;
+    gj = live ? gj : total - 1;
+    const u64 pr = gj >> ilog2_64(n_leaves), j = gj & (n_leaves - 1);
+    const u64 *row = rows + pr * ps_rows + j * width;
+    const bool vec = ((((u64)(uintptr_t)rows >> 3) | ps_rows | width) & 1) == 0;
+    u64 s[12];
+#pragma unroll
+    for (int i = 0; i < 12; i++) s[i] = 0;
+    for (u32 c = 0; c < width; c += 8) {
+        const u32 rest = width - c;
+        if (vec && rest >= 8) {
+            const ulonglong2 *p = reinterpret_cast<const ulonglong2 *>(row + c);
+            const ulonglong2 a = p[0], b = p[1], d = p[2], e = p[3];
+            s[0] = a.x; s[1] = a.y; s[2] = b.x; s[3] = b.y; s[4] = d.x; s[5] = d.y; s[6] = e.x; s[7] = e.y;
+        } else {
+#pragma unroll
+            for (int i = 0; i < 8; i++)
+                if (c + i < width) s[i] = row[c + i];
+        }
+        Perm::body(s, p2, lds);
+        if (rest <= 8) { Perm::own_copy(s); Perm::template last_rows<0, 4, true>(s); }
+        else if (rest >= 16) { Perm::own_copy(s); Perm::template last_rows<8, 4, false>(s); }
+        else { Perm::own_copy(s); Perm::template last_rows<0, 12, false>(s); }
+    }
+    if (live) {
+        u64 *out = digests + pr * ps_digests + j * 4;
 #pragma unroll
         for (int i = 0; i < 4; i++) out[i] = s[i];
     }
@@ -123,9 +172,14 @@
     const u64 idx = first + threadIdx.x, nonce = base + idx;
     const u64 *st = a.states + 12 * (u64)pr;
     u64 s[12];
-#pragma unroll
-    for (int i = 0; i < 12; i++) s[i] = (i == (int)a.pos) ? nonce : st[i];
-    permute_rows<Perm, 7, 1, true>(s, p2, lds);
+    if constexpr (Perm::POW_FROM_ROUND1) {
+        Perm::pow_body(s, a.heads + poseidon::POW_HEAD_WORDS * (u64)pr, a.pos, nonce, p2, lds);
+        Perm::template last_rows<7, 1, true>(s);
+    } else {
+#pragma unroll
+        for (int i = 0; i < 12; i++) s[i] = (i == (int)a.pos) ? nonce : st[i];
+        permute_rows<Perm, 7, 1, true>(s, p2, lds);
+    }
     if (idx < a.count && (s[7] >> (64 - a.pow_bits)) == 0) atomicMin((unsigned long long *)&a.results[pr], (unsigned long long)nonce);
 }
 
@@ -145,12 +199,13 @@
 template <class Perm>
 static hipError_t allow_table_in_lds() {
     hipError_t e = hipFuncSetAttribute((const void *)mx::leaf_hash_kernel<Perm>, hipFuncAttributeMaxDynamicSharedMemorySize, pmf::TABLE_BYTES);
+    if (e == hipSuccess) e = hipFuncSetAttribute((const void *)mx::leaf_hash_rows_kernel<Perm>, hipFuncAttributeMaxDynamicSharedMemorySize, pmf::TABLE_BYTES);
     if (e == hipSuccess) e = hipFuncSetAttribute((const void *)mx::node_kernel<Perm>, hipFuncAttributeMaxDynamicSharedMemorySize, pmf::TABLE_BYTES);
     if (e == hipSuccess) e = hipFuncSetAttribute((const void *)mx::pow_kernel<Perm>, hipFuncAttributeMaxDynamicSharedMemorySize, pmf::TABLE_BYTES);
     return e;
 }
 template <class Perm, class HostPerm>
-static hipError_t device_selftest(HostPerm host_perm, const poseidon2::Params *host_p2) {
+static hipError_t device_selftest(HostPerm host_perm, const poseidon2::Params *host_p2, const u64 *rc360) {
     constexpr int N = 4 * mx::WG;
     std::vector<u64> in((size_t)N * 12), out((size_t)N * 12);
     u64 seed = 0x9E3779B97F4A7C15ull;
@@ -182,17 +237,19 @@
         }
     constexpr u64 NL = 1ull << 19, NN = NL / 2, POW_COUNT = 1ull << 18;
     constexpr u32 WCOLS = 17, POW_BITS = 11, POW_BATCH = 2;
-    u64 *d_cols = nullptr, *d_dig = nullptr, *d_pow = nullptr;
-    std::vector<u64> cols((size_t)WCOLS * NL), dig(4 * (NL + NN)), powbuf(12 * POW_BATCH + 2 * POW_BATCH);
+    u64 *d_cols = nullptr, *d_dig = nullptr, *d_rdig = nullptr, *d_pow = nullptr;
+    std::vector<u64> cols((size_t)WCOLS * NL), dig(4 * (NL + NN)), rdig(4 * NL), powbuf((12 + 2 + poseidon::POW_HEAD_WORDS) * POW_BATCH);
     if (e == hipSuccess) {
         for (size_t i = 0; i < cols.size(); i++) { seed = seed * 6364136223846793005ull + 1442695040888963407ull; cols[i] = (seed ^ (seed >> 29)) % gl::P; }
         for (u32 b = 0; b < POW_BATCH; b++) {
             for (int i = 0; i < 12; i++) { seed = seed * 6364136223846793005ull + 1442695040888963407ull; powbuf[12 * b + i] = (seed ^ (seed >> 29)) % gl::P; }
             powbuf[12 * POW_BATCH + b] = 1000 * (b + 1);
             powbuf[12 * POW_BATCH + POW_BATCH + b] = ~0ull;
+            if (rc360) poseidon::pow_head(&powbuf[12 * b], 3, rc360, &powbuf[14 * POW_BATCH + poseidon::POW_HEAD_WORDS * b]);
         }
         e = hipMalloc((void **)&d_cols, cols.size() * 8);
         if (e == hipSuccess) e = hipMalloc((void **)&d_dig, dig.size() * 8);
+        if (e == hipSuccess) e = hipMalloc((void **)&d_rdig, rdig.size() * 8);
         if (e == hipSuccess) e = hipMalloc((void **)&d_pow, powbuf.size() * 8);
         if (e == hipSuccess) e = hipMemcpy(d_cols, cols.data(), cols.size() * 8, hipMemcpyHostToDevice);
         if (e == hipSuccess) e = hipMemcpy(d_pow, powbuf.data(), powbuf.size() * 8, hipMemcpyHostToDevice);
@@ -201,14 +258,16 @@
         MerkleLeafArgs la{};
         la.src0 = d_cols; la.stride0 = NL; la.ncols0 = WCOLS; la.n_leaves = NL; la.digests = d_dig; la.batch = 1;
         hipLaunchKernelGGL(mx::leaf_hash_kernel<Perm>, dim3((unsigned)(NL / mx::WG)), dim3(mx::WG), pmf::TABLE_BYTES, st, la, dp);
+        hipLaunchKernelGGL(mx::leaf_hash_rows_kernel<Perm>, dim3((unsigned)(NL / mx::WG)), dim3(mx::WG), pmf::TABLE_BYTES, st, (const u64 *)d_cols, NL, WCOLS, d_rdig, 1u, (u64)0, (u64)0, dp);
         hipLaunchKernelGGL(mx::node_kernel<Perm>, dim3((unsigned)(NN / mx::WG)), dim3(mx::WG), pmf::TABLE_BYTES, st, d_dig, d_dig + 4 * NL, NN, 1u, (u64)0, 1u, dp);
         PowArgs pa{};
         pa.states = d_pow; pa.bases = d_pow + 12 * POW_BATCH; pa.results = d_pow + 12 * POW_BATCH + POW_BATCH;
-        pa.pos = 3; pa.pow_bits = POW_BITS; pa.batch = POW_BATCH; pa.count = POW_COUNT;
+        pa.heads = d_pow + 14 * POW_BATCH; pa.pos = 3; pa.pow_bits = POW_BITS; pa.batch = POW_BATCH; pa.count = POW_COUNT;
         hipLaunchKernelGGL(mx::pow_kernel<Perm>, dim3((unsigned)(POW_COUNT / mx::WG * POW_BATCH)), dim3(mx::WG), pmf::TABLE_BYTES, st, pa, dp);
         e = hipGetLastError();
         if (e == hipSuccess) e = hipStreamSynchronize(st);
         if (e == hipSuccess) e = hipMemcpy(dig.data(), d_dig, dig.size() * 8, hipMemcpyDeviceToHost);
+        if (e == hipSuccess) e = hipMemcpy(rdig.data(), d_rdig, rdig.size() * 8, hipMemcpyDeviceToHost);
         if (e == hipSuccess) e = hipMemcpy(powbuf.data(), d_pow, powbuf.size() * 8, hipMemcpyDeviceToHost);
     }
     if (e == hipSuccess) {
@@ -220,6 +279,15 @@
                 host_perm(s);
             }
             for (int i = 0; i < 4; i++) if (s[i] != dig[4 * j + i]) e = hipErrorAssert;
+        }
+        for (u64 w = 0; w < NL / 64 && e == hipSuccess; w++) {
+            const u64 j = w * 64 + (w * 13) % 64;
+            u64 s[12] = {0};
+            for (u32 c = 0; c < WCOLS; c += 8) {
+                for (u32 i = 0; i < 8 && c + i < WCOLS; i++) s[i] = cols[(size_t)j * WCOLS + c + i];
+                host_perm(s);
+            }
+            for (int i = 0; i < 4; i++) if (s[i] != rdig[4 * j + i]) e = hipErrorAssert;
         }
         for (u64 w = 0; w < NN / 64 && e == hipSuccess; w++) {
             const u64 i0 = w * 64 + (w * 11) % 64;
@@ -242,6 +310,7 @@
     }
     if (d_cols) (void)hipFree(d_cols);
     if (d_dig) (void)hipFree(d_dig);
+    if (d_rdig) (void)hipFree(d_rdig);
     if (d_pow) (void)hipFree(d_pow);
     if (st) (void)hipStreamDestroy(st);
     if (d) (void)hipFree(d);
@@ -255,20 +324,27 @@
     if (e != hipSuccess) return e;
     e = hipMemcpyToSymbol(HIP_SYMBOL(mx::g_table), tab.data(), pmf::TABLE_BYTES);
     if (e == hipSuccess) e = allow_table_in_lds<mx::PoseidonV1>();
-    return e != hipSuccess ? e : device_selftest<mx::PoseidonV1>([&](u64 (&s)[12]) { poseidon::permute(s, rc360); }, nullptr);
+    return e != hipSuccess ? e : device_selftest<mx::PoseidonV1>([&](u64 (&s)[12]) { poseidon::permute(s, rc360); }, nullptr, rc360);
 }
 hipError_t merkle_upload_p2_tables(const poseidon2::Params &qp) {
     std::vector<unsigned char> tab(pmf::TABLE_BYTES);
     if (!pmf::build_tables_p2(qp, tab.data()) || !pmf::host_selfcheck_p2(qp, tab.data(), 64)) return hipErrorInvalidValue;
     hipError_t e = hipMemcpyToSymbol(HIP_SYMBOL(mx::g_table_p2), tab.data(), pmf::TABLE_BYTES);
     if (e == hipSuccess) e = allow_table_in_lds<mx::Poseidon2QP>();
-    return e != hipSuccess ? e : device_selftest<mx::Poseidon2QP>([&](u64 (&s)[12]) { poseidon2::permute(s, qp); }, &qp);
+    return e != hipSuccess ? e : device_selftest<mx::Poseidon2QP>([&](u64 (&s)[12]) { poseidon2::permute(s, qp); }, &qp, nullptr);
 }
 hipError_t merkle_mx_leaves(const MerkleLeafArgs &a, u64 total, const HasherDev &h, hipStream_t st) {
     const u64 blocks = (total + mx::WG - 1) / mx::WG;
     if (blocks > 0x7FFFFFFFull) return hipErrorInvalidValue;
     if (h.kind == hasher::POSEIDON2) hipLaunchKernelGGL(mx::leaf_hash_kernel<mx::Poseidon2QP>, dim3((unsigned)blocks), dim3(mx::WG), pmf::TABLE_BYTES, st, a, h.p2);
     else hipLaunchKernelGGL(mx::leaf_hash_kernel<mx::PoseidonV1>, dim3((unsigned)blocks), dim3(mx::WG), pmf::TABLE_BYTES, st, a, h.p2);
+    return hipGetLastError();
+}
+hipError_t merkle_mx_rows(const u64 *rows, u64 n_leaves, u32 width, u64 *digests, u32 batch, u64 ps_rows, u64 ps_digests, const HasherDev &h, hipStream_t st) {
+    const u64 blocks = (n_leaves * batch + mx::WG - 1) / mx::WG;
+    if (blocks > 0x7FFFFFFFull || width <= 4) return hipErrorInvalidValue;
+    if (h.kind == hasher::POSEIDON2) hipLaunchKernelGGL(mx::leaf_hash_rows_kernel<mx::Poseidon2QP>, dim3((unsigned)blocks), dim3(mx::WG), pmf::TABLE_BYTES, st, rows, n_leaves, width, digests, batch, ps_rows, ps_digests, h.p2);
+    else hipLaunchKernelGGL(mx::leaf_hash_rows_kernel<mx::PoseidonV1>, dim3((unsigned)blocks), dim3(mx::WG), pmf::TABLE_BYTES, st, rows, n_leaves, width, digests, batch, ps_rows, ps_digests, h.p2);
     return hipGetLastError();
 }
 hipError_t merkle_mx_nodes(const u64 *in, u64 *out, u64 n_out, u32 batch, u64 ps, const HasherDev &h, hipStream_t st) {
@@ -283,7 +359,8 @@
 }
 hipError_t merkle_mx_pow(const PowArgs &a, const HasherDev &h, hipStream_t st) {
     const u64 chunks = (a.count + mx::WG - 1) / mx::WG;
-    if (chunks * a.batch > 0x7FFFFFFFull) return hipErrorInvalidValue;
+    if (chunks * a.batch > 0x7FFFFFFFull || a.pos >= 12) return hipErrorInvalidValue;
+    if (h.kind != hasher::POSEIDON2 && !a.heads) return hipErrorInvalidValue;
     if (h.kind == hasher::POSEIDON2) hipLaunchKernelGGL(mx::pow_kernel<mx::Poseidon2QP>, dim3((unsigned)(chunks * a.batch)), dim3(mx::WG), pmf::TABLE_BYTES, st, a, h.p2);
     else hipLaunchKernelGGL(mx::pow_kernel<mx::PoseidonV1>, dim3((unsigned)(chunks * a.batch)), dim3(mx::WG), pmf::TABLE_BYTES, st, a, h.p2);
     return hipGetLastError();
diff --git a/qp-zk-circuits_amd/csrc/poseidon.hpp b/qp-zk-circuits_amd/csrc/poseidon.hpp
--- a/qp-zk-circuits_amd/csrc/poseidon.hpp
+++ b/qp-zk-circuits_amd/csrc/poseidon.hpp
@@ -259,11 +259,14 @@
     for (int i = 0; i < WIDTH; i++) s[i] = join_signed_halves(lo[i], hi[i]);
 }
 
-GL_HD void permute(u64 (&s)[WIDTH], const u64 *rc) {
-    int r = 0;
-    for (int k = 0; k < HALF_FULL; k++, r++) {
-#pragma unroll
-        for (int i = 0; i < WIDTH; i++) s[i] = gl::add_canonical(s[i], rc[r * WIDTH + i]);
+template <bool FROM_ROUND1>
+GL_HD void permute_from(u64 (&s)[WIDTH], const u64 *rc) {
+    int r = FROM_ROUND1 ? 1 : 0;
+    for (int k = r; k < HALF_FULL; k++, r++) {
+        if (!(FROM_ROUND1 && k == 1)) {
+#pragma unroll
+            for (int i = 0; i < WIDTH; i++) s[i] = gl::add_canonical(s[i], rc[r * WIDTH + i]);
+        }
         sbox7_layer(s);
         mds_layer(s);
     }
@@ -279,6 +282,22 @@
     }
 #pragma unroll
     for (int i = 0; i < WIDTH; i++) s[i] = gl::canon(s[i]);
+}
+GL_HD void permute(u64 (&s)[WIDTH], const u64 *rc) { permute_from<false>(s, rc); }
+constexpr int POW_HEAD_WORDS = 2 * WIDTH;
+GL_HD void pow_head(const u64 *st, int pos, const u64 *rc, u64 *head) {
+    constexpr u32 C[WIDTH] = {17, 15, 41, 16, 2, 28, 13, 13, 39, 18, 34, 20};
+    u64 t[WIDTH];
+    for (int i = 0; i < WIDTH; i++) t[i] = i == pos ? 0 : sbox7(gl::add_canonical(st[i], rc[i]));
+    mds_layer_naive(t);
+    for (int r = 0; r < WIDTH; r++) {
+        head[r] = gl::canon(gl::add_canonical(t[r], rc[WIDTH + r]));
+        head[WIDTH + r] = C[(pos - r + WIDTH) % WIDTH] + ((r == 0 && pos == 0) ? 8u : 0u);
+    }
+}
+GL_HD void pow_head_state(u64 (&s)[WIDTH], const u64 *head, int pos, u64 nonce, const u64 *rc) {
+    const u64 y = sbox7(gl::add_canonical(nonce, rc[pos]));
+    for (int r = 0; r < WIDTH; r++) s[r] = gl::add(head[r], gl::mul(y, head[WIDTH + r]));
 }
 GL_HD void permute_layerwise(u64 (&s)[WIDTH], const u64 *rc) {
     int r = 0;
diff --git a/qp-zk-circuits_amd/csrc/poseidon_mfma.hpp b/qp-zk-circuits_amd/csrc/poseidon_mfma.hpp
--- a/qp-zk-circuits_amd/csrc/poseidon_mfma.hpp
+++ b/qp-zk-circuits_amd/csrc/poseidon_mfma.hpp
@@ -486,11 +486,14 @@
         for (int o = 0; o < 4; o++) s[4 * f + o] = recombine(Z[o]);
     }
 }
+template <bool FROM_ROUND1 = false>
 __device__ __forceinline__ void permute_head(u64 (&s)[12], const u64 *rc, const unsigned char *lds) {
     using namespace poseidon;
-#pragma unroll
-    for (int i = 0; i < WIDTH; i++) s[i] = gl::add_canonical(s[i], rc[i]);
-    for (int k = 0; k < HALF_FULL; k++) {
+    if (!FROM_ROUND1) {
+#pragma unroll
+        for (int i = 0; i < WIDTH; i++) s[i] = gl::add_canonical(s[i], rc[i]);
+    }
+    for (int k = FROM_ROUND1 ? 1 : 0; k < HALF_FULL; k++) {
         sbox7_layer(s);
         if (k + 1 < HALF_FULL) mds_layer_words_rc(s, rc + (k + 1) * WIDTH);
     }
@@ -547,7 +550,7 @@
 }
 #elif defined(__HIPCC__)
 __device__ void permute(u64 (&s)[12], const u64 *rc, const unsigned char *lds);
-__device__ void permute_head(u64 (&s)[12], const u64 *rc, const unsigned char *lds);
+template <bool FROM_ROUND1 = false> __device__ void permute_head(u64 (&)[12], const u64 *, const unsigned char *) {}
 __device__ void permute_tail(u64 (&s)[12], const u64 *rc);
 __device__ void permute_tail_rounds(u64 (&s)[12], const u64 *rc);
 template <int FIRST, int COUNT, bool CANON> __device__ void last_layer_rows(u64 (&)[12]) {}
diff --git a/qp-zk-circuits_amd/csrc/prover_host.hpp b/qp-zk-circuits_amd/csrc/prover_host.hpp
--- a/qp-zk-circuits_amd/csrc/prover_host.hpp
+++ b/qp-zk-circuits_amd/csrc/prover_host.hpp
@@ -74,7 +74,7 @@
     static size_t words(const FriParams &p, const std::vector<size_t> &leaf_widths, size_t max_batch_polys, uint32_t nb);
     void bind(gl::u64 *base, const FriParams &p, const std::vector<size_t> &leaf_widths, size_t max_batch_polys, uint32_t nb);
     static size_t stage_words(const FriParams &p, size_t max_batch_polys, uint32_t nb) {
-        return (size_t)nb * (2 * max_batch_polys + p.num_queries + 2 * 2 * 4 + 2 * (p.arity_bits.size() + 1) + 14 + 8) + 64;
+        return (size_t)nb * (2 * max_batch_polys + p.num_queries + 2 * 2 * 4 + 2 * (p.arity_bits.size() + 1) + 14 + 24 + 8) + 64;
     }
 };
 
diff --git a/qp-zk-circuits_amd/csrc/prover_kernels.hpp b/qp-zk-circuits_amd/csrc/prover_kernels.hpp
--- a/qp-zk-circuits_amd/csrc/prover_kernels.hpp
+++ b/qp-zk-circuits_amd/csrc/prover_kernels.hpp
@@ -35,6 +35,7 @@
     const uint64_t *states;
     const uint64_t *bases;
     uint64_t *results;
+    const uint64_t *heads;
     uint32_t pos, pow_bits, batch;
     uint64_t count;
 };
```

Measured after the change: 1717. About the same (-0.1%).
